# honglianghe/CDNet

Measured on AMD Instinct MI355X. Metric: tiles/sec (train fwd+bwd+Adam), 256x256, higher is better.
Workload: dtype fp32

## Files before the change

cdnet_amd/_lib.py:

```python
import ctypes as C
import os

_HERE = os.path.dirname(os.path.abspath(__file__))
LIB_PATH = os.environ.get('CDNET_LIB_PATH') or os.path.join(_HERE, 'libcdnet_hip.so')

_vp, _i, _sz, _f, _u = C.c_void_p, C.c_int, C.c_size_t, C.c_float, C.c_uint


class ConvSrc(C.Structure):
    _fields_ = [('x', C.c_void_p), ('res', C.c_void_p), ('scale', C.c_void_p), ('shift', C.c_void_p),
                ('C', C.c_int), ('Hs', C.c_int), ('Ws', C.c_int), ('pool', C.c_int), ('relu', C.c_int),
                ('off_y', C.c_int), ('off_x', C.c_int), ('f16', C.c_int), ('row_stride', C.c_int)]


class ConvArgs(C.Structure):
    _fields_ = [('src', ConvSrc * 2), ('nsrc', C.c_int), ('w', C.c_void_p), ('bias', C.c_void_p),
                ('oscale', C.c_void_p), ('oshift', C.c_void_p), ('orelu', C.c_int), ('out', C.c_void_p),
                ('Cout', C.c_int), ('out_cstride', C.c_int), ('out_coff', C.c_int), ('stats', C.c_void_p),
                ('N', C.c_int), ('H', C.c_int), ('W', C.c_int), ('taps', C.c_int), ('npar', C.c_int),
                ('ostride', C.c_int), ('nchunk', C.c_int), ('tile', C.c_int), ('CK', C.c_int), ('BN', C.c_int),
                ('out_f16', C.c_int), ('debug', C.c_int), ('ws', C.c_int), ('f32', C.c_int),
                ('eres', C.c_void_p), ('eres_scale', C.c_void_p), ('eres_shift', C.c_void_p), ('eres_f16', C.c_int), ('eres_relu', C.c_int),
                ('taps1', C.c_int), ('pad_', C.c_int), ('pool_out', C.c_void_p),
                ('dot_w', C.c_void_p), ('dot_b', C.c_void_p), ('dot_out', C.c_void_p)]


class PackJob(C.Structure):
    _fields_ = [('w', C.c_void_p), ('packed', C.c_void_p), ('Cout', C.c_int), ('Cin', C.c_int), ('KH', C.c_int), ('KW', C.c_int),
                ('CK', C.c_int), ('BN', C.c_int), ('mode', C.c_int), ('pad_', C.c_int)]


class HeadFeat(C.Structure):
    _fields_ = [('raw', C.c_void_p), ('res', C.c_void_p), ('scale', C.c_void_p), ('shift', C.c_void_p),
                ('relu', C.c_int), ('f16', C.c_int)]


class FuseTerm(C.Structure):
    _fields_ = [('x', C.c_void_p), ('Hs', C.c_int), ('Ws', C.c_int), ('scale', C.c_void_p), ('shift', C.c_void_p),
                ('f16', C.c_int), ('pad_', C.c_int)]


class GradTerm(C.Structure):
    _fields_ = [('g', C.c_void_p), ('cstride', C.c_int), ('coff', C.c_int)]


class GradIn(C.Structure):
    _fields_ = [('g', C.c_void_p), ('Hg', C.c_int), ('Wg', C.c_int), ('oy', C.c_int), ('ox', C.c_int),
                ('pooled', C.c_int), ('coff', C.c_int), ('cstride', C.c_int), ('pad_', C.c_int)]


class BnBwdArgs(C.Structure):
    _fields_ = [('raw', C.c_void_p), ('res', C.c_void_p), ('scale', C.c_void_p), ('shift', C.c_void_p),
                ('mean', C.c_void_p), ('invstd', C.c_void_p), ('gin', GradIn * 3), ('ngin', C.c_int),
                ('f16', C.c_int), ('relu', C.c_int), ('N', C.c_int), ('H', C.c_int), ('W', C.c_int), ('C', C.c_int)]


class AugSample(C.Structure):
    _fields_ = [('minv', C.c_double * 6), ('img', C.c_void_p), ('weight', C.c_void_p), ('label', C.c_void_p)] + \
        [(n, C.c_int32) for n in ('H', 'W', 'img_stride', 'weight_stride', 'label_stride', 'label_i32')] + \
        [('color', C.c_float * 4)] + [(n, C.c_int32) for n in ('hflip', 'vflip', 'filter', 'y0', 'x0')] + \
        [('alpha', C.c_float), ('sigma', C.c_float), ('seed', C.c_uint32)]


class AugGeo(C.Structure):
    _fields_ = [('paff', C.c_double * 6), ('rinv', C.c_double * 6)] + [(n, C.c_int32) for n in ('Hr', 'Wr', 'fy0', 'fx0')] + \
        [('flags', C.c_uint32), ('reserved', C.c_int32)]


class WgradReduceDesc(C.Structure):
    _fields_ = [('slab', C.c_void_p), ('dw', C.c_void_p)] + [(n, C.c_int) for n in (
        'ksplit', 'npar', 'ci_blocks', 'co_blocks', 'taps', 'CI', 'CO', 'Csrc_real', 'Cin_real', 'src_coff', 'Cout', 'mode', 'block0', 'blocks')]

class DilatedConvArgs(C.Structure):
    _fields_ = [(n, C.c_void_p) for n in ('in_', 'w', 'scale', 'shift', 'out')] + [(n, C.c_int) for n in (
        'N', 'H', 'W', 'Cin', 'in_cstride', 'Cout', 'out_cstride', 'out_coff', 'taps', 'dilation', 'leaky')] + [
        ('slope', C.c_float), ('f32', C.c_int), ('out_nchw', C.c_int)]

class DilatedBwdDataArgs(C.Structure):
    _fields_ = [(n, C.c_void_p) for n in ('g', 'w', 'dx')] + [(n, C.c_int) for n in (
        'N', 'H', 'W', 'Cout', 'g_cstride', 'Cin', 'dx_cstride', 'dx_coff', 'taps', 'dilation', 'accumulate', 'f32')]

class DilatedWgradArgs(C.Structure):
    _fields_ = [(n, C.c_void_p) for n in ('x', 'g', 'dw', 'ws')] + [('ws_bytes', C.c_size_t)] + [(n, C.c_int) for n in (
        'N', 'H', 'W', 'Cin', 'x_cstride', 'Cout', 'g_cstride', 'taps', 'dilation')]

class SliceBnFwdArgs(C.Structure):
    _fields_ = [(n, C.c_void_p) for n in ('z', 'out', 'gamma', 'beta', 'running_mean', 'running_var', 'mean', 'invstd', 'ws')] + [
        ('ws_floats', C.c_size_t), ('P', C.c_longlong)] + [(n, C.c_int) for n in ('C', 'z_cstride', 'out_cstride', 'out_coff')] + [
        (n, C.c_float) for n in ('eps', 'momentum', 'p_drop')] + [('layer', C.c_int), ('key', C.c_ulonglong)]

class SliceBnBwdArgs(C.Structure):
    _fields_ = [(n, C.c_void_p) for n in ('dy', 'z', 'mean', 'invstd', 'gamma', 'dgamma', 'dbeta', 'g', 'ws')] + [
        ('ws_floats', C.c_size_t), ('P', C.c_longlong)] + [(n, C.c_int) for n in ('C', 'z_cstride', 'dy_cstride', 'dy_coff', 'g_cstride')] + [
        (n, C.c_float) for n in ('slope', 'p_drop')] + [('layer', C.c_int), ('key', C.c_ulonglong)]


MIRRORS = {
    'cdnet_conv_src': ConvSrc, 'cdnet_conv_args': ConvArgs, 'cdnet_pack_job': PackJob, 'cdnet_head_feat': HeadFeat,
    'cdnet_wgrad_reduce_desc': WgradReduceDesc, 'cdnet_grad_in': GradIn, 'cdnet_bn_bwd_args': BnBwdArgs, 'cdnet_fuse_term': FuseTerm,
    'cdnet_grad_term': GradTerm, 'cdnet_aug_sample': AugSample, 'cdnet_aug_geo': AugGeo, 'cdnet_dilated_conv_args': DilatedConvArgs,
    'cdnet_dilated_bwd_data_args': DilatedBwdDataArgs, 'cdnet_dilated_wgrad_args': DilatedWgradArgs,
    'cdnet_slice_bn_fwd_args': SliceBnFwdArgs, 'cdnet_slice_bn_bwd_args': SliceBnBwdArgs,
}

SIGNATURES = {
    'cdnet_abi_version': (_i, []),
    'cdnet_abi_sizeof': (_sz, [C.c_char_p]),
    'cdnet_last_error': (C.c_char_p, []),
    'cdnet_build_info': (C.c_char_p, []),
    'cdnet_spin': (_i, [_i, _vp]),
    'cdnet_box_copy': (_i, [_vp, _vp, _sz, _vp]),
    'cdnet_box_mfma': (_i, [_vp, _vp, _vp, _i, _i, _i, _vp]),
    'cdnet_ddm_codes': (_i, [_vp, _i, _i, _i, _i, _vp, _i, _i, _vp, _vp, _vp]),
    'cdnet_ddm_normalize': (_i, [_vp, _vp, _i, _i, _i, _vp, _vp]),
    'cdnet_probmaps': (_i, [_vp, _vp, _i, _i, _i, _i, _vp, _vp, _vp]),
    'cdnet_tta_boost_argmax': (_i, [_vp, _vp, _vp, _vp, _i, _i, _vp, _i, _i, _vp, _vp, _vp, _vp, _vp, _vp]),
    'cdnet_fuse_sum': (_i, [_vp, _i, _i, _i, _i, _i, _i, _vp, _i, _i, _vp]),
    'cdnet_upsample_bilinear_backward': (_i, [_vp, _i, _i, _i, _i, _i, _i, _i, _i, _vp, _vp]),
    'cdnet_s2d_to_nhwc': (_i, [_vp, _i, _i, _i, _i, _vp, _vp]),
    'cdnet_fuse_sum_f32': (_i, [_vp, _i, _i, _i, _i, _i, _i, _vp, _i, _i, _vp]),
    'cdnet_upsample_bilinear_backward_f32': (_i, [_vp, _i, _i, _i, _i, _i, _i, _i, _i, _vp, _vp]),
    'cdnet_s2d_to_nhwc_f32': (_i, [_vp, _i, _i, _i, _i, _vp, _vp]),
    'cdnet_bn_backward_stats': (_i, [_vp, _vp, _vp, _vp, _vp, _sz, _vp, _vp]),
    'cdnet_bn_backward_apply': (_i, [_vp, _vp, _vp, _vp]),
    'cdnet_bn_backward_finalize': (_i, [_vp, _vp, _vp, _vp, _vp, _i, _vp, _vp]),
    'cdnet_conv_ws_eligible': (_i, [_vp]),
    'cdnet_grad_sum': (_i, [_vp, _i, _vp, C.c_longlong, _i, _vp, _vp]),
    'cdnet_grad_sum_f32': (_i, [_vp, _i, _vp, C.c_longlong, _i, _vp, _vp]),
    'cdnet_label_pair_histogram': (_i, [_vp, _vp, _i, _i, _i, _i, _vp, _vp, _vp, _vp, _vp, _vp]),
    'cdnet_remap_label': (_i, [_vp, _i, _i, _i, _vp, _vp, _vp, _vp]),
    'cdnet_label_areas': (_i, [_vp, _i, _i, _i, _vp, _vp, _vp]),
    'cdnet_label_apply': (_i, [_vp, _i, _i, _i, _vp, _vp, _vp]),
    'cdnet_label_csr_workspace_bytes': (_sz, [_i]),
    'cdnet_label_csr': (_i, [_vp, _i, _i, _i, _vp, _sz, _vp, _vp, _vp, _vp, _vp]),
    'cdnet_hausdorff_tile_pixels': (_i, []),
    'cdnet_hausdorff_chunk_pixels': (_i, []),
    'cdnet_hausdorff_pairs': (_i, [_vp] * 8 + [_i, _i, _i, _vp, _i, _vp, _i, _vp, _vp, _vp]),
    'cdnet_watershed_workspace_bytes': (_sz, [_i, _i, _i]),
    'cdnet_watershed_process': (_i, [_vp, _i, _i, _i, _i, _vp, _sz, _vp, _vp, _vp, _vp]),
    'cdnet_fill_label_process': (_i, [_vp, _i, _i, _i, _i, _vp, _sz, _vp, _vp]),
    'cdnet_label_process': (_i, [_vp, _i, _i, _i, _i, _vp, _sz, _vp, _vp]),
    'cdnet_instance_redilate_workspace_bytes': (_sz, [_i, _i, _i, _i]),
    'cdnet_instance_redilate': (_i, [_vp, _i, _i, _i, _i, _i, _vp, _sz, _vp, _vp, _vp]),
    'cdnet_instance_redilate_lds_rows': (_i, []),
    'cdnet_instance_redilate_lds_cols': (_i, []),
    'cdnet_label_count': (_i, [_vp, _i, _i, _i, _vp, _vp, _vp, _vp]),
    'cdnet_tile_postproc_workspace_bytes': (_sz, [_i, _i, _i, _i]),
    'cdnet_tile_postproc': (_i, [_vp, _vp, _vp, _i, _i, _i, _i, _vp, _i, _i, _i, _i, _vp, _sz] + [_vp] * 10),
    'cdnet_cc_workspace_bytes': (_sz, [_i, _i, _i]),
    'cdnet_cc_chain': (_i, [_vp, _i, _i, _i, _i, _i, _i, _vp, _sz, _vp, _vp, _vp, _vp, _vp, _vp]),
    'cdnet_mask_views_argmax': (_i, [_vp, _i, _i, _i, _vp, _i, _i, _vp, _vp, _vp]),
    'cdnet_tile_mask_postproc_workspace_bytes': (_sz, [_i, _i, _i, _i]),
    'cdnet_tile_mask_postproc': (_i, [_vp, _i, _i, _i, _i, _i, _i, _vp, _sz] + [_vp] * 8),
    'cdnet_dilate_labels': (_i, [_vp, _i, _i, _i, _i, _vp, _vp]),
    'cdnet_conv_packed_weight_elems': (_sz, [_i] * 6),
    'cdnet_pack_conv_weights': (_i, [_vp, _vp] + [_i] * 7 + [_vp]),
    'cdnet_pack_conv_weights_scaled': (_i, [_vp, _vp, _vp] + [_i] * 7 + [_vp]),
    'cdnet_pack_batch_table_bytes': (_sz, [_i]),
    'cdnet_pack_conv_weights_batch': (_i, [_vp, _i, _vp, _sz, _i, _vp]),
    'cdnet_conv_forward': (_i, [_vp, _vp]),
    'cdnet_dilated_packed_weight_elems': (_sz, [_i, _i, _i, _i]),
    'cdnet_dilated_pack_weights': (_i, [_vp, _vp, _i, _i, _i, _i, _vp]),
    'cdnet_dilated_conv_forward': (_i, [_vp, _vp]),
    'cdnet_dilated_pack_weights_bwd': (_i, [_vp, _vp, _i, _i, _i, _i, _vp]),
    'cdnet_dilated_conv_backward_data': (_i, [_vp, _vp]),
    'cdnet_dilated_wgrad_workspace_bytes': (_sz, [_i] * 6),
    'cdnet_dilated_conv_backward_weight': (_i, [_vp, _vp]),
    'cdnet_slice_bn_workspace_floats': (_sz, [C.c_longlong, _i]),
    'cdnet_slice_bn_train_forward': (_i, [_vp, _vp]),
    'cdnet_slice_bn_train_backward': (_i, [_vp, _vp]),
    'cdnet_dropout_mask': (_i, [C.c_ulonglong, _i, _sz, _f, _vp, _vp]),
    'cdnet_maxpool2_forward': (_i, [_vp, _i, _vp, _i, _i, _vp, _i, _i, _i, _i, _i, _i, _vp]),
    'cdnet_maxpool2_backward': (_i, [_vp, _i, _i, _vp, _i, _vp, _i, _i, _i, _i, _i, _vp]),
    'cdnet_upsample4_bilinear_forward': (_i, [_vp, _i, _vp, _i, _i, _i, _i, _i, _i, _i, _vp]),
    'cdnet_upsample4_bilinear_backward': (_i, [_vp, _i, _i, _vp, _i, _i, _i, _i, _i, _vp]),
    'cdnet_src_materialize': (_i, [_vp, _i, _i, _i, _vp, _vp]),
    'cdnet_input_pack': (_i, [_vp, _i, _i, _i, _i, _vp, _vp]),
    'cdnet_input_pack_f32': (_i, [_vp, _i, _i, _i, _i, _vp, _vp]),
    'cdnet_bn_fold_eval': (_i, [_vp, _vp, _vp, _vp, _vp, _f, _i, _vp, _vp, _vp]),
    'cdnet_bn_finalize_train': (_i, [_vp, _i, _i, _f, _vp, _vp, _vp, _f, _f, _vp, _vp, _vp, _vp, _vp, _vp, _vp]),
    'cdnet_dam_head_forward': (_i, [_vp, _vp, _vp, _vp, _i, _i, _i, _vp, _vp, _vp, _vp]),
    'cdnet_final_conv1x1': (_i, [_vp, _vp, _vp, _i, _i, _i, _i, _vp, _vp]),
    'cdnet_bias_grad_workspace_floats': (_sz, [_i]),
    'cdnet_bias_grad': (_i, [_vp, _sz, _i, _vp, _sz, _vp, _vp]),
    'cdnet_bias_grad_f32': (_i, [_vp, _sz, _i, _vp, _sz, _vp, _vp]),
    'cdnet_final_conv1x1_backward_workspace_floats': (_sz, []),
    'cdnet_final_conv1x1_backward': (_i, [_vp, _vp, _vp, _i, _i, _i, _i, _vp, _vp, _sz, _vp, _vp, _vp]),
    'cdnet_final_conv1x1_c16': (_i, [_vp, _vp, _vp, _i, _i, _i, _i, _vp, _vp]),
    'cdnet_final_conv1x1_c16_backward_workspace_floats': (_sz, []),
    'cdnet_final_conv1x1_c16_backward': (_i, [_vp, _vp, _vp, _i, _i, _i, _i, _vp, _vp, _sz, _vp, _vp, _vp]),
    'cdnet_conv_wgrad_slab_floats': (_sz, [_i] * 6),
    'cdnet_conv_backward_weight': (_i, [_vp, _i, _i, _i, _vp] + [_i] * 9 + [_vp, _vp, _i, _vp]),
    'cdnet_conv_backward_weight_last_form': (_i, []),
    'cdnet_conv_forward_last_form': (_i, []),
    'cdnet_wgrad_reduce_desc_fill': (_i, [_i] * 9 + [_vp, _vp, _i, _i, _vp]),
    'cdnet_wgrad_reduce_batch': (_i, [_vp, _i, _i, _vp]),
    'cdnet_bn_backward_workspace_floats': (_sz, [_i]),
    'cdnet_bn_backward': (_i, [_vp, _vp, _vp, _vp, _vp, _sz, _vp, _vp, _vp]),
    'cdnet_bn_backward_last_plan': (_i, []),
    'cdnet_bn_backward_last_sums_plan': (_i, []),
    'cdnet_dam_head_backward_workspace_floats': (_sz, [_i, _i, _i]),
    'cdnet_dam_head_backward': (_i, [_vp] * 7 + [_i, _i, _i, _vp, _vp, _vp, _vp, _sz, _vp, _vp]),
    'cdnet_dam_head_backward_fused_blocks': (_i, []),
    'cdnet_dam_head_backward_fused_scratch_bytes': (_i, []),
    'cdnet_dam_head_backward_fused_workspace_floats': (_sz, []),
    'cdnet_dam_head_backward_fused': (_i, [_vp] * 7 + [_i, _i, _i, _vp, _vp, _vp, _vp, _sz, _vp, _vp]),
    'cdnet_dam_loss_workspace_floats': (_sz, [_i, _i]),
    'cdnet_dam_loss': (_i, [_vp] * 7 + [_i, _i, _i, _i, _vp, _sz, _vp, _vp, _vp, _vp, _vp]),
    'cdnet_dam_loss_classes_workspace_floats': (_sz, [_i, _i, _i]),
    'cdnet_dam_loss_classes': (_i, [_vp] * 7 + [_i, _i, _i, _i, _i, _vp, _sz, _vp, _vp, _vp, _vp, _vp]),
    'cdnet_dam_loss_terms': (_i, [_vp] * 7 + [_i, _i, _i, _i, _i, _vp, _sz, _vp, _vp, _vp, _vp, _vp, _u]),
    'cdnet_mask_loss_workspace_floats': (_sz, [_i, _i]),
    'cdnet_mask_loss': (_i, [_vp, _vp, _vp, _i, _i, _i, _u, _vp, _sz, _vp, _vp, _vp]),
    'cdnet_variance_loss_workspace_bytes': (_sz, [_i, _i, _i, _i]),
    'cdnet_variance_loss': (_i, [_vp, _vp, _i, _i, _i, _i, _i, _f, _vp, _sz, _vp, _vp, _vp, _vp, _vp, _vp]),
    'cdnet_boundary_loss_workspace_bytes': (_sz, [_i, _i, _i, _i, _i]),
    'cdnet_boundary_loss': (_i, [_vp, _vp, _i, _i, _i, _i, _i, _f, _vp, _sz, _vp, _vp, _vp, _vp]),
    'cdnet_boundary_loss_scratch_bytes': (_i, []),
    'cdnet_dam_val_sums_workspace_floats': (_sz, [_i, _i]),
    'cdnet_dam_val_sums': (_i, [_vp] * 8 + [_i, _i, _i, _vp, _sz, _vp, _vp]),
    'cdnet_dam_val_sums_classes_workspace_floats': (_sz, [_i, _i, _i]),
    'cdnet_dam_val_sums_classes': (_i, [_vp] * 8 + [_i, _i, _i, _i, _vp, _sz, _vp, _vp]),
    'cdnet_adam_step': (_i, [_vp, _vp, _vp, _vp, _sz, _f, _f, _f, _f, _f, _i, _f, _vp]),
    'cdnet_moment_step': (_i, [_vp, _vp, _vp, _vp, _vp, _sz, C.c_double, C.c_double, _f, _i, _i, _f, _f, _f, _f, _i, _f, _vp]),
    'cdnet_sgd_step': (_i, [_vp, _vp, _vp, _sz, _f, _f, _f, _i, _f, _vp]),
    'cdnet_window_pack': (_i, [_vp] + [_i] * 9 + [_vp, _vp]),
    'cdnet_window_pack_f32': (_i, [_vp] + [_i] * 9 + [_vp, _vp]),
    'cdnet_window_stitch': (_i, [_vp] + [_i] * 9 + [_vp, _vp]),
    'cdnet_label_encoding_workspace_bytes': (_sz, [_i, _i, _i, _i]),
    'cdnet_label_encoding_instances_workspace_bytes': (_sz, [_i, _i, _i, _i]),
    'cdnet_label_encoding_instances': (_i, [_vp, _i, _i, _i, _i, _vp, _vp, _vp, _sz, _vp, _vp, _vp, _vp, _vp, _vp]),
    'cdnet_augment_workspace_bytes': (_sz, [_i, _i, _i]),
    'cdnet_augment_batch': (_i, [_vp, _vp, _i, _i, _vp, _vp, _sz, _vp, _vp, _vp, _i, _vp, _vp, _vp]),
    'cdnet_augment_geo_workspace_bytes': (_sz, [_i, _i, _i, _i]),
    'cdnet_augment_batch_geo': (_i, [_vp, _vp, _vp, _vp, _i, _i, _i, _vp, _vp, _sz, _vp, _vp, _vp, _i, _vp, _vp, _vp]),
    'cdnet_label_encoding': (_i, [_vp, _i, _i, _i, _i, _vp, _vp, _vp, _sz, _vp, _vp, _vp, _vp, _vp, _vp]),
    'cdnet_weight_map_radius': (_i, [C.c_double, C.c_double]),
    'cdnet_weight_map': (_i, [_vp, _i, _i, C.c_double, C.c_double, _vp, _vp]),
}

_lib = None


class CdnetHipError(RuntimeError):
    pass


def load():
    global _lib
    if _lib is not None:
        return _lib
    import torch
    if not os.path.exists(LIB_PATH):
        raise CdnetHipError('libcdnet_hip.so is not built: run `python -m cdnet_amd.csrc.build` '
                            '(or __graft_entry__.build()). There is no CPU fallback.')
    lib = C.CDLL(LIB_PATH)
    for name, (res, args) in SIGNATURES.items():
        fn = getattr(lib, name)
        fn.restype = res
        fn.argtypes = args
    if lib.cdnet_abi_version() != 5:
        raise CdnetHipError('ABI version mismatch (libcdnet_hip.so is version %d, this binding 5): rebuild with python -m cdnet_amd.csrc.build' % lib.cdnet_abi_version())
    _lib = lib
    return lib


def check(status, what=''):
    if status != 0:
        msg = load().cdnet_last_error().decode(errors='replace')
        raise CdnetHipError('%s failed (code %d): %s' % (what, status, msg))


def call(name, *args):
    check(getattr(load(), name)(*args), name)


def entry(name, f32):
    return name + '_f32' if f32 else name


_RAW_STREAM = None


def stream_ptr():
    global _RAW_STREAM
    if _RAW_STREAM is None:
        import torch
        get, dev = getattr(torch._C, '_cuda_getCurrentRawStream', None), getattr(torch._C, '_cuda_getDevice', None)
        if get is not None and dev is not None:
            _RAW_STREAM = lambda: get(dev())
        else:
            _RAW_STREAM = lambda: torch.cuda.current_stream().cuda_stream
    return C.c_void_p(_RAW_STREAM())


def ptr(t):
    if t is None:
        return None
    assert t.is_cuda and t.is_contiguous(), 'ABI needs contiguous device tensors'
    return C.c_void_p(t.data_ptr())
```

cdnet_amd/csrc/bn_bwd.hip:

```cpp
#include "train_util.h"
#include "bn_sums.h"

using namespace cdnet;

namespace {

struct GradIn {
    const unsigned short *g;
    int Hg, Wg;
    int oy, ox;
    int pooled;
    int coff, cstride;
};

struct BnBwdArgs {
    const unsigned short *raw;
    const unsigned short *res;
    int f16;
    const float *scale, *shift;
    int relu;
    const float *mean, *invstd;
    GradIn gin[3];
    int ngin;
    int N, H, W, C;
    float *partial;
    const float *k1, *k2, *k3;
    unsigned short *draw;
    unsigned short *dz_out;
    int rev;
};


__device__ __forceinline__ void act8_f32(const BnBwdArgs &A, size_t e, const float *sc, const float *sh, float *a, float *rawf) {
    float x[8], r[8];
    ldf8(A.raw, e, x);
    if (A.res) ldf8(A.res, e, r);
#pragma unroll
    for (int j = 0; j < 8; ++j) {
        if (rawf) rawf[j] = x[j];
        float v = A.scale ? fmaf(x[j], sc[j], sh[j]) : x[j];
        if (A.relu == 2) v = r[j];
        else {
            if (A.res) v += r[j];
            if (A.relu) v = fmaxf(v, 0.f);
        }
        a[j] = v;
    }
}

template <bool F32 = false>
__device__ __forceinline__ void act8(const BnBwdArgs &A, size_t e, const float *sc, const float *sh, float *a, float *rawf) {
    if (F32) { act8_f32(A, e, sc, sh, a, rawf); return; }
    V16 r, rr;
    r.u = *reinterpret_cast<const uint4 *>(A.raw + e);
    rr.u = make_uint4(0, 0, 0, 0);
    if (A.res) rr.u = *reinterpret_cast<const uint4 *>(A.res + e);
    const bool f16 = A.f16 != 0;
#pragma unroll
    for (int j = 0; j < 8; ++j) {
        float x = ld16(r.h[j], f16);
        if (rawf) rawf[j] = x;
        float v = A.scale ? fmaf(x, sc[j], sh[j]) : x;
        if (A.res) v += ld16(rr.h[j], f16);
        if (A.relu) v = fmaxf(v, 0.f);
        a[j] = bf2f(f2bf(v));
    }
}

template <bool WANT_XHAT, bool F32 = false>
__device__ __forceinline__ void dz8(const BnBwdArgs &A, int n, int y, int x, int c0, const float *sc, const float *sh,
                                    const float *mu, const float *is, float *dz, float *xhat) {
    const size_t e = (((size_t)n * A.H + y) * A.W + x) * A.C + c0;
    float a[8], rawf[8];
    act8<F32>(A, e, sc, sh, a, rawf);
    float g[8];
#pragma unroll
    for (int j = 0; j < 8; ++j) g[j] = 0.f;
    for (int k = 0; k < A.ngin; ++k) {
        const GradIn &gi = A.gin[k];
        if (!gi.pooled) {
            const int yy = y + gi.oy, xx = x + gi.ox;
            if (yy >= 0 && yy < gi.Hg && xx >= 0 && xx < gi.Wg) {
                const size_t ge = (((size_t)n * gi.Hg + yy) * gi.Wg + xx) * gi.cstride + gi.coff + c0;
                if (F32) {
                    float t[8];
                    ldf8(gi.g, ge, t);
#pragma unroll
                    for (int j = 0; j < 8; ++j) g[j] += t[j];
                } else {
                    V16 v;
                    v.u = *reinterpret_cast<const uint4 *>(gi.g + ge);
#pragma unroll
                    for (int j = 0; j < 8; ++j) g[j] += bf2f(v.h[j]);
                }
            }
        } else {
            const int py = y >> 1, px = x >> 1;
            if (py < gi.Hg && px < gi.Wg) {
                bool sel[8];
#pragma unroll
                for (int j = 0; j < 8; ++j) sel[j] = true;
                const int q0 = (y & 1) * 2 + (x & 1);
#pragma unroll
                for (int q = 0; q < 4; ++q) {
                    if (q == q0) continue;
                    const int yy = (y & ~1) + (q >> 1), xx = (x & ~1) + (q & 1);
                    if (yy >= A.H || xx >= A.W) continue;
                    float b[8];
                    act8<F32>(A, (((size_t)n * A.H + yy) * A.W + xx) * A.C + c0, sc, sh, b, nullptr);
#pragma unroll
                    for (int j = 0; j < 8; ++j) sel[j] = sel[j] && (q < q0 ? a[j] > b[j] : a[j] >= b[j]);
                }
                const size_t ge = (((size_t)n * gi.Hg + py) * gi.Wg + px) * gi.cstride + gi.coff + c0;
                if (F32) {
                    float t[8];
                    ldf8(gi.g, ge, t);
#pragma unroll
                    for (int j = 0; j < 8; ++j) g[j] += sel[j] ? t[j] : 0.f;
                } else {
                    V16 v;
                    v.u = *reinterpret_cast<const uint4 *>(gi.g + ge);
#pragma unroll
                    for (int j = 0; j < 8; ++j) g[j] += sel[j] ? bf2f(v.h[j]) : 0.f;
                }
            }
        }
    }
#pragma unroll
    for (int j = 0; j < 8; ++j) {
        dz[j] = (A.relu && !(a[j] > 0.f)) ? 0.f : g[j];
        if (WANT_XHAT) xhat[j] = A.mean ? (rawf[j] - mu[j]) * is[j] : 0.f;
    }
}

template <int V>
__device__ __forceinline__ void bn_load_row(const float *p, int c0, float *o, float dflt) {
#pragma unroll
    for (int j = 0; j < V; ++j) o[j] = p ? p[c0 + j] : dflt;
}

template <int V>
__device__ __forceinline__ void bn_load_const(const BnBwdArgs &A, int c0, bool apply, float (&sc)[V], float (&sh)[V], float (&mu)[V], float (&is)[V],
                                              float (&k1)[V], float (&k2)[V], float (&k3)[V]) {
    bn_load_row<V>(A.scale, c0, sc, 1.f); bn_load_row<V>(A.shift, c0, sh, 0.f); bn_load_row<V>(A.mean, c0, mu, 0.f); bn_load_row<V>(A.invstd, c0, is, 1.f);
    if (apply) { bn_load_row<V>(A.k1, c0, k1, 1.f); bn_load_row<V>(A.k2, c0, k2, 0.f); bn_load_row<V>(A.k3, c0, k3, 0.f); }
}

template <int V>
__device__ __forceinline__ void bn_write_partial(float *partial, int C, int VPP, const float *s1, const float *s2) {
    __shared__ float s_red[256][2 * V + 1];
    const int tid = threadIdx.x;
#pragma unroll
    for (int j = 0; j < V; ++j) { s_red[tid][j] = s1[j]; s_red[tid][V + j] = s2[j]; }
    __syncthreads();
    for (int q = tid; q < 2 * V * VPP; q += 256) {
        const int sl = q % VPP, j = q / VPP;
        float t = 0.f;
        for (int k = sl; k < 256; k += VPP) t += s_red[k][j];
        float *op = partial + (size_t)blockIdx.x * 2 * C;
        op[(j / V) * C + sl * V + (j % V)] = t;
    }
}

constexpr int BN_U = 4;
constexpr int BN_MAX_BLOCKS = 2048;
constexpr int BN_BLOCKS_CAP = 512;
static_assert(BN_BLOCKS_CAP <= BN_MAX_BLOCKS, "workspace rows");

static int bn_grid(size_t count, int C, int V, int unroll) {
    const size_t per_block = (size_t)(256 / (C / V)) * unroll;
    const size_t nb = (count + per_block - 1) / per_block;
    return nb > (size_t)BN_BLOCKS_CAP ? BN_BLOCKS_CAP : (nb < 1 ? 1 : (int)nb);
}

template <bool F32 = false>
__device__ __forceinline__ void dz8_at(const BnBwdArgs &A, unsigned p, unsigned HW, int c0, const float *sc, const float *sh, const float *mu,
                                       const float *is, float *dz, float *xh) {
    const unsigned n = p / HW, r = p - n * HW;
    const unsigned y = r / (unsigned)A.W, x = r - y * (unsigned)A.W;
    dz8<true, F32>(A, (int)n, (int)y, (int)x, c0, sc, sh, mu, is, dz, xh);
}

template <typename Body>
__device__ __forceinline__ void bn_bwd_dispatch(bool f16, int relu, Body &&body) {
    using T_ = std::true_type;
    using F_ = std::false_type;
    if (f16) {
        if (relu == 0) body(T_{}, std::integral_constant<int, 0>{});
        else if (relu == 1) body(T_{}, std::integral_constant<int, 1>{});
        else body(T_{}, std::integral_constant<int, 2>{});
    } else {
        if (relu == 0) body(F_{}, std::integral_constant<int, 0>{});
        else if (relu == 1) body(F_{}, std::integral_constant<int, 1>{});
        else body(F_{}, std::integral_constant<int, 2>{});
    }
}

template <int NF, bool APPLY>
__global__ __launch_bounds__(256) void bn_bwd_window_kernel(BnBwdArgs A, int kp) {
    const int VPP = A.C / 8;
    const int slot = (int)threadIdx.x % VPP, c0 = slot * 8;
    float sc[8], sh[8], mu[8], is[8], k1[8], k2[8], k3[8], s1[8], s2[8];
    bn_load_const(A, c0, APPLY, sc, sh, mu, is, k1, k2, k3);
#pragma unroll
    for (int j = 0; j < 8; ++j) { s1[j] = 0.f; s2[j] = 0.f; }
    const unsigned H = A.H, W = A.W, Hp = (H + 1) / 2, Wp = (W + 1) / 2, nwin = (unsigned)A.N * Hp * Wp;
    const unsigned ppb = 256 / VPP;
    const GradIn gp = A.gin[kp];
    int kf[2] = {0, 0};
    {
        int m = 0;
        for (int k = 0; k < A.ngin && m < NF; ++k)
            if (k != kp) kf[m++] = k;
    }
    bn_bwd_dispatch(A.f16 != 0, A.relu != 0 ? 1 : 0, [&](auto f16_c, auto relu_c) {
    constexpr bool f16 = decltype(f16_c)::value, relu = decltype(relu_c)::value != 0;
    for (unsigned w0 = first_pixel(ppb, VPP); w0 < nwin; w0 += gridDim.x * ppb) {
        const unsigned w = (APPLY && A.rev) ? nwin - 1 - w0 : w0;
        const unsigned n = w / (Hp * Wp), r = w - n * Hp * Wp;
        const unsigned py = r / Wp, px = r - py * Wp;
        V16 raw[4], g[4][NF > 0 ? NF : 1], gv;
        unsigned pix[4];
        bool ok[4];
#pragma unroll
        for (int q = 0; q < 4; ++q) {
            unsigned yy = 2 * py + (q >> 1), xx = 2 * px + (q & 1);
            ok[q] = yy < H && xx < W;
            yy = yy < H ? yy : H - 1;
            xx = xx < W ? xx : W - 1;
            pix[q] = (n * H + yy) * W + xx;
            raw[q].u = *reinterpret_cast<const uint4 *>(A.raw + (size_t)pix[q] * A.C + c0);
#pragma unroll
            for (int m = 0; m < NF; ++m)
                g[q][m].u = *reinterpret_cast<const uint4 *>(A.gin[kf[m]].g + (size_t)pix[q] * A.gin[kf[m]].cstride + A.gin[kf[m]].coff + c0);
        }
        const bool pok = py < (unsigned)gp.Hg && px < (unsigned)gp.Wg;
        {
            const unsigned cy = pok ? py : 0, cx = pok ? px : 0;
            gv.u = *reinterpret_cast<const uint4 *>(gp.g + (((size_t)n * gp.Hg + cy) * gp.Wg + cx) * gp.cstride + gp.coff + c0);
        }
        V16 o[4];
#pragma unroll
        for (int j = 0; j < 8; ++j) {
            float x[4], a[4];
#pragma unroll
            for (int q = 0; q < 4; ++q) {
                x[q] = ld16(raw[q].h[j], f16);
                float v = fmaf(x[q], sc[j], sh[j]);
                if (relu) v = fmaxf(v, 0.f);
                a[q] = bf2f(f2bf(v));
            }
            int bi = 0;
            float best = a[0];
#pragma unroll
            for (int q = 1; q < 4; ++q)
                if (ok[q] && a[q] > best) { best = a[q]; bi = q; }
            const float gpool = pok ? bf2f(gv.h[j]) : 0.f;
#pragma unroll
            for (int q = 0; q < 4; ++q) {
                float gs = (bi == q) ? gpool : 0.f;
#pragma unroll
                for (int m = 0; m < NF; ++m) gs += bf2f(g[q][m].h[j]);
                const float dz = (!ok[q] || (relu && !(a[q] > 0.f))) ? 0.f : gs;
                const float xh = (x[q] - mu[j]) * is[j];
                if (APPLY) o[q].h[j] = f2bf(k1[j] * (dz - k2[j] - xh * k3[j]));
                else { s1[j] += dz; s2[j] = fmaf(dz, xh, s2[j]); }
            }
        }
        if (APPLY) {
#pragma unroll
            for (int q = 0; q < 4; ++q)
                if (ok[q]) *reinterpret_cast<uint4 *>(A.draw + (size_t)pix[q] * A.C + c0) = o[q].u;
        }
    }
    });
    if (!APPLY) bn_write_partial<8>(A.partial, A.C, VPP, s1, s2);
}

template <int NG, bool RES, bool APPLY>
__global__ __launch_bounds__(256) void bn_bwd_flat_kernel(BnBwdArgs A) {
    const int VPP = A.C / 8;
    const int slot = (int)threadIdx.x % VPP, c0 = slot * 8;
    float sc[8], sh[8], mu[8], is[8], k1[8], k2[8], k3[8], s1[8], s2[8];
    bn_load_const(A, c0, APPLY, sc, sh, mu, is, k1, k2, k3);
#pragma unroll
    for (int j = 0; j < 8; ++j) { s1[j] = 0.f; s2[j] = 0.f; }
    const unsigned npix = (unsigned)(A.N * A.H * A.W);
    const unsigned ppb = 256 / VPP, step = gridDim.x * ppb;
    const bool rev = APPLY && A.rev != 0;
    bn_bwd_dispatch(A.f16 != 0, A.relu, [&](auto f16_c, auto relu_c) {
        constexpr bool F16 = decltype(f16_c)::value;
        constexpr int RELU = decltype(relu_c)::value;
        for (unsigned p0 = first_pixel(ppb, VPP); p0 < npix; p0 += step * BN_U) {
            V16 raw[BN_U], res[BN_U], g[BN_U][NG];
#pragma unroll
            for (int u = 0; u < BN_U; ++u) {
                unsigned p = p0 + u * step;
                p = p < npix ? p : npix - 1;
                p = rev ? npix - 1 - p : p;
                raw[u].u = *reinterpret_cast<const uint4 *>(A.raw + (size_t)p * A.C + c0);
                if (RES) res[u].u = *reinterpret_cast<const uint4 *>(A.res + (size_t)p * A.C + c0);
#pragma unroll
                for (int k = 0; k < NG; ++k)
                    g[u][k].u = *reinterpret_cast<const uint4 *>(A.gin[k].g + (size_t)p * A.gin[k].cstride + A.gin[k].coff + c0);
            }
#pragma unroll
            for (int u = 0; u < BN_U; ++u) {
                const unsigned p = p0 + u * step;
                const bool valid = p < npix;
                V16 o, z;
#pragma unroll
                for (int j = 0; j < 8; ++j) {
                    const float x = ld16(raw[u].h[j], F16);
                    float v = fmaf(x, sc[j], sh[j]);
                    if (RES) v = RELU == 2 ? bf2f(res[u].h[j]) : v + ld16(res[u].h[j], F16);
                    float gs = bf2f(g[u][0].h[j]);
#pragma unroll
                    for (int k = 1; k < NG; ++k) gs += bf2f(g[u][k].h[j]);
                    const bool keep = (APPLY || valid) & (RELU == 0 || bf2f(f2bf(v)) > 0.f);
                    const float dz = keep ? gs : 0.f;
                    const float xh = (x - mu[j]) * is[j];
                    if (APPLY) {
                        o.h[j] = f2bf(k1[j] * (dz - k2[j] - xh * k3[j]));
                        z.h[j] = f2bf(dz);
                    } else {
                        s1[j] += dz;
                        s2[j] = fmaf(dz, xh, s2[j]);
                        if (RES) res[u].h[j] = f2bf(dz);
                    }
                }
                if (APPLY) {
                    if (valid) {
                        const unsigned pw = rev ? npix - 1 - p : p;
                        *reinterpret_cast<uint4 *>(A.draw + (size_t)pw * A.C + c0) = o.u;
                        if (RES) *reinterpret_cast<uint4 *>(A.dz_out + (size_t)pw * A.C + c0) = z.u;
                    }
                } else {
                    if (RES && A.dz_out && valid) *reinterpret_cast<uint4 *>(A.dz_out + (size_t)p * A.C + c0) = res[u].u;
                }
            }
        }
    });
    if (!APPLY) bn_write_partial<8>(A.partial, A.C, VPP, s1, s2);
}

template <int NG, bool RES, bool APPLY>
__global__ __launch_bounds__(256) void bn_bwd_flat32_kernel(BnBwdArgs A) {
    const int VPP = A.C / 4;
    const int slot = (int)threadIdx.x % VPP, c0 = slot * 4;
    float sc[4], sh[4], mu[4], is[4], k1[4], k2[4], k3[4], s1[4], s2[4];
    bn_load_row<4>(A.scale, c0, sc, 1.f); bn_load_row<4>(A.shift, c0, sh, 0.f); bn_load_row<4>(A.mean, c0, mu, 0.f); bn_load_row<4>(A.invstd, c0, is, 1.f);
    if (APPLY) { bn_load_row<4>(A.k1, c0, k1, 1.f); bn_load_row<4>(A.k2, c0, k2, 0.f); bn_load_row<4>(A.k3, c0, k3, 0.f); }
#pragma unroll
    for (int j = 0; j < 4; ++j) { s1[j] = 0.f; s2[j] = 0.f; }
    const unsigned npix = (unsigned)(A.N * A.H * A.W);
    const unsigned ppb = 256 / VPP, step = gridDim.x * ppb;
    const bool relu = A.relu != 0, outmask = A.relu == 2;
    const float *raw = reinterpret_cast<const float *>(A.raw), *resp = reinterpret_cast<const float *>(A.res);
    float *draw = reinterpret_cast<float *>(A.draw), *dzo = reinterpret_cast<float *>(A.dz_out);
    for (unsigned p0 = first_pixel(ppb, VPP); p0 < npix; p0 += step * BN_U) {
        f32x4 x[BN_U], r[BN_U], g[BN_U][NG];
#pragma unroll
        for (int u = 0; u < BN_U; ++u) {
            unsigned p = p0 + u * step;
            p = p < npix ? p : npix - 1;
            if (APPLY && A.rev) p = npix - 1 - p;
            x[u] = *reinterpret_cast<const f32x4 *>(raw + (size_t)p * A.C + c0);
            if (RES) r[u] = *reinterpret_cast<const f32x4 *>(resp + (size_t)p * A.C + c0);
#pragma unroll
            for (int k = 0; k < NG; ++k)
                g[u][k] = *reinterpret_cast<const f32x4 *>(reinterpret_cast<const float *>(A.gin[k].g) + (size_t)p * A.gin[k].cstride + A.gin[k].coff + c0);
        }
#pragma unroll
        for (int u = 0; u < BN_U; ++u) {
            const unsigned p = p0 + u * step;
            const bool valid = p < npix;
            f32x4 o, z;
#pragma unroll
            for (int j = 0; j < 4; ++j) {
                float v = fmaf(x[u][j], sc[j], sh[j]);
                if (RES) v = outmask ? r[u][j] : v + r[u][j];
                float gs = g[u][0][j];
#pragma unroll
                for (int k = 1; k < NG; ++k) gs += g[u][k][j];
                const float dz = (!valid || (relu && !(v > 0.f))) ? 0.f : gs;
                const float xh = (x[u][j] - mu[j]) * is[j];
                if (APPLY) { o[j] = k1[j] * (dz - k2[j] - xh * k3[j]); z[j] = dz; }
                else { s1[j] += dz; s2[j] = fmaf(dz, xh, s2[j]); z[j] = dz; }
            }
            if (APPLY && valid) {
                const unsigned pw = A.rev ? npix - 1 - p : p;
                *reinterpret_cast<f32x4 *>(draw + (size_t)pw * A.C + c0) = o;
                if (RES) *reinterpret_cast<f32x4 *>(dzo + (size_t)pw * A.C + c0) = z;
            }
            if (!APPLY && RES && dzo && valid) *reinterpret_cast<f32x4 *>(dzo + (size_t)p * A.C + c0) = z;
        }
    }
    if (!APPLY) bn_write_partial<4>(A.partial, A.C, VPP, s1, s2);
}

template <int NF, bool APPLY>
__global__ __launch_bounds__(256) void bn_bwd_window32_kernel(BnBwdArgs A, int kp) {
    const int VPP = A.C / 4;
    const int slot = (int)threadIdx.x % VPP, c0 = slot * 4;
    float sc[4], sh[4], mu[4], is[4], k1[4], k2[4], k3[4], s1[4], s2[4];
    bn_load_const(A, c0, APPLY, sc, sh, mu, is, k1, k2, k3);
#pragma unroll
    for (int j = 0; j < 4; ++j) { s1[j] = 0.f; s2[j] = 0.f; }
    const unsigned H = A.H, W = A.W, Hp = (H + 1) / 2, Wp = (W + 1) / 2, nwin = (unsigned)A.N * Hp * Wp;
    const unsigned ppb = 256 / VPP;
    const bool relu = A.relu != 0;
    const GradIn gp = A.gin[kp];
    const float *gpool_p = reinterpret_cast<const float *>(gp.g);
    const float *raw = reinterpret_cast<const float *>(A.raw);
    float *draw = reinterpret_cast<float *>(A.draw);
    const float *gf[NF > 0 ? NF : 1];
    int gcs[NF > 0 ? NF : 1], gco[NF > 0 ? NF : 1];
    {
        int m = 0;
        for (int k = 0; k < A.ngin && m < NF; ++k)
            if (k != kp) { gf[m] = reinterpret_cast<const float *>(A.gin[k].g); gcs[m] = A.gin[k].cstride; gco[m] = A.gin[k].coff; ++m; }
    }
    for (unsigned w0 = first_pixel(ppb, VPP); w0 < nwin; w0 += gridDim.x * ppb) {
        const unsigned w = (APPLY && A.rev) ? nwin - 1 - w0 : w0;
        const unsigned n = w / (Hp * Wp), r = w - n * Hp * Wp;
        const unsigned py = r / Wp, px = r - py * Wp;
        f32x4 x[4], g[4][NF > 0 ? NF : 1], gv;
        unsigned pix[4];
        bool ok[4];
#pragma unroll
        for (int q = 0; q < 4; ++q) {
            unsigned yy = 2 * py + (q >> 1), xx = 2 * px + (q & 1);
            ok[q] = yy < H && xx < W;
            yy = yy < H ? yy : H - 1;
            xx = xx < W ? xx : W - 1;
            pix[q] = (n * H + yy) * W + xx;
            x[q] = *reinterpret_cast<const f32x4 *>(raw + (size_t)pix[q] * A.C + c0);
#pragma unroll
            for (int m = 0; m < NF; ++m)
                g[q][m] = *reinterpret_cast<const f32x4 *>(gf[m] + (size_t)pix[q] * gcs[m] + gco[m] + c0);
        }
        const bool pok = py < (unsigned)gp.Hg && px < (unsigned)gp.Wg;
        {
            const unsigned cy = pok ? py : 0, cx = pok ? px : 0;
            gv = *reinterpret_cast<const f32x4 *>(gpool_p + (((size_t)n * gp.Hg + cy) * gp.Wg + cx) * gp.cstride + gp.coff + c0);
        }
        f32x4 o[4];
#pragma unroll
        for (int j = 0; j < 4; ++j) {
            float a[4];
#pragma unroll
            for (int q = 0; q < 4; ++q) {
                const float v = fmaf(x[q][j], sc[j], sh[j]);
                a[q] = relu ? fmaxf(v, 0.f) : v;
            }
            int bi = 0;
            float best = a[0];
#pragma unroll
            for (int q = 1; q < 4; ++q)
                if (ok[q] && a[q] > best) { best = a[q]; bi = q; }
            const float gpool = pok ? gv[j] : 0.f;
#pragma unroll
            for (int q = 0; q < 4; ++q) {
                const float pt = (bi == q) ? gpool : 0.f;
                float gsum;
                if (NF == 0) gsum = 0.f + pt;
                else if (NF == 1) gsum = (0.f + (kp == 0 ? pt : g[q][0][j])) + (kp == 0 ? g[q][0][j] : pt);
                else gsum = ((0.f + (kp == 0 ? pt : g[q][0][j])) + (kp == 0 ? g[q][0][j] : (kp == 1 ? pt : g[q][NF - 1][j]))) +
                            (kp == 2 ? pt : g[q][NF - 1][j]);
                const float dz = (!ok[q] || (relu && !(a[q] > 0.f))) ? 0.f : gsum;
                const float xh = (x[q][j] - mu[j]) * is[j];
                if (APPLY) o[q][j] = k1[j] * (dz - k2[j] - xh * k3[j]);
                else { s1[j] += dz; s2[j] = fmaf(dz, xh, s2[j]); }
            }
        }
        if (APPLY) {
#pragma unroll
            for (int q = 0; q < 4; ++q)
                if (ok[q]) *reinterpret_cast<f32x4 *>(draw + (size_t)pix[q] * A.C + c0) = o[q];
        }
    }
    if (!APPLY) bn_write_partial<4>(A.partial, A.C, VPP, s1, s2);
}

template <bool F32, bool APPLY>
__global__ __launch_bounds__(256) void bn_bwd_generic_kernel(BnBwdArgs A) {
    const int VPP = A.C / 8;
    const int slot = (int)threadIdx.x % VPP, c0 = slot * 8;
    float sc[8], sh[8], mu[8], is[8], k1[8], k2[8], k3[8], s1[8], s2[8];
    bn_load_const(A, c0, APPLY, sc, sh, mu, is, k1, k2, k3);
#pragma unroll
    for (int j = 0; j < 8; ++j) { s1[j] = 0.f; s2[j] = 0.f; }
    const unsigned HW = (unsigned)(A.H * A.W), npix = (unsigned)A.N * HW;
    const unsigned ppb = 256 / VPP;
    const unsigned step = gridDim.x * ppb;
    for (unsigned p0 = first_pixel(ppb, VPP); p0 < npix; p0 += step * BN_U) {
        float dz[BN_U][8], xh[BN_U][8];
#pragma unroll
        for (int u = 0; u < BN_U; ++u) {
            const unsigned p = p0 + u * step;
            if (p < npix) dz8_at<F32>(A, p, HW, c0, sc, sh, mu, is, dz[u], xh[u]);
            else if (!APPLY) {
#pragma unroll
                for (int j = 0; j < 8; ++j) { dz[u][j] = 0.f; xh[u][j] = 0.f; }
            }
        }
#pragma unroll
        for (int u = 0; u < BN_U; ++u) {
            const unsigned p = p0 + u * step;
            if (!APPLY) {
#pragma unroll
                for (int j = 0; j < 8; ++j) { s1[j] += dz[u][j]; s2[j] = fmaf(dz[u][j], xh[u][j], s2[j]); }
                continue;
            }
            if (p >= npix) continue;
            float o32[8];
#pragma unroll
            for (int j = 0; j < 8; ++j) o32[j] = k1[j] * (dz[u][j] - k2[j] - xh[u][j] * k3[j]);
            if (F32) {
                if (A.draw) stf8(A.draw, (size_t)p * A.C + c0, o32);
                if (A.dz_out) stf8(A.dz_out, (size_t)p * A.C + c0, dz[u]);
                continue;
            }
            V16 o, z;
#pragma unroll
            for (int j = 0; j < 8; ++j) { o.h[j] = f2bf(o32[j]); z.h[j] = f2bf(dz[u][j]); }
            if (A.draw) *reinterpret_cast<uint4 *>(A.draw + (size_t)p * A.C + c0) = o.u;
            if (A.dz_out) *reinterpret_cast<uint4 *>(A.dz_out + (size_t)p * A.C + c0) = z.u;
        }
    }
    if (!APPLY) bn_write_partial<8>(A.partial, A.C, VPP, s1, s2);
}

__global__ __launch_bounds__(256) void bn_bwd_finalize_kernel(const float *__restrict__ partial, int nb, int C, float M, const float *gamma,
                                                              const float *invstd, float *dgamma, float *dbeta, float *k1, float *k2,
                                                              float *k3) {
    const int c = blockIdx.x;
    double s1, s2;
    bn_sum_partials(partial, nb, C, c, s1, s2);
    if (threadIdx.x == 0) {
        if (dbeta) dbeta[c] = (float)s1;
        if (dgamma) dgamma[c] = (float)s2;
        k1[c] = gamma[c] * invstd[c];
        k2[c] = (float)(s1 / M);
        k3[c] = (float)(s2 / M);
    }
}

__global__ void bn_ktab_copy_kernel(const float *scale, const float *shift, const float *mean, const float *invstd, int C, float *ktab) {
    const int c = blockIdx.x * blockDim.x + threadIdx.x;
    if (c < C) { ktab[c] = scale[c]; ktab[C + c] = shift[c]; ktab[2 * C + c] = mean[c]; ktab[3 * C + c] = invstd[c]; }
}

}

static int fill_bn_args(const cdnet_bn_bwd_args *a, BnBwdArgs &A, const char *who) {
    CDNET_REQUIRE(a && a->raw, "%s: null pointer", who);
    CDNET_REQUIRE(a->C % 8 == 0 && a->C >= 8 && a->C <= 2048 , "%s: C=%d unsupported", who, a->C);
    CDNET_REQUIRE(a->ngin >= 1 && a->ngin <= 3, "%s: ngin=%d", who, a->ngin);
    A.raw = a->raw; A.res = a->res; A.f16 = a->f16; A.scale = a->scale; A.shift = a->shift; A.relu = a->relu;
    A.mean = a->mean; A.invstd = a->invstd;
    for (int k = 0; k < 3; ++k) {
        A.gin[k].g = a->gin[k].g; A.gin[k].Hg = a->gin[k].Hg; A.gin[k].Wg = a->gin[k].Wg;
        A.gin[k].oy = a->gin[k].oy; A.gin[k].ox = a->gin[k].ox; A.gin[k].pooled = a->gin[k].pooled;
        A.gin[k].coff = a->gin[k].coff; A.gin[k].cstride = a->gin[k].cstride ? a->gin[k].cstride : a->C;
        if (k < a->ngin) CDNET_REQUIRE(a->gin[k].g, "%s: null gradient input %d", who, k);
        if (k < a->ngin) CDNET_REQUIRE(a->gin[k].Hg >= 1 && a->gin[k].Wg >= 1, "%s: empty gradient input %d (%d x %d)", who, k, a->gin[k].Hg, a->gin[k].Wg);
    }
    A.ngin = a->ngin; A.N = a->N; A.H = a->H; A.W = a->W; A.C = a->C;
    A.partial = nullptr; A.k1 = A.k2 = A.k3 = nullptr; A.draw = nullptr; A.dz_out = nullptr;
    return CDNET_OK;
}

enum BnPath { BN_WINDOW, BN_FLAT, BN_GENERIC };
struct BnPlan {
    BnPath path;
    bool f32;
    int nb;
    int kp, nflat;
    bool flat_sources;
};

static size_t bn_npix(const BnBwdArgs &A) { return (size_t)A.N * A.H * A.W; }

static BnPlan bn_plan_plain(const BnBwdArgs &A) {
    const bool f32 = A.f16 == 2;
    return BnPlan{BN_FLAT, f32, bn_grid(bn_npix(A), A.C, f32 ? 4 : 8, BN_U), 0, 0, true};
}

static BnPlan bn_plan(const BnBwdArgs &A, const void *draw, const void *dz_out) {
    bool simple = true;
    int npool = 0, kp = 0, nflat = 0;
    for (int k = 0; k < A.ngin; ++k) {
        const GradIn &g = A.gin[k];
        const bool same = !g.pooled && g.oy == 0 && g.ox == 0 && g.Hg == A.H && g.Wg == A.W;
        simple = simple && same;
        if (g.pooled) { ++npool; kp = k; }
        else if (same) ++nflat;
    }
    const bool window = npool == 1 && nflat == A.ngin - 1 && nflat <= 2 && A.mean && A.scale && !A.res && draw && !dz_out;
    const bool flat = !window && simple && A.mean && A.scale && draw && ((A.res != nullptr) == (dz_out != nullptr));
    const bool f32 = A.f16 == 2, fits32 = A.C <= 1024;
    BnPlan P{BN_GENERIC, f32, 0, kp, nflat, flat};
    if (window && (!f32 || (fits32 && A.shift && A.invstd))) P.path = BN_WINDOW;
    else if (flat && (!f32 || fits32)) P.path = BN_FLAT;
    const int V = f32 && P.path != BN_GENERIC ? 4 : 8;
    P.nb = window ? bn_grid((size_t)A.N * ((A.H + 1) / 2) * ((A.W + 1) / 2), A.C, V, 1) : bn_grid(bn_npix(A), A.C, V, BN_U);
    return P;
}

static thread_local int g_bn_last_plan[2] = {0, 0};
static thread_local int g_bn_last_pass = 0;

static int bn_plan_record(const BnPlan &P, const BnBwdArgs &A, bool apply, bool dz_source) {
    const int path = P.path == BN_WINDOW ? CDNET_BN_PATH_WINDOW : P.path == BN_FLAT ? CDNET_BN_PATH_FLAT : CDNET_BN_PATH_GENERIC;
    const int n = P.path == BN_WINDOW ? P.nflat : P.path == BN_FLAT ? A.ngin : 0;
    const int res = P.path == BN_FLAT && A.res ? 1 : 0;
    const int kp = P.path == BN_WINDOW ? P.kp : 0;
    return path | (P.f32 ? 1 : 0) << 2 | n << 3 | res << 5 | kp << 6 | (apply ? 1 : 0) << 8 | (dz_source ? 1 : 0) << 9 | P.nb << 10;
}

template <bool APPLY>
static void launch(const BnPlan &P, const BnBwdArgs &A, hipStream_t st, bool dz_source = false) {
    g_bn_last_plan[APPLY ? 1 : 0] = bn_plan_record(P, A, APPLY, dz_source);
    g_bn_last_pass = APPLY ? 1 : 0;
    auto window = [&](auto nf) {
        constexpr int NF = decltype(nf)::value;
        if (P.f32) bn_bwd_window32_kernel<NF, APPLY><<<P.nb, 256, 0, st>>>(A, P.kp);
        else bn_bwd_window_kernel<NF, APPLY><<<P.nb, 256, 0, st>>>(A, P.kp);
    };
    auto flat = [&](auto ng, auto res) {
        constexpr int NG = decltype(ng)::value;
        constexpr bool RES = decltype(res)::value;
        if (P.f32) bn_bwd_flat32_kernel<NG, RES, APPLY><<<P.nb, 256, 0, st>>>(A);
        else bn_bwd_flat_kernel<NG, RES, APPLY><<<P.nb, 256, 0, st>>>(A);
    };
    using std::integral_constant;
    using std::true_type;
    using std::false_type;
    switch (P.path) {
        case BN_WINDOW:
            if (P.nflat == 0) window(integral_constant<int, 0>{});
            else if (P.nflat == 1) window(integral_constant<int, 1>{});
            else window(integral_constant<int, 2>{});
            break;
        case BN_FLAT:
            switch (A.ngin * 2 + (A.res ? 1 : 0)) {
                case 2: flat(integral_constant<int, 1>{}, false_type{}); break;
                case 3: flat(integral_constant<int, 1>{}, true_type{}); break;
                case 4: flat(integral_constant<int, 2>{}, false_type{}); break;
                case 5: flat(integral_constant<int, 2>{}, true_type{}); break;
                case 6: flat(integral_constant<int, 3>{}, false_type{}); break;
                default: flat(integral_constant<int, 3>{}, true_type{}); break;
            }
            break;
        case BN_GENERIC:
            if (P.f32) bn_bwd_generic_kernel<true, APPLY><<<P.nb, 256, 0, st>>>(A);
            else bn_bwd_generic_kernel<false, APPLY><<<P.nb, 256, 0, st>>>(A);
            break;
    }
}

static void bn_finalize(const BnBwdArgs &A, const float *partial, int nb, const float *gamma, float *dgamma, float *dbeta, float *k,
                        hipStream_t st) {
    bn_bwd_finalize_kernel<<<A.C, 256, 0, st>>>(partial, nb, A.C, (float)bn_npix(A), gamma, A.invstd, dgamma, dbeta, k, k + A.C, k + 2 * A.C);
}

static void bn_set_coeffs(BnBwdArgs &A, const float *k) { A.k1 = k; A.k2 = k + A.C; A.k3 = k + 2 * A.C; }

static BnBwdArgs bn_dz_as_source(const BnBwdArgs &A, const unsigned short *dz) {
    BnBwdArgs B = A;
    B.ngin = 1;
    B.gin[0].g = dz; B.gin[0].Hg = A.H; B.gin[0].Wg = A.W; B.gin[0].oy = 0; B.gin[0].ox = 0; B.gin[0].pooled = 0;
    B.gin[0].coff = 0; B.gin[0].cstride = A.C;
    B.res = nullptr; B.relu = 0; B.dz_out = nullptr;
    return B;
}

extern "C" int cdnet_bn_backward(const cdnet_bn_bwd_args *a, const float *gamma, float *dgamma, float *dbeta, float *workspace,
                                 size_t workspace_floats, uint16_t *draw, uint16_t *dz_out, void *stream) {
    BnBwdArgs A;
    int rc = fill_bn_args(a, A, "cdnet_bn_backward");
    if (rc) return rc;
    hipStream_t st = (hipStream_t)stream;
    const size_t npix = bn_npix(A);
    CDNET_REQUIRE(npix * (size_t)A.C < ((size_t)1 << 32) && npix < ((size_t)1 << 31), "cdnet_bn_backward: tensor too large for 32-bit pixel indexing");
    const BnPlan P = bn_plan(A, draw, dz_out);
    CDNET_REQUIRE(A.relu != 2 || (P.flat_sources && A.res), "cdnet_bn_backward: relu = 2 (mask from the stored output) needs same-size gradient sources and res");
    static const bool dz_reuse = !(getenv("CDNET_BN_DZ_REUSE") && atoi(getenv("CDNET_BN_DZ_REUSE")) == 0);
    const bool reuse = dz_reuse && P.path == BN_FLAT && A.mean && A.res && dz_out;
    A.draw = draw;
    A.rev = 1;
    if (A.mean) {
        CDNET_REQUIRE(gamma && A.invstd && workspace, "cdnet_bn_backward: BatchNorm layer needs gamma/invstd/workspace");
        const size_t need = (size_t)P.nb * 2 * A.C + 3 * (size_t)A.C;
        if (workspace_floats < need) { set_error("cdnet_bn_backward: workspace %zu < %zu floats", workspace_floats, need); return CDNET_E_WORKSPACE; }
        A.partial = workspace;
        A.dz_out = dz_reuse ? dz_out : nullptr;
        float *k = workspace + (size_t)P.nb * 2 * A.C;
        launch<false>(P, A, st);
        bn_finalize(A, A.partial, P.nb, gamma, dgamma, dbeta, k, st);
        bn_set_coeffs(A, k);
    }
    A.dz_out = dz_out;
    launch<true>(P, reuse ? bn_dz_as_source(A, dz_out) : A, st, reuse);
    return check_launch("cdnet_bn_backward");
}

static bool bn_plain_case(const BnBwdArgs &A, bool masked = false) {
    const GradIn &g = A.gin[0];
    return A.ngin == 1 && !g.pooled && g.oy == 0 && g.ox == 0 && g.Hg == A.H && g.Wg == A.W && A.mean && A.scale && A.shift && A.invstd && !A.res &&
           (A.relu == 1 || (masked && A.relu == 0)) && (g.cstride == 0 || g.cstride == A.C) && g.coff == 0;
}

extern "C" int cdnet_bn_backward_stats(const cdnet_bn_bwd_args *a, const float *gamma, float *dgamma, float *dbeta, float *workspace,
                                       size_t workspace_floats, float *ktab, void *stream) {
    BnBwdArgs A;
    int rc = fill_bn_args(a, A, "cdnet_bn_backward_stats");
    if (rc) return rc;
    CDNET_REQUIRE(bn_plain_case(A) && A.f16 != 2 && gamma && workspace && ktab, "cdnet_bn_backward_stats: plain 16-bit case only (one same-size gradient, BatchNorm + ReLU, no residual)");
    hipStream_t st = (hipStream_t)stream;
    const size_t npix = bn_npix(A);
    CDNET_REQUIRE(npix * (size_t)A.C < ((size_t)1 << 32) && npix < ((size_t)1 << 31), "cdnet_bn_backward_stats: tensor too large for 32-bit pixel indexing");
    const BnPlan P = bn_plan_plain(A);
    const size_t need = (size_t)P.nb * 2 * A.C;
    if (workspace_floats < need) { set_error("cdnet_bn_backward_stats: workspace %zu < %zu floats", workspace_floats, need); return CDNET_E_WORKSPACE; }
    A.partial = workspace;
    A.rev = 0;
    bn_ktab_copy_kernel<<<cdiv(A.C, 256), 256, 0, st>>>(A.scale, A.shift, A.mean, A.invstd, A.C, ktab);
    launch<false>(P, A, st);
    bn_finalize(A, A.partial, P.nb, gamma, dgamma, dbeta, ktab + 4 * A.C, st);
    return check_launch("cdnet_bn_backward_stats");
}

extern "C" int cdnet_bn_backward_finalize(const cdnet_bn_bwd_args *a, const float *gamma, float *dgamma, float *dbeta, const float *partial,
                                          int nb, float *ktab, void *stream) {
    BnBwdArgs A;
    int rc = fill_bn_args(a, A, "cdnet_bn_backward_finalize");
    if (rc) return rc;
    CDNET_REQUIRE(bn_plain_case(A) && gamma && partial && ktab && nb >= 1, "cdnet_bn_backward_finalize: plain case only");
    bn_finalize(A, partial, nb, gamma, dgamma, dbeta, ktab + 4 * A.C, (hipStream_t)stream);
    return check_launch("cdnet_bn_backward_finalize");
}

extern "C" int cdnet_bn_backward_apply(const cdnet_bn_bwd_args *a, const float *ktab, uint16_t *draw, void *stream) {
    BnBwdArgs A;
    int rc = fill_bn_args(a, A, "cdnet_bn_backward_apply");
    if (rc) return rc;
    CDNET_REQUIRE(bn_plain_case(A, true) && ktab && draw, "cdnet_bn_backward_apply: plain case only");
    CDNET_REQUIRE(A.f16 != 2 || A.C <= 1024, "cdnet_bn_backward_apply(f32): C=%d > 1024", A.C);
    A.rev = 1;
    A.draw = draw;
    bn_set_coeffs(A, ktab + 4 * A.C);
    launch<true>(bn_plan_plain(A), A, (hipStream_t)stream);
    return check_launch("cdnet_bn_backward_apply");
}

extern "C" int cdnet_bn_backward_last_plan(void) { return g_bn_last_plan[g_bn_last_pass]; }
extern "C" int cdnet_bn_backward_last_sums_plan(void) { return g_bn_last_plan[0]; }

extern "C" size_t cdnet_bn_backward_workspace_floats(int C) { return (size_t)BN_MAX_BLOCKS * 2 * C + 3 * (size_t)C; }
```

cdnet_amd/csrc/head_bwd.hip:

```cpp
#include "train_util.h"
#include "head_feat.h"

using namespace cdnet;

namespace {

__device__ __forceinline__ void feat8_f32(const HeadFeat &f, size_t pix, int c0, const float *s_sc, const float *s_sh, float *v) {
    float x[8], r[8];
    ldf8(f.raw, pix * 64 + c0, x);
    if (f.res) ldf8(f.res, pix * 64 + c0, r);
#pragma unroll
    for (int j = 0; j < 8; ++j) {
        float t = x[j];
        if (f.scale) t = fmaf(t, s_sc[c0 + j], s_sh[c0 + j]);
        if (f.res) t += r[j];
        if (f.relu) t = fmaxf(t, 0.f);
        v[j] = t;
    }
}

__device__ __forceinline__ void feat8(const HeadFeat &f, size_t pix, int c0, const float *s_sc, const float *s_sh, float *v) {
    if (f.f16 == 2) { feat8_f32(f, pix, c0, s_sc, s_sh, v); return; }
    V16 r, rr;
    r.u = *reinterpret_cast<const uint4 *>(f.raw + pix * 64 + c0);
    rr.u = make_uint4(0, 0, 0, 0);
    if (f.res) rr.u = *reinterpret_cast<const uint4 *>(f.res + pix * 64 + c0);
    if (f.f16 && f.scale && f.relu) {
        const u32x4 a = __builtin_bit_cast(u32x4, r.u), b = __builtin_bit_cast(u32x4, rr.u);
        if (f.res) xf_bnrelu_f16_to_f32<true>(a, b, s_sc + c0, s_sh + c0, v);
        else xf_bnrelu_f16_to_f32<false>(a, a, s_sc + c0, s_sh + c0, v);
        return;
    }
#pragma unroll
    for (int j = 0; j < 8; ++j) {
        float x = f.f16 ? h2f(r.h[j]) : bf2f(r.h[j]);
        if (f.scale || f.res || f.relu) {
            if (f.scale) x = fmaf(x, s_sc[c0 + j], s_sh[c0 + j]);
            if (f.res) x += f.f16 ? h2f(rr.h[j]) : bf2f(rr.h[j]);
            if (f.relu) x = fmaxf(x, 0.f);
            x = bf2f(f2bf(x));
        }
        v[j] = x;
    }
}

struct FeatRaw8 {
    uint4 r, s;
};
template <int FM>
__device__ __forceinline__ void load_raw8(const HeadFeat &f, size_t pix, int c0, FeatRaw8 &R) {
    R.r = *reinterpret_cast<const uint4 *>(f.raw + pix * 64 + c0);
    R.s = make_uint4(0, 0, 0, 0);
    if (FM == 1 || (FM == 2 && f.res)) R.s = *reinterpret_cast<const uint4 *>(f.res + pix * 64 + c0);
}
template <int FM>
__device__ __forceinline__ void feat_from_raw8(const HeadFeat &f, const FeatRaw8 &R, int c0, const float *s_sc, const float *s_sh, float *v) {
    const u32x4 a = __builtin_bit_cast(u32x4, R.r), b = __builtin_bit_cast(u32x4, R.s);
    if (FM == 1) { xf_bnrelu_f16_to_f32<true>(a, b, s_sc + c0, s_sh + c0, v); return; }
    if (FM == 0) {
        V16 r0;
        r0.u = R.r;
#pragma unroll
        for (int j = 0; j < 8; ++j) v[j] = bf2f(r0.h[j]);
        return;
    }
    if (f.f16 && f.scale && f.relu) {
        if (f.res) xf_bnrelu_f16_to_f32<true>(a, b, s_sc + c0, s_sh + c0, v);
        else xf_bnrelu_f16_to_f32<false>(a, a, s_sc + c0, s_sh + c0, v);
        return;
    }
    V16 r, rr;
    r.u = R.r; rr.u = R.s;
#pragma unroll
    for (int j = 0; j < 8; ++j) {
        float x = f.f16 ? h2f(r.h[j]) : bf2f(r.h[j]);
        if (f.scale || f.res || f.relu) {
            if (f.scale) x = fmaf(x, s_sc[c0 + j], s_sh[c0 + j]);
            if (f.res) x += f.f16 ? h2f(rr.h[j]) : bf2f(rr.h[j]);
            if (f.relu) x = fmaxf(x, 0.f);
            x = bf2f(f2bf(x));
        }
        v[j] = x;
    }
}

__device__ __forceinline__ void feat16(const HeadFeat &f, size_t pix, int q, const float *s_sc, const float *s_sh, float *v) {
    feat8(f, pix, q * 16, s_sc, s_sh, v);
    feat8(f, pix, q * 16 + 8, s_sc, s_sh, v + 8);
}
__device__ __forceinline__ void store16_bf16(unsigned short *dst, const float *v) {
#pragma unroll
    for (int h2 = 0; h2 < 2; ++h2) {
        V16 o;
#pragma unroll
        for (int j = 0; j < 8; ++j) o.h[j] = f2bf(v[h2 * 8 + j]);
        reinterpret_cast<uint4 *>(dst)[h2] = o.u;
    }
}

__device__ __forceinline__ void store16_grad(unsigned short *base, size_t e, const float *v, bool f32) {
    if (f32) { stf8(base, e, v); stf8(base, e + 8, v + 8); }
    else store16_bf16(base + e, v);
}

template <int FM>
__global__ __launch_bounds__(256) void dam_head_bwd_kernel(HeadFeat f1, HeadFeat f2, HeadFeat f3, const HeadW *__restrict__ hw,
                                                           const float *__restrict__ dmask, const float *__restrict__ dpoint,
                                                           const float *__restrict__ ddir, int N, int plane,
                                                           unsigned short *__restrict__ df1, unsigned short *__restrict__ df2,
                                                           unsigned short *__restrict__ df3, float *__restrict__ coef,
                                                           float *__restrict__ partial) {
    __shared__ HeadW w;
    __shared__ float s_sc[3][64], s_sh[3][64];
    __shared__ float s_red[64][24];
    const int tid = threadIdx.x;
    {
        const float *src = reinterpret_cast<const float *>(hw);
        float *dst = reinterpret_cast<float *>(&w);
        for (int i = tid; i < HEADW_FLOATS; i += 256) dst[i] = src[i];
        if (tid < 64) {
            const HeadFeat *fs[3] = {&f1, &f2, &f3};
#pragma unroll
            for (int k = 0; k < 3; ++k) {
                s_sc[k][tid] = fs[k]->scale ? fs[k]->scale[tid] : 1.f;
                s_sh[k][tid] = fs[k]->scale ? fs[k]->shift[tid] : 0.f;
            }
        }
    }
    __syncthreads();
    const size_t total = (size_t)N * plane;
    const int q = tid & 3;
    const bool f32 = f1.f16 == 2;
    float sg[23];
#pragma unroll
    for (int j = 0; j < 23; ++j) sg[j] = 0.f;
    for (size_t base = (size_t)blockIdx.x * 64; base < total; base += (size_t)gridDim.x * 64) {
        const size_t i = base + (tid >> 2);
        const bool ok = i < total;
        const size_t ii = ok ? i : total - 1;
        const size_t n = ii / plane, p = ii - n * plane;
        asm volatile("" ::: "memory");
        float v[16];
        FeatRaw8 R3[2], R2[2], R1[2];
        constexpr bool all16 = FM != 2;
        if (all16) {
#pragma unroll
            for (int h2 = 0; h2 < 2; ++h2) {
                load_raw8<FM>(f3, ii, q * 16 + h2 * 8, R3[h2]);
                load_raw8<FM>(f2, ii, q * 16 + h2 * 8, R2[h2]);
                load_raw8<FM>(f1, ii, q * 16 + h2 * 8, R1[h2]);
            }
        }
        float go_m[3], go_d[9], go_p;
#pragma unroll
        for (int k = 0; k < 3; ++k) go_m[k] = ok ? dmask[(n * 3 + k) * plane + p] : 0.f;
#pragma unroll
        for (int k = 0; k < 9; ++k) go_d[k] = ok ? ddir[(n * 9 + k) * plane + p] : 0.f;
        go_p = ok ? dpoint[n * plane + p] : 0.f;
        auto feat = [&](const HeadFeat &f, const FeatRaw8 (&R)[2], int k) {
            if (all16) {
                feat_from_raw8<FM>(f, R[0], q * 16, s_sc[k], s_sh[k], v);
                feat_from_raw8<FM>(f, R[1], q * 16 + 8, s_sc[k], s_sh[k], v + 8);
            } else {
                feat16(f, ii, q, s_sc[k], s_sh[k], v);
            }
        };
        feat(f3, R3, 2);
        const float pt = xf_quad_sum(xf_dot16(w.wp + q * 16, v)) + w.bp;
        const float sg1 = 1.f / (1.f + expf(-(w.a1 * pt)));
        const float g1 = 1.f + sg1;
        feat(f2, R2, 1);
        float u[9], d[9], q2 = 0.f;
#pragma unroll
        for (int k = 0; k < 9; ++k) {
            u[k] = xf_quad_sum(xf_dot16(w.wd[k] + q * 16, v));
            d[k] = fmaf(g1, u[k], w.bd[k]);
            q2 = fmaf(w.a2[k], d[k], q2);
        }
        const float sg2 = 1.f / (1.f + expf(-q2));
        const float g2 = 1.f + sg2;
        feat(f1, R1, 0);
        float dm[3], dg2 = 0.f;
#pragma unroll
        for (int k = 0; k < 3; ++k) {
            const float mk = xf_quad_sum(xf_dot16(w.wm[k] + q * 16, v));
            const float go = go_m[k];
            dg2 = fmaf(go, mk, dg2);
            dm[k] = go * g2;
            sg[k] += go;
        }
        xf_axpy16(dm[0], w.wm[0] + q * 16, v, false);
        xf_axpy16(dm[1], w.wm[1] + q * 16, v, true);
        xf_axpy16(dm[2], w.wm[2] + q * 16, v, true);
        if (ok) store16_grad(df1, ii * 64 + q * 16, v, f32);
        const float dq2 = dg2 * sg2 * (1.f - sg2);
        float du[9], dg1 = 0.f;
#pragma unroll
        for (int k = 0; k < 9; ++k) {
            const float dd = go_d[k] + dq2 * w.a2[k];
            sg[3 + k] += dd;
            sg[14 + k] = fmaf(dq2, d[k], sg[14 + k]);
            dg1 = fmaf(dd, u[k], dg1);
            du[k] = dd * g1;
        }
#pragma unroll
        for (int k = 0; k < 9; ++k) xf_axpy16(du[k], w.wd[k] + q * 16, v, k != 0);
        if (ok) store16_grad(df2, ii * 64 + q * 16, v, f32);
        const float dsg1 = dg1 * sg1 * (1.f - sg1);
        const float dpt = go_p + dsg1 * w.a1;
        sg[12] += dpt;
        sg[13] = fmaf(dsg1, pt, sg[13]);
        xf_axpy16(dpt, w.wp + q * 16, v, false);
        if (ok) {
            store16_grad(df3, ii * 64 + q * 16, v, f32);
            float4 cf;
            if (q == 0) cf = make_float4(dpt, du[0], du[1], du[2]);
            else if (q == 1) cf = make_float4(du[3], du[4], du[5], du[6]);
            else if (q == 2) cf = make_float4(du[7], du[8], dm[0], dm[1]);
            else cf = make_float4(dm[2], 0.f, 0.f, 0.f);
            reinterpret_cast<float4 *>(coef + ii * 16)[q] = cf;
        }
    }
    if (q == 0) {
#pragma unroll
        for (int j = 0; j < 23; ++j) s_red[tid >> 2][j] = sg[j];
    }
    __syncthreads();
    if (tid < 23) {
        float s = 0.f;
        for (int k = 0; k < 64; ++k) s += s_red[k][tid];
        int dst;
        if (tid < 3) dst = 832 + 10 + tid;
        else if (tid < 12) dst = 832 + 1 + (tid - 3);
        else if (tid == 12) dst = 832;
        else if (tid == 13) dst = 832 + 13;
        else dst = 832 + 14 + (tid - 14);
        partial[(size_t)blockIdx.x * HEADW_FLOATS + dst] = s;
    }
}

template <int FM>
__global__ __launch_bounds__(256) void dam_head_wgrad_kernel(HeadFeat f1, HeadFeat f2, HeadFeat f3, const float *__restrict__ coef,
                                                             int N, int plane, float *__restrict__ partial) {
    __shared__ float s_sc[3][64], s_sh[3][64];
    __shared__ float s_w[4][13][64];
    const int tid = threadIdx.x;
    if (tid < 64) {
        const HeadFeat *fs[3] = {&f1, &f2, &f3};
#pragma unroll
        for (int k = 0; k < 3; ++k) {
            s_sc[k][tid] = fs[k]->scale ? fs[k]->scale[tid] : 1.f;
            s_sh[k][tid] = fs[k]->scale ? fs[k]->shift[tid] : 0.f;
        }
    }
    __syncthreads();
    float gw[13][8];
#pragma unroll
    for (int j = 0; j < 13; ++j)
#pragma unroll
        for (int q = 0; q < 8; ++q) gw[j][q] = 0.f;
    const int c8 = (tid & 7) * 8, pg = tid >> 3;
    const size_t total = (size_t)N * plane;
    for (size_t ip = (size_t)blockIdx.x * 32 + pg; ip < total; ip += (size_t)gridDim.x * 32) {
        const float4 *cr = reinterpret_cast<const float4 *>(coef + ip * 16);
        const float4 c0 = cr[0], c1 = cr[1], c2 = cr[2], c3 = cr[3];
        const float cf[13] = {c0.x, c0.y, c0.z, c0.w, c1.x, c1.y, c1.z, c1.w, c2.x, c2.y, c2.z, c2.w, c3.x};
        float x[8];
        FeatRaw8 R3, R2, R1;
        constexpr bool all16 = FM != 2;
        if (all16) { load_raw8<FM>(f3, ip, c8, R3); load_raw8<FM>(f2, ip, c8, R2); load_raw8<FM>(f1, ip, c8, R1); }
        if (all16) feat_from_raw8<FM>(f3, R3, c8, s_sc[2], s_sh[2], x);
        else feat8(f3, ip, c8, s_sc[2], s_sh[2], x);
#pragma unroll
        for (int q = 0; q < 8; ++q) gw[0][q] = fmaf(cf[0], x[q], gw[0][q]);
        if (all16) feat_from_raw8<FM>(f2, R2, c8, s_sc[1], s_sh[1], x);
        else feat8(f2, ip, c8, s_sc[1], s_sh[1], x);
#pragma unroll
        for (int j = 0; j < 9; ++j)
#pragma unroll
            for (int q = 0; q < 8; ++q) gw[1 + j][q] = fmaf(cf[1 + j], x[q], gw[1 + j][q]);
        if (all16) feat_from_raw8<FM>(f1, R1, c8, s_sc[0], s_sh[0], x);
        else feat8(f1, ip, c8, s_sc[0], s_sh[0], x);
#pragma unroll
        for (int j = 0; j < 3; ++j)
#pragma unroll
            for (int q = 0; q < 8; ++q) gw[10 + j][q] = fmaf(cf[10 + j], x[q], gw[10 + j][q]);
    }
#pragma unroll
    for (int j = 0; j < 13; ++j)
#pragma unroll
        for (int q = 0; q < 8; ++q) {
            float t = gw[j][q];
            t += __shfl_xor(t, 8); t += __shfl_xor(t, 16); t += __shfl_xor(t, 32);
            gw[j][q] = t;
        }
    if ((tid & 63) < 8) {
#pragma unroll
        for (int j = 0; j < 13; ++j)
#pragma unroll
            for (int q = 0; q < 8; ++q) s_w[tid >> 6][j][c8 + q] = gw[j][q];
    }
    __syncthreads();
    float *o = partial + (size_t)blockIdx.x * HEADW_FLOATS;
    for (int idx = tid; idx < 13 * 64; idx += 256) {
        const int row = idx / 64, cc = idx % 64;
        o[idx] = (s_w[0][row][cc] + s_w[1][row][cc]) + (s_w[2][row][cc] + s_w[3][row][cc]);
    }
}

constexpr int HEAD_FUSED_BLOCKS = 1024;
constexpr int HF_ROW = 68;

template <int R0>
__device__ __forceinline__ void head_wgrad_rows(float (&gw)[7][8], const float *cfrow, const float *f3p, const float *f2p, const float *f1p) {
    const float4 *cr = reinterpret_cast<const float4 *>(cfrow);
    const float4 c0 = cr[0], c1 = cr[1], c2 = cr[2], c3 = cr[3];
    const float cf[16] = {c0.x, c0.y, c0.z, c0.w, c1.x, c1.y, c1.z, c1.w, c2.x, c2.y, c2.z, c2.w, c3.x, c3.y, c3.z, c3.w};
    float x3[8], x2[8], x1[8];
    if (R0 == 0) ldf8(f3p, 0, x3);
    ldf8(f2p, 0, x2);
    if (R0 != 0) ldf8(f1p, 0, x1);
#pragma unroll
    for (int r = 0; r < 7; ++r) {
        const int row = R0 + r;
        if (row >= 13) continue;
#pragma unroll
        for (int k = 0; k < 8; ++k) {
            const float x = row == 0 ? x3[k] : row < 10 ? x2[k] : x1[k];
            gw[r][k] = fmaf(cf[row], x, gw[r][k]);
        }
    }
}

__global__ __launch_bounds__(512)
void dam_head_bwd_fused_kernel(const float *__restrict__ f1, const float *__restrict__ f2, const float *__restrict__ f3,
                               const HeadW *__restrict__ hw, const float *__restrict__ dmask, const float *__restrict__ dpoint,
                               const float *__restrict__ ddir, int N, int plane, float *__restrict__ df1, float *__restrict__ df2,
                               float *__restrict__ dz3, float *__restrict__ partial, float *__restrict__ sgbuf) {
    __shared__ HeadW w;
    __shared__ __attribute__((aligned(16))) float s_cf[128 * 16];
    __shared__ __attribute__((aligned(16))) float s_f[3][128 * HF_ROW];
    __shared__ float s_sg[64 * 4][12];
    const int tid = threadIdx.x;
    {
        const float *src = reinterpret_cast<const float *>(hw);
        float *dst = reinterpret_cast<float *>(&w);
        for (int i = tid; i < HEADW_FLOATS; i += 512) dst[i] = src[i];
    }
    __syncthreads();
    const unsigned total = (unsigned)N * (unsigned)plane;
    const int q = tid & 3, slot = tid >> 2;
    const int sh = slot >> 5, sj = slot & 31;
    const int c8 = (tid & 7) * 8, pg = (tid & 255) >> 3, rs = tid >> 8;
    float sgq[6];
#pragma unroll
    for (int j = 0; j < 6; ++j) sgq[j] = 0.f;
    float gw[7][8];
#pragma unroll
    for (int j = 0; j < 7; ++j)
#pragma unroll
        for (int k = 0; k < 8; ++k) gw[j][k] = 0.f;
    for (unsigned base = blockIdx.x * 32; base < total; base += 4 * 32768) {
        const unsigned i = base + sj + sh * 32768;
        const bool ok = i < total;
        const unsigned ii = ok ? i : total - 1;
        const unsigned n = ii / (unsigned)plane, p = ii - n * (unsigned)plane;
        asm volatile("" ::: "memory");
        float F3[16], F2[16], F1[16], v[16];
        const unsigned e = ii * 64 + q * 16;
        ldf8(f3, e, F3); ldf8(f3, e + 8, F3 + 8);
        ldf8(f2, e, F2); ldf8(f2, e + 8, F2 + 8);
        ldf8(f1, e, F1); ldf8(f1, e + 8, F1 + 8);
        float go_m[3], go_d[9], go_p;
#pragma unroll
        for (int k = 0; k < 3; ++k) go_m[k] = dmask[(n * 3 + k) * plane + p];
#pragma unroll
        for (int k = 0; k < 9; ++k) go_d[k] = ddir[(n * 9 + k) * plane + p];
        go_p = dpoint[n * plane + p];
#pragma unroll
        for (int k = 0; k < 3; ++k) go_m[k] = ok ? go_m[k] : 0.f;
#pragma unroll
        for (int k = 0; k < 9; ++k) go_d[k] = ok ? go_d[k] : 0.f;
        go_p = ok ? go_p : 0.f;
        auto stage = [&](const float *F, int k) {
            float *dst = s_f[k] + slot * HF_ROW + q * 16;
#pragma unroll
            for (int h = 0; h < 4; ++h) *reinterpret_cast<float4 *>(dst + 4 * h) = make_float4(F[4 * h], F[4 * h + 1], F[4 * h + 2], F[4 * h + 3]);
        };
        __syncthreads();
        const float pt = xf_quad_sum(xf_dot16(w.wp + q * 16, F3)) + w.bp;
        unsigned pos3 = 0;
#pragma unroll
        for (int j = 0; j < 16; ++j) pos3 |= F3[j] > 0.f ? 1u << j : 0u;
        stage(F3, 0);
        __builtin_amdgcn_sched_barrier(0);
        const float sg1 = 1.f / (1.f + expf(-(w.a1 * pt)));
        const float g1 = 1.f + sg1;
        float u[9], d[9], q2 = 0.f;
#pragma unroll
        for (int k = 0; k < 9; ++k) {
            u[k] = xf_quad_sum(xf_dot16(w.wd[k] + q * 16, F2));
            d[k] = fmaf(g1, u[k], w.bd[k]);
            q2 = fmaf(w.a2[k], d[k], q2);
        }
        stage(F2, 1);
        __builtin_amdgcn_sched_barrier(0);
        const float sg2 = 1.f / (1.f + expf(-q2));
        const float g2 = 1.f + sg2;
        float dm[3], dg2 = 0.f;
#pragma unroll
        for (int k = 0; k < 3; ++k) {
            const float mk = xf_quad_sum(xf_dot16(w.wm[k] + q * 16, F1));
            const float go = go_m[k];
            dg2 = fmaf(go, mk, dg2);
            dm[k] = go * g2;
        }
        stage(F1, 2);
        __builtin_amdgcn_sched_barrier(0);
        xf_axpy16(dm[0], w.wm[0] + q * 16, v, false);
        xf_axpy16(dm[1], w.wm[1] + q * 16, v, true);
        xf_axpy16(dm[2], w.wm[2] + q * 16, v, true);
        if (ok) { stf8(df1, e, v); stf8(df1, e + 8, v + 8); }
        __builtin_amdgcn_sched_barrier(0);
        const float dq2 = dg2 * sg2 * (1.f - sg2);
        float du[9], dd[9], dg1 = 0.f;
#pragma unroll
        for (int k = 0; k < 9; ++k) {
            dd[k] = go_d[k] + dq2 * w.a2[k];
            dg1 = fmaf(dd[k], u[k], dg1);
            du[k] = dd[k] * g1;
        }
#pragma unroll
        for (int k = 0; k < 9; ++k) xf_axpy16(du[k], w.wd[k] + q * 16, v, k != 0);
        if (ok) { stf8(df2, e, v); stf8(df2, e + 8, v + 8); }
        __builtin_amdgcn_sched_barrier(0);
        const float dsg1 = dg1 * sg1 * (1.f - sg1);
        const float dpt = go_p + dsg1 * w.a1;
        float sx[6], sy[6];
        {
            float tx[24], ty[24];
#pragma unroll
            for (int j = 0; j < 3; ++j) { tx[j] = go_m[j]; ty[j] = 1.f; }
#pragma unroll
            for (int j = 0; j < 9; ++j) { tx[3 + j] = dd[j]; ty[3 + j] = 1.f; tx[14 + j] = dq2; ty[14 + j] = d[j]; }
            tx[12] = dpt; ty[12] = 1.f; tx[13] = dsg1; ty[13] = pt; tx[23] = 0.f; ty[23] = 0.f;
#pragma unroll
            for (int s = 0; s < 6; ++s) {
                sx[s] = q == 0 ? tx[4 * s] : q == 1 ? tx[4 * s + 1] : q == 2 ? tx[4 * s + 2] : tx[4 * s + 3];
                sy[s] = q == 0 ? ty[4 * s] : q == 1 ? ty[4 * s + 1] : q == 2 ? ty[4 * s + 2] : ty[4 * s + 3];
            }
        }
        if (sh < 2) {
#pragma unroll
            for (int s = 0; s < 6; ++s) sgq[s] = fmaf(sx[s], sy[s], sgq[s]);
        } else {
#pragma unroll
            for (int s = 0; s < 6; ++s) { s_sg[tid - 256][s] = sx[s]; s_sg[tid - 256][6 + s] = sy[s]; }
        }
        xf_axpy16(dpt, w.wp + q * 16, v, false);
#pragma unroll
        for (int j = 0; j < 16; ++j) v[j] = (pos3 >> j & 1) ? v[j] : 0.f;
        if (ok) { stf8(dz3, e, v); stf8(dz3, e + 8, v + 8); }
        __builtin_amdgcn_sched_barrier(0);
        {
            float4 cf;
            if (q == 0) cf = make_float4(dpt, du[0], du[1], du[2]);
            else if (q == 1) cf = make_float4(du[3], du[4], du[5], du[6]);
            else if (q == 2) cf = make_float4(du[7], du[8], dm[0], dm[1]);
            else cf = make_float4(dm[2], 0.f, 0.f, 0.f);
            *reinterpret_cast<float4 *>(s_cf + slot * 16 + q * 4) = cf;
        }
        __syncthreads();
        if (sh < 2) {
#pragma unroll
            for (int s = 0; s < 6; ++s) sgq[s] = fmaf(s_sg[tid][s], s_sg[tid][6 + s], sgq[s]);
        }
#pragma unroll 1
        for (int h = 0; h < 4; ++h) {
            if (base + pg + h * 32768 < total) {
                const int s = h * 32 + pg;
                if (rs == 0) head_wgrad_rows<0>(gw, s_cf + s * 16, s_f[0] + s * HF_ROW + c8, s_f[1] + s * HF_ROW + c8, s_f[2] + s * HF_ROW + c8);
                else head_wgrad_rows<7>(gw, s_cf + s * 16, s_f[0] + s * HF_ROW + c8, s_f[1] + s * HF_ROW + c8, s_f[2] + s * HF_ROW + c8);
            }
        }
    }
    if (sh < 2) {
        float *o = sgbuf + ((size_t)((blockIdx.x >> 1) + 512 * sh) * 64 + 32 * (blockIdx.x & 1) + sj) * 24;
#pragma unroll
        for (int s = 0; s < 6; ++s) o[4 * s + q] = sgq[s];
    }
#pragma unroll
    for (int j = 0; j < 7; ++j)
#pragma unroll
        for (int k = 0; k < 8; ++k) {
            float t = gw[j][k];
            t += __shfl_xor(t, 8); t += __shfl_xor(t, 16); t += __shfl_xor(t, 32);
            gw[j][k] = t;
        }
    __syncthreads();
    float *s_w = s_f[0];
    if ((tid & 63) < 8) {
#pragma unroll
        for (int j = 0; j < 7; ++j)
            if (rs * 7 + j < 13) {
#pragma unroll
                for (int k = 0; k < 8; ++k) s_w[((((tid & 255) >> 6) * 13) + rs * 7 + j) * 64 + c8 + k] = gw[j][k];
            }
    }
    __syncthreads();
    float *o = partial + (size_t)blockIdx.x * HEADW_FLOATS;
    for (int idx = tid; idx < 13 * 64; idx += 512) o[idx] = (s_w[idx] + s_w[832 + idx]) + (s_w[2 * 832 + idx] + s_w[3 * 832 + idx]);
}

__global__ __launch_bounds__(64) void head_scalar_reduce_kernel(const float *__restrict__ sgbuf, float *__restrict__ partial) {
    const int tid = threadIdx.x;
    if (tid < 23) {
        const float *sg = sgbuf + (size_t)blockIdx.x * 64 * 24;
        float s = 0.f;
        for (int k = 0; k < 64; ++k) s += sg[k * 24 + tid];
        int dst;
        if (tid < 3) dst = 832 + 10 + tid;
        else if (tid < 12) dst = 832 + 1 + (tid - 3);
        else if (tid == 12) dst = 832;
        else if (tid == 13) dst = 832 + 13;
        else dst = 832 + 14 + (tid - 14);
        partial[(size_t)blockIdx.x * HEADW_FLOATS + dst] = s;
    }
}

constexpr int FC_KMAX = 4;
constexpr int FC_KWIDE = 12;
constexpr int FC_KMOST = 20;

template <int KM, int LPP>
__global__ __launch_bounds__(256) void final_conv_bwd_kernel(HeadFeat f, const float *__restrict__ w, const float *__restrict__ dl,
                                                             int K, int N, int plane, unsigned short *__restrict__ df,
                                                             float *__restrict__ partial) {
    constexpr int CH = 64 / LPP, PPB = 256 / LPP, ROW = KM * 64 + KM;
    static_assert(CH == 16 || CH == 8, "16 or 8 channels per lane");
    __shared__ float s_w[KM * 64], s_sc[64], s_sh[64];
    __shared__ float s_red[4][ROW];
    const int tid = threadIdx.x, lane = tid & 63, wave = tid >> 6;
    for (int i = tid; i < K * 64; i += 256) s_w[i] = w[i];
    if (tid < 64) { s_sc[tid] = f.scale ? f.scale[tid] : 1.f; s_sh[tid] = f.scale ? f.shift[tid] : 0.f; }
    __syncthreads();
    const int q = tid % LPP;
    float gw[KM][CH], gb[KM];
#pragma unroll
    for (int k = 0; k < KM; ++k) {
        gb[k] = 0.f;
#pragma unroll
        for (int c = 0; c < CH; ++c) gw[k][c] = 0.f;
    }
    const size_t total = (size_t)N * plane;
    for (size_t base = (size_t)blockIdx.x * PPB; base < total; base += (size_t)gridDim.x * PPB) {
        const size_t i = base + (tid / LPP);
        const bool ok = i < total;
        const size_t ii = ok ? i : total - 1;
        const size_t n = ii / plane, p = ii - n * plane;
        float v[CH], d[KM];
        if (CH == 16) feat16(f, ii, q, s_sc, s_sh, v);
        else feat8(f, ii, q * 8, s_sc, s_sh, v);
#pragma unroll
        for (int k = 0; k < KM; ++k) d[k] = (ok && k < K) ? dl[(n * K + k) * plane + p] : 0.f;
        float o[CH];
#pragma unroll
        for (int c = 0; c < CH; ++c) {
            float t = 0.f;
#pragma unroll
            for (int k = 0; k < KM; ++k) {
                t = fmaf(d[k], s_w[(k < K ? k : 0) * 64 + q * CH + c], t);
                gw[k][c] = fmaf(d[k], v[c], gw[k][c]);
            }
            o[c] = t;
        }
#pragma unroll
        for (int k = 0; k < KM; ++k) gb[k] += d[k];
        if (ok) {
            if (CH == 16) store16_grad(df, ii * 64 + q * 16, o, f.f16 == 2);
            else if (f.f16 == 2) stf8(df, ii * 64 + q * 8, o);
            else {
                V16 ov;
#pragma unroll
                for (int j = 0; j < 8; ++j) ov.h[j] = f2bf(o[j]);
                *reinterpret_cast<uint4 *>(df + ii * 64 + q * 8) = ov.u;
            }
        }
    }
#pragma unroll
    for (int k = 0; k < KM; ++k) {
#pragma unroll
        for (int c = 0; c < CH; ++c) {
            float t = gw[k][c];
#pragma unroll
            for (int m = LPP; m < 64; m <<= 1) t += __shfl_xor(t, m);
            if (lane < LPP) s_red[wave][k * 64 + lane * CH + c] = t;
        }
        float t = gb[k];
#pragma unroll
        for (int m = LPP; m < 64; m <<= 1) t += __shfl_xor(t, m);
        if (lane == 0) s_red[wave][KM * 64 + k] = t;
    }
    __syncthreads();
    for (int j = tid; j < ROW; j += 256)
        partial[(size_t)blockIdx.x * ROW + j] = (s_red[0][j] + s_red[1][j]) + (s_red[2][j] + s_red[3][j]);
}

__global__ void final_conv_scatter_kernel(const float *__restrict__ sums, int K, int KM, float *__restrict__ dw, float *__restrict__ db) {
    const int t = threadIdx.x + blockIdx.x * blockDim.x;
    if (t < K * 64) dw[t] = sums[t];
    if (t < K) db[t] = sums[KM * 64 + t];
}

template <bool F32>
__global__ __launch_bounds__(256) void bias_grad_kernel(const unsigned short *__restrict__ g, unsigned npix, int C,
                                                        float *__restrict__ partial) {
    __shared__ float s_red[256][9];
    const int VPP = C / 8, tid = threadIdx.x;
    const int slot = tid % VPP;
    float acc[8];
#pragma unroll
    for (int j = 0; j < 8; ++j) acc[j] = 0.f;
    const unsigned ppb = 256 / VPP;
    for (unsigned p = first_pixel(ppb, VPP); p < npix; p += gridDim.x * ppb) {
        if (F32) {
            float t[8];
            ldf8(g, (size_t)p * C + slot * 8, t);
#pragma unroll
            for (int j = 0; j < 8; ++j) acc[j] += t[j];
        } else {
            V16 v;
            v.u = *reinterpret_cast<const uint4 *>(g + (size_t)p * C + slot * 8);
#pragma unroll
            for (int j = 0; j < 8; ++j) acc[j] += bf2f(v.h[j]);
        }
    }
#pragma unroll
    for (int j = 0; j < 8; ++j) s_red[tid][j] = acc[j];
    __syncthreads();
    for (int q = tid; q < C; q += 256) {
        const int sl = q / 8, j = q % 8;
        float t = 0.f;
        for (int k = sl; k < 256; k += VPP) t += s_red[k][j];
        partial[(size_t)blockIdx.x * C + q] = t;
    }
}

}

extern "C" int cdnet_dam_head_backward(const cdnet_head_feat *f1, const cdnet_head_feat *f2, const cdnet_head_feat *f3,
                                       const float *head_weights, const float *dmask, const float *dpoint, const float *ddir,
                                       int N, int H, int W, uint16_t *df1, uint16_t *df2, uint16_t *df3, float *workspace,
                                       size_t workspace_floats, float *dhead_weights, void *stream) {
    CDNET_REQUIRE(f1 && f2 && f3 && head_weights && dmask && dpoint && ddir && df1 && df2 && df3 && workspace && dhead_weights,
                  "cdnet_dam_head_backward: null pointer");
    const size_t total = (size_t)N * H * W;
    const int nb = 1024;
    const size_t need = (size_t)nb * HEADW_FLOATS + total * 16;
    if (workspace_floats < need) { set_error("cdnet_dam_head_backward: workspace %zu < %zu floats", workspace_floats, need); return CDNET_E_WORKSPACE; }
    hipStream_t st = (hipStream_t)stream;
    float *partial = workspace, *coef = workspace + (size_t)nb * HEADW_FLOATS;
    const HeadFeat a = mk_hf(*f1), b = mk_hf(*f2), c = mk_hf(*f3);
    auto plain = [](const HeadFeat &f) { return f.f16 == 0 && !f.scale && !f.relu && !f.res; };
    auto train = [](const HeadFeat &f) { return f.f16 == 1 && f.scale && f.relu && f.res; };
    const HeadW *hw = reinterpret_cast<const HeadW *>(head_weights);
    if (plain(a) && plain(b) && plain(c)) {
        dam_head_bwd_kernel<0><<<nb, 256, 0, st>>>(a, b, c, hw, dmask, dpoint, ddir, N, H * W, df1, df2, df3, coef, partial);
        dam_head_wgrad_kernel<0><<<nb, 256, 0, st>>>(a, b, c, coef, N, H * W, partial);
    } else if (train(a) && train(b) && train(c)) {
        dam_head_bwd_kernel<1><<<nb, 256, 0, st>>>(a, b, c, hw, dmask, dpoint, ddir, N, H * W, df1, df2, df3, coef, partial);
        dam_head_wgrad_kernel<1><<<nb, 256, 0, st>>>(a, b, c, coef, N, H * W, partial);
    } else {
        dam_head_bwd_kernel<2><<<nb, 256, 0, st>>>(a, b, c, hw, dmask, dpoint, ddir, N, H * W, df1, df2, df3, coef, partial);
        dam_head_wgrad_kernel<2><<<nb, 256, 0, st>>>(a, b, c, coef, N, H * W, partial);
    }
    reduce_partials_kernel<<<cdiv(HEADW_FLOATS, 4), 256, 0, st>>>(workspace, nb, HEADW_FLOATS, dhead_weights);
    return check_launch("cdnet_dam_head_backward");
}

extern "C" size_t cdnet_dam_head_backward_workspace_floats(int N, int H, int W) {
    return (size_t)1024 * HEADW_FLOATS + (size_t)N * H * W * 16;
}

extern "C" int cdnet_dam_head_backward_fused_blocks(void) { return HEAD_FUSED_BLOCKS; }
extern "C" int cdnet_dam_head_backward_fused_scratch_bytes(void) {
    hipFuncAttributes at;
    if (hipFuncGetAttributes(&at, reinterpret_cast<const void *>(dam_head_bwd_fused_kernel)) != hipSuccess) return -1;
    return (int)at.localSizeBytes;
}
extern "C" size_t cdnet_dam_head_backward_fused_workspace_floats(void) { return (size_t)HEAD_FUSED_BLOCKS * (HEADW_FLOATS + 64 * 24); }

extern "C" int cdnet_dam_head_backward_fused(const cdnet_head_feat *f1, const cdnet_head_feat *f2, const cdnet_head_feat *f3,
                                             const float *head_weights, const float *dmask, const float *dpoint, const float *ddir,
                                             int N, int H, int W, float *df1, float *df2, float *dz3, float *workspace,
                                             size_t workspace_floats, float *dhead_weights, void *stream) {
    CDNET_REQUIRE(f1 && f2 && f3 && head_weights && dmask && dpoint && ddir && df1 && df2 && dz3 && workspace && dhead_weights,
                  "cdnet_dam_head_backward_fused: null pointer");
    auto plain32 = [](const cdnet_head_feat &f) { return f.raw && f.f16 == 2 && !f.scale && !f.shift && !f.relu && !f.res; };
    CDNET_REQUIRE(plain32(*f1) && plain32(*f2) && plain32(*f3),
                  "cdnet_dam_head_backward_fused: plain stored fp32 features only (f16 = 2, no scale / shift / relu / res)");
    CDNET_REQUIRE(N >= 1 && H >= 1 && W >= 1, "cdnet_dam_head_backward_fused: N=%d H=%d W=%d", N, H, W);
    CDNET_REQUIRE((size_t)N * H * W * 64 < ((size_t)1 << 32), "cdnet_dam_head_backward_fused: tensor too large for 32-bit element indexing");
    static_assert(HEAD_FUSED_BLOCKS == 1024, "the chains of the two-kernel path: 1024 workgroups");
    const int nb = HEAD_FUSED_BLOCKS;
    const size_t need = (size_t)nb * (HEADW_FLOATS + 64 * 24);
    if (workspace_floats < need) { set_error("cdnet_dam_head_backward_fused: workspace %zu < %zu floats", workspace_floats, need); return CDNET_E_WORKSPACE; }
    hipStream_t st = (hipStream_t)stream;
    float *partial = workspace, *sgbuf = workspace + (size_t)nb * HEADW_FLOATS;
    auto fp = [](const cdnet_head_feat &f) { return reinterpret_cast<const float *>(f.raw); };
    dam_head_bwd_fused_kernel<<<nb, 512, 0, st>>>(fp(*f1), fp(*f2), fp(*f3), reinterpret_cast<const HeadW *>(head_weights), dmask, dpoint, ddir,
                                                  N, H * W, df1, df2, dz3, partial, sgbuf);
    head_scalar_reduce_kernel<<<nb, 64, 0, st>>>(sgbuf, partial);
    reduce_partials_kernel<<<cdiv(HEADW_FLOATS, 4), 256, 0, st>>>(workspace, nb, HEADW_FLOATS, dhead_weights);
    return check_launch("cdnet_dam_head_backward_fused");
}

extern "C" size_t cdnet_final_conv1x1_backward_workspace_floats(void) { return (size_t)1025 * (FC_KMOST * 64 + FC_KMOST); }

extern "C" int cdnet_final_conv1x1_backward(const cdnet_head_feat *f, const float *w, const float *dlogits, int K, int N, int H, int W,
                                            uint16_t *df, float *workspace, size_t workspace_floats, float *dw, float *db, void *stream) {
    CDNET_REQUIRE(f && f->raw && w && dlogits && df && workspace && dw && db, "cdnet_final_conv1x1_backward: null pointer");
    CDNET_REQUIRE(K >= 1 && K <= FC_KMOST && N > 0 && H > 0 && W > 0, "cdnet_final_conv1x1_backward: K=%d must be in [1,%d]", K, FC_KMOST);
    if (workspace_floats < cdnet_final_conv1x1_backward_workspace_floats()) { set_error("cdnet_final_conv1x1_backward: workspace too small"); return CDNET_E_WORKSPACE; }
    hipStream_t st = (hipStream_t)stream;
    const size_t npix = (size_t)N * H * W;
    const bool wide = K > FC_KMAX;
    const bool most = K > FC_KWIDE;
    const int KM = most ? FC_KMOST : wide ? FC_KWIDE : FC_KMAX;
    int nb = (int)((npix + (wide ? 31 : 63)) / (wide ? 32 : 64));
    if (nb > 1024) nb = 1024;
    const int ROW = KM * 64 + KM;
    float *sums = workspace + (size_t)1024 * ROW;
    if (most) final_conv_bwd_kernel<FC_KMOST, 8><<<nb, 256, 0, st>>>(mk_hf(*f), w, dlogits, K, N, H * W, df, workspace);
    else if (wide) final_conv_bwd_kernel<FC_KWIDE, 8><<<nb, 256, 0, st>>>(mk_hf(*f), w, dlogits, K, N, H * W, df, workspace);
    else final_conv_bwd_kernel<FC_KMAX, 4><<<nb, 256, 0, st>>>(mk_hf(*f), w, dlogits, K, N, H * W, df, workspace);
    reduce_partials_kernel<<<cdiv(ROW, 4), 256, 0, st>>>(workspace, nb, ROW, sums);
    final_conv_scatter_kernel<<<cdiv(K * 64, 256), 256, 0, st>>>(sums, K, KM, dw, db);
    return check_launch("cdnet_final_conv1x1_backward");
}

extern "C" size_t cdnet_bias_grad_workspace_floats(int C) { return (size_t)512 * C; }

static int bias_grad_impl(const uint16_t *grad_out, size_t npix, int C, float *workspace, size_t workspace_floats, float *db, void *stream, bool f32);
extern "C" int cdnet_bias_grad(const uint16_t *grad_out, size_t npix, int C, float *workspace, size_t workspace_floats, float *db,
                               void *stream) {
    return bias_grad_impl(grad_out, npix, C, workspace, workspace_floats, db, stream, false);
}
extern "C" int cdnet_bias_grad_f32(const float *grad_out, size_t npix, int C, float *workspace, size_t workspace_floats, float *db,
                                   void *stream) {
    return bias_grad_impl(reinterpret_cast<const uint16_t *>(grad_out), npix, C, workspace, workspace_floats, db, stream, true);
}
static int bias_grad_impl(const uint16_t *grad_out, size_t npix, int C, float *workspace, size_t workspace_floats, float *db, void *stream, bool f32) {
    CDNET_REQUIRE(grad_out && workspace && db, "cdnet_bias_grad: null pointer");
    CDNET_REQUIRE(C >= 8 && C % 8 == 0 && C <= 2048 && npix > 0 && npix < ((size_t)1 << 31), "cdnet_bias_grad: C=%d unsupported", C);
    if (workspace_floats < cdnet_bias_grad_workspace_floats(C)) { set_error("cdnet_bias_grad: workspace too small"); return CDNET_E_WORKSPACE; }
    hipStream_t st = (hipStream_t)stream;
    const unsigned ppb = 256 / (C / 8);
    int nb = (int)((npix + ppb * 8 - 1) / (ppb * 8));
    if (nb > 512) nb = 512;
    if (nb < 1) nb = 1;
    if (f32) bias_grad_kernel<true><<<nb, 256, 0, st>>>(grad_out, (unsigned)npix, C, workspace);
    else bias_grad_kernel<false><<<nb, 256, 0, st>>>(grad_out, (unsigned)npix, C, workspace);
    reduce_partials_kernel<<<cdiv(C, 4), 256, 0, st>>>(workspace, nb, C, db);
    return check_launch("cdnet_bias_grad");
}
```

cdnet_amd/trainer.py:

```python
import ctypes as C
import os

import torch

from . import _lib, engine, optim, runtime, streams
from ._lib import BnBwdArgs, GradIn, GradTerm
from .allreduce import BucketReducer, bucketed_allreduce
from .engine import Src
from .optim import HEAD_PARAMS, FlatState
from .synth import synthetic_batch


_WGRAD_WGS_DEEP, _WGRAD_WGS_SHALLOW = 128, 160
_WGRAD_WGS_KQ = 128
_WGRAD_WGS_F32 = 160
_RU_1X1_SIDE = True
WGRAD_STREAM = True
HEAD_BWD_FUSE = True
_WGRAD_DEFER = 0x100
_WGRAD_DEEP_HW = 16384


class _on_stream:
    __slots__ = ('s', 'prev')

    def __init__(self, s):
        self.s = s

    def __enter__(self):
        self.prev = torch.cuda.current_stream()
        torch.cuda.set_stream(self.s)

    def __exit__(self, *exc):
        torch.cuda.set_stream(self.prev)
        return False


class _G:
    __slots__ = ('t', 'Hg', 'Wg', 'oy', 'ox', 'pooled', 'coff', 'cstride', 'event', 'masked')

    def __init__(self, t, Hg, Wg, oy=0, ox=0, pooled=0, coff=0, cstride=0):
        self.t, self.Hg, self.Wg, self.oy, self.ox, self.pooled, self.coff, self.cstride = t, Hg, Wg, oy, ox, pooled, coff, cstride
        self.event = None
        self.masked = False


def _choose_ci_tiles(C_src, Cout):
    if Cout <= 32 and runtime.PRECISION != 'fp32':
        return 1
    best, best_cost = 2, None
    for ci_t in (2, 1, 4):
        CI, CO = ci_t * 32, (4 // ci_t) * 32
        cost = -(-C_src // CI) * CI * -(-Cout // CO) * CO
        if best_cost is None or cost < best_cost:
            best, best_cost = ci_t, cost
    return best


def _wgrad_wgs(beside, HW, Cout):
    if not beside:
        return 256
    if runtime.PRECISION == 'fp32':
        return _WGRAD_WGS_F32
    if Cout <= 32 and HW > 65536:
        return _WGRAD_WGS_KQ
    return _WGRAD_WGS_DEEP if HW <= _WGRAD_DEEP_HW or HW > 65536 else _WGRAD_WGS_SHALLOW


class Trainer:
    def __init__(self, model, lr=1e-3, weight_decay=1e-4, betas=(0.9, 0.99), eps=None, quirk_sample0=True,
                 world_size=1, bucket_mb=25, optimizer='adam', momentum=0.95):
        self.model = model
        self._pack_jobs = None
        self._pack_prec = None
        self._ar = None
        self.optimizer = str(optimizer).lower()
        if self.optimizer not in optim.OPTIMIZERS:
            raise ValueError('Optimizer {} not available (one of {})'.format(optimizer, ', '.join(optim.OPTIMIZERS)))
        if eps is None:
            eps = optim.RANGER_EPS if self.optimizer == 'ranger' else 1e-8
        self.lr, self.wd, self.betas, self.eps, self.momentum = lr, weight_decay, betas, eps, momentum
        self.quirk = int(quirk_sample0)
        self.world = world_size
        self.bucket = int(float(bucket_mb) * (1 << 20) // 4)
        self.flat = FlatState(model, self.optimizer)
        model._head_flat = self.flat.P[:self.flat.n_head] if self.flat.n_head == 855 else None
        self.dev = self.flat.P.device
        self._bufs = {}
        self._wss = {}
        self.losses = torch.zeros((11,), dtype=torch.float32, device=self.dev)
        self.alpha = 0.0
        self.dice, self.weight_map = 1, 1
        self.loss_var = torch.full((1,), -1.0, dtype=torch.float32, device=self.dev)
        self.boundary = 0
        self.loss_boundary = torch.zeros((1,), dtype=torch.float32, device=self.dev)
        self.tape = []
        self._cat_cache = {}
        self._wstream, self._events = None, {}
        self.ar_stats = None
        self._packb_pending = False
        self._packb_stream = True
        self._side_active = False
        self.head_fused = False
        self._rd_mb = float(os.environ.get('CDNET_WGRAD_REDUCE_MB', '300'))
        self._rd_pending, self._rd_params, self._rd_bytes, self._rd_tables = [], [], 0, {}
        self._forwards, self._bn_base = 0, 0
        if world_size > 1:
            self.sync_from_rank0()

    def sync_from_rank0(self, src=0):
        import torch.distributed as dist
        if not (dist.is_available() and dist.is_initialized()) or dist.get_world_size() == 1:
            return
        f = self.flat
        works = [dist.broadcast(t, src=src, async_op=True) for t in (f.P, f.M, f.V, f.S) if t is not None]
        meta = torch.tensor([float(f.step_count), float(self._bn_base + self._forwards)], dtype=torch.float64, device=self.dev)
        works.append(dist.broadcast(meta, src=src, async_op=True))
        bufs = [b for b in self.model.buffers() if b.is_floating_point()]
        if bufs:
            flatb = torch.cat([b.detach().reshape(-1).float() for b in bufs])
            dist.broadcast(flatb, src=src)
            off = 0
            with torch.no_grad():
                for b in bufs:
                    b.copy_(flatb[off:off + b.numel()].view(b.shape))
                    off += b.numel()
        for w in works:
            w.wait()
        f.step_count = int(meta[0].item())
        self._bn_base, self._forwards = int(meta[1].item()), 0
        self.refresh_parameters()

    def reduce_scalars(self, values):
        import torch.distributed as dist
        if self.world <= 1 or not (dist.is_available() and dist.is_initialized()):
            return values
        t = torch.as_tensor(values, dtype=torch.float64).to(self.dev)
        dist.all_reduce(t, op=dist.ReduceOp.SUM)
        return (t / dist.get_world_size()).cpu().numpy()

    def buf(self, key, shape, dtype):
        b = self._bufs.get(key)
        if b is None or tuple(b.shape) != tuple(shape) or b.dtype != dtype:
            b = torch.empty(shape, dtype=dtype, device=self.dev)
            self._bufs[key] = b
        return b

    def _ws(self, name, need, side=False):
        ws = self._wss.get(name)
        if ws is None or ws.numel() < need:
            if side and self._wstream is not None:
                self._wstream.synchronize()
            ws = self._wss[name] = torch.empty((need,), dtype=torch.float32, device=self.dev)
        return ws

    def grad_sum(self, gl, mask, npix, Cc, out):
        assert 1 <= len(gl) <= 6
        arr = (GradTerm * len(gl))()
        for k, g in enumerate(gl):
            assert not g.pooled and g.oy == 0 and g.ox == 0
            arr[k].g, arr[k].cstride, arr[k].coff = g.t.data_ptr(), g.cstride or Cc, g.coff
        _lib.call(_lib.entry('cdnet_grad_sum', out.dtype == torch.float32), C.byref(arr), len(gl), None if mask is None else _lib.ptr(mask),
                  npix, Cc, _lib.ptr(out), _lib.stream_ptr())

    def take(self, grads, key):
        gl = grads.pop(key, None)
        if gl is not None:
            for g_ in gl:
                if g_.event is not None:
                    torch.cuda.current_stream().wait_event(g_.event)
                    g_.event = None
        return gl

    def cat_grad(self, o, grads):
        key = id(o)
        if key not in self._cat_cache:
            gl = self.take(grads, key)
            if gl is None:
                d = None
            elif len(gl) == 1 and not gl[0].coff and gl[0].cstride in (0, o.shape[3]):
                d = gl[0].t
            else:
                d = self.buf(('dcat', key), o.shape, runtime.act_dtype())
                self.grad_sum(gl, None, o.shape[0] * o.shape[1] * o.shape[2], o.shape[3], d)
            self._cat_cache[key] = d
        return self._cat_cache[key]

    def forward(self, x):
        m = self.model
        m.train()
        self._forwards += 1
        runtime.TAPE = self.tape
        del self.tape[:]
        try:
            out = m(x)
        finally:
            runtime.TAPE = None
        return out

    def loss_and_grads(self, mask, point, direction, label, dirlab, point_t, weight):
        B, _, H, W = mask.shape
        lib = _lib.load()
        ND = direction.shape[1]
        ws = self._ws('loss', lib.cdnet_dam_loss_classes_workspace_floats(B, H * W, ND))
        dmask = self.buf('dmask', mask.shape, torch.float32)
        dpoint = self.buf('dpoint', point.shape, torch.float32)
        ddir = self.buf('ddir', direction.shape, torch.float32)
        assert label.dtype == torch.uint8 and dirlab.dtype == torch.uint8 and weight.dtype == torch.uint8
        assert point_t.dtype == torch.float16
        if self.dice != 1:
            raise ValueError('dice = %r with a DAM model: the reference dies on an unbound loss_direction_dice (train_util_dam.py:297); only 1 works'
                             % (self.dice,))
        from .utils import loss_terms
        terms = loss_terms(self.dice, self.weight_map, self.alpha)
        args = (_lib.ptr(mask), _lib.ptr(point), _lib.ptr(direction), _lib.ptr(label.contiguous()),
                _lib.ptr(dirlab.contiguous()), _lib.ptr(point_t.contiguous()), _lib.ptr(weight.contiguous()), B, H, W, ND,
                self.quirk, _lib.ptr(ws), ws.numel(), _lib.ptr(self.losses), _lib.ptr(dmask),
                _lib.ptr(dpoint), _lib.ptr(ddir), _lib.stream_ptr())
        if terms == 7:
            _lib.call('cdnet_dam_loss_classes', *args)
        else:
            _lib.call('cdnet_dam_loss_terms', *args, terms)
        if self.alpha:
            self._variance_term(mask, label, dmask)
        if self.boundary:
            self._boundary_term(mask, label, dmask)
        return dmask, dpoint, ddir

    def _variance_term(self, mask, label, dmask, total=None):
        if self.alpha not in (1, 2):
            raise ValueError('alpha = %r: the variance term is built for alpha = 1 and 2 (0 switches it off)' % (self.alpha,))
        B, K, H, W = mask.shape
        need = _lib.load().cdnet_variance_loss_workspace_bytes(B, K, H, W)
        ws = self._ws('variance', (need + 3) // 4)
        total = self.losses[0:1] if total is None else total
        _lib.call('cdnet_variance_loss', _lib.ptr(mask), _lib.ptr(label.contiguous()), 1, B, K, H, W, float(self.alpha), _lib.ptr(ws),
                  ws.numel() * 4, _lib.ptr(self.loss_var), None if dmask is None else _lib.ptr(total), None if dmask is None else _lib.ptr(dmask),
                  None, None, _lib.stream_ptr())

    def _boundary_term(self, mask, label, dmask, total=None):
        if self.boundary not in (1, 2, 3):
            raise ValueError('boundary = %r: 1 (BoundaryLoss), 2 (FocalLoss2d) or 3 (RobustFocalLoss2d); 0 switches the term off' % (self.boundary,))
        B, K, H, W = mask.shape
        need = _lib.load().cdnet_boundary_loss_workspace_bytes(self.boundary, B, K, H, W)
        if need == 0:
            raise ValueError('the boundary term serves three-class mask logits, got %s' % (tuple(mask.shape),))
        ws = self._ws('boundary', (need + 3) // 4)
        total = self.losses[0:1] if total is None else total
        _lib.call('cdnet_boundary_loss', _lib.ptr(mask), _lib.ptr(label.contiguous()), self.boundary, B, K, H, W, 1.0, _lib.ptr(ws),
                  ws.numel() * 4, _lib.ptr(self.loss_boundary), _lib.ptr(total), _lib.ptr(dmask), _lib.stream_ptr())

    def backward(self, dmask, dpoint, ddir):
        m = self.model
        f1, f2, f3 = m._last_feats
        N, H, W, _ = f1.x.shape
        df = [self.buf('dF%d' % k, (N, H, W, 64), runtime.act_dtype()) for k in range(3)]
        hf = [runtime.head_feat(f) for f in (f1, f2, f3)]
        dhead = self.flat.G[:self.flat.n_head]
        owner = self._head_fusable(f1, f2, f3)
        self.head_fused = owner is not None
        if owner is not None:
            ws = self._ws('head', _lib.load().cdnet_dam_head_backward_fused_workspace_floats())
            _lib.call('cdnet_dam_head_backward_fused', C.byref(hf[0]), C.byref(hf[1]), C.byref(hf[2]), _lib.ptr(m.head_weight_block()),
                      _lib.ptr(dmask), _lib.ptr(dpoint), _lib.ptr(ddir), N, H, W, _lib.ptr(df[0]), _lib.ptr(df[1]), _lib.ptr(df[2]),
                      _lib.ptr(ws), ws.numel(), _lib.ptr(dhead), _lib.stream_ptr())
            heads = [(f.x, _G(d, H, W)) for f, d in zip((f1, f2, f3), df)]
            heads[2][1].masked = True
            self._run_tape(heads, None)
            return
        ws = self._ws('head', _lib.load().cdnet_dam_head_backward_workspace_floats(N, H, W))
        _lib.call('cdnet_dam_head_backward', C.byref(hf[0]), C.byref(hf[1]), C.byref(hf[2]), _lib.ptr(m.head_weight_block()),
                  _lib.ptr(dmask), _lib.ptr(dpoint), _lib.ptr(ddir), N, H, W, _lib.ptr(df[0]), _lib.ptr(df[1]),
                  _lib.ptr(df[2]), _lib.ptr(ws), ws.numel(), _lib.ptr(dhead), _lib.stream_ptr())
        self._run_tape([((f.grad_to or (f.x,))[0], _G(d, H, W)) for f, d in zip((f1, f2, f3), df)], None)

    def _head_fusable(self, f1, f2, f3):
        if not HEAD_BWD_FUSE or runtime.PRECISION != 'fp32' or getattr(self.model, 'VARIANT', None) != 'rev1':
            return None
        for f in (f1, f2, f3):
            if f.x.dtype != torch.float32 or f.scale is not None or f.shift is not None or f.res is not None or f.relu or f.pool \
                    or f.grad_to is not None or tuple(f.off) != (0, 0) or f.C != 64:
                return None
        owner = None
        for Rt in self.tape:
            if isinstance(Rt, runtime.FuseRecord):
                if any(t.x is f3.x for t in Rt.terms):
                    return None
                continue
            if any(sx.x is f3.x or sx.res is f3.x for sx in Rt.srcs):
                return None
            if Rt.out is f3.x:
                owner = Rt.fused_res_of if Rt.layer.kind == 'conv1' else None
        if owner is None or owner.layer.bn is None or owner.relu != 2 or owner.res is not f3.x \
                or owner.out.dtype != torch.float32 or tuple(owner.out.shape) != tuple(f3.x.shape):
            return None
        return owner

    def _classifier_backward(self, key, f, conv, dl):
        N, H, W, _ = f.x.shape
        K = conv.out_channels
        df = self.buf(key, (N, H, W, 64), runtime.act_dtype())
        ws = self._ws('slab', _lib.load().cdnet_final_conv1x1_backward_workspace_floats(), side=True)
        hf = runtime.head_feat(f)
        w = conv.weight.detach().reshape(K, 64)
        _lib.call('cdnet_final_conv1x1_backward', C.byref(hf), _lib.ptr(w), _lib.ptr(dl), K, N, H, W, _lib.ptr(df), _lib.ptr(ws),
                  ws.numel(), _lib.ptr(conv.weight.grad), _lib.ptr(conv.bias.grad), _lib.stream_ptr())
        return _G(df, H, W)

    def _run_tape(self, heads, params):
        grads = {}

        def add(t, g):
            grads.setdefault(id(t), []).append(g)
        for t, g in heads:
            add(t, g)
        self._overlap_begin()
        self._overlap_done(params)
        self._backward_tape(grads, add)

    def _backward_tape(self, grads, add):
        self._cat_cache = {}
        self._rd_pending, self._rd_params, self._rd_bytes = [], [], 0
        if len(self._rd_tables) > 16:
            self._rd_tables.clear()
        self._readers, self._producer, self._bn_partials = {}, {}, {}
        self._tape_pos = {Rt: k for k, Rt in enumerate(self.tape)}
        for Rt in self.tape:
            if isinstance(Rt, runtime.FuseRecord):
                for t in Rt.terms:
                    self._readers[id(t.x)] = self._readers.get(id(t.x), 0) + 1
                continue
            for sx in Rt.srcs:
                self._readers[id(sx.x)] = self._readers.get(id(sx.x), 0) + 1
                if sx.res is not None:
                    self._readers[id(sx.res)] = self._readers.get(id(sx.res), 0) + 1
            self._producer[id(Rt.out)] = Rt
        side = self._side_stream()
        self._side_active = side is not None
        if self._packb_pending:
            torch.cuda.current_stream().wait_event(self._event('packb'))
            self._packb_pending = False
        for k, R in enumerate(reversed(self.tape)):
            if isinstance(R, runtime.FuseRecord):
                self._fuse_backward(R, grads, add)
                continue
            gl = self.take(grads, id(R.out))
            if gl is None:
                continue
            owner = R.fused_res_of
            if owner is not None:
                grads.setdefault(id(owner.out), []).extend(gl)
                owner.deferred = R
                continue
            self._layer_backward(k, R, gl, grads, add, side)
            d = R.deferred
            if d is not None:
                R.deferred = None
                self._layer_backward(('deferred', k), d, self.take(grads, id(d.out)), grads, add, side)
        if side is not None:
            with _on_stream(side):
                self._flush_reduces()
            ev = self._event(-1)
            ev.record(side)
            torch.cuda.current_stream().wait_event(ev)
        else:
            self._flush_reduces()

    def _fuse_backward(self, R, grads, add):
        terms, o, relu, H, W, Cc, coff, name = R.terms, R.out, R.relu, R.H, R.W, R.C, R.coff, R.node.name
        sliced = o.shape[3] != Cc
        if sliced:
            d, dcs, dco = self.cat_grad(o, grads), o.shape[3], coff
            if d is None:
                return
        else:
            gl = self.take(grads, id(o))
            if gl is None:
                return
            if relu and self._residual_tail(grads, gl, terms, o, H, W, Cc):
                return
            if relu or len(gl) > 1 or gl[0].coff or gl[0].cstride not in (0, Cc):
                d = self.buf(('dfuse', name), o.shape, o.dtype)
                self.grad_sum(gl, o if relu else None, o.shape[0] * H * W, Cc, d)
            else:
                d = gl[0].t
            dcs, dco = 0, 0
        N = o.shape[0]
        for k, t in enumerate(terms):
            if t.Hs == H and t.Ws == W:
                add(t.x, _G(d, H, W, coff=dco, cstride=dcs))
            else:
                din = self.buf(('dup', name, k), (N, t.Hs, t.Ws, Cc), d.dtype)
                _lib.call(_lib.entry('cdnet_upsample_bilinear_backward', d.dtype == torch.float32), _lib.ptr(d),
                          N, H, W, Cc, dcs, dco, t.Hs, t.Ws, _lib.ptr(din), _lib.stream_ptr())
                add(t.x, _G(din, t.Hs, t.Ws))

    def _residual_tail(self, grads, gl, terms, o, H, W, Cc):
        if runtime.DEBUG_NORELU:
            return False
        if len(terms) == 1:
            y = terms[0]
            P = self._producer.get(id(y.x)) if y.scale is not None else None
            if P is None or P.layer.bn is None or P.res is not None or self._readers.get(id(y.x), 0) != 1 or id(y.x) in grads \
                    or tuple(y.x.shape) != tuple(o.shape) or P.fused_res_of is not None or (y.Hs, y.Ws) != (H, W):
                return False
            P.relu, P.res = True, None
            grads[id(y.x)] = gl
            return True
        if len(terms) != 2 or len(gl) > 3:
            return False
        bn_t = [t for t in terms if t.scale is not None]
        if not bn_t or any((t.Hs, t.Ws) != (H, W) for t in terms):
            return False
        y = max(bn_t, key=lambda t: self._tape_pos.get(self._producer.get(id(t.x)), -1))
        x = terms[1] if terms[0] is y else terms[0]
        P = self._producer.get(id(y.x))
        if P is None or P.layer.bn is None or P.res is not None or self._readers.get(id(y.x), 0) != 1 or id(y.x) in grads \
                or tuple(y.x.shape) != tuple(o.shape) or P.fused_res_of is not None:
            return False
        if any(g.pooled or g.oy or g.ox or (g.Hg, g.Wg) != (H, W) for g in gl):
            return False
        P.relu, P.res, P.res_grad_to = 2, o, x.x
        grads[id(y.x)] = gl
        return True

    def _weights_done(self, params):
        if not self._rd_pending:
            self._overlap_done(params)
            return
        self._rd_params.append(params)
        if self._rd_bytes >= self._rd_mb * (1 << 20):
            self._flush_reduces()

    def _flush_reduces(self):
        if self._rd_pending:
            key = tuple(self._rd_pending)
            tab = self._rd_tables.get(key)
            if tab is None:
                lib = _lib.load()
                descs = (_lib.WgradReduceDesc * len(key))()
                b0 = 0
                for i, a in enumerate(key):
                    _lib.call('cdnet_wgrad_reduce_desc_fill', *a, b0, C.byref(descs[i]))
                    b0 += descs[i].blocks
                dev_tab = torch.frombuffer(bytearray(bytes(descs)), dtype=torch.uint8).to(self.dev)
                tab = self._rd_tables[key] = (dev_tab, len(key), b0)
            _lib.call('cdnet_wgrad_reduce_batch', _lib.ptr(tab[0]), tab[1], tab[2], _lib.stream_ptr())
        for params in self._rd_params:
            self._overlap_done(params)
        self._rd_pending, self._rd_params, self._rd_bytes = [], [], 0

    def _layer_backward(self, k, R, gl, grads, add, side):
        L, srcs, out, Hl, Wl = R.layer, R.srcs, R.out, R.H, R.W
        No, Ho, Wo, Co = out.shape
        params = (L.weight, L.bias, None if L.bn is None else L.bn.weight, None if L.bn is None else L.bn.bias)
        part = self._bn_partials.pop(id(out), None)
        if len(gl) == 1 and gl[0].masked:
            g = self._bn_backward_masked(R, out, gl[0], add)
        elif part is not None:
            assert len(gl) == 1, (L.name, len(gl))
            a, ktab = self._bn_backward_stats(L, out, gl[0], partial=part)
            g = self.buf(('draw', L.name), (No, Ho, Wo, Co), runtime.act_dtype())
            _lib.call('cdnet_bn_backward_apply', C.byref(a), _lib.ptr(ktab), _lib.ptr(g), _lib.stream_ptr())
        elif L.bn is not None or len(gl) > 1 or gl[0].pooled or gl[0].coff or (gl[0].cstride not in (0, Co)):
            g = self._bn_backward(R, out, gl, add)
        else:
            g = gl[0].t
        if side is None:
            self._weight_backward(L, srcs, g, Hl, Wl)
            self._weights_done(params)
            self._input_backward(L, srcs, g, Hl, Wl, add)
        else:
            ev = self._event(k)
            ev.record()
            beside = _RU_1X1_SIDE and L.kind == 'conv1' and isinstance(k, tuple) and L.needs_input_grad
            if not beside:
                self._input_backward(L, srcs, g, Hl, Wl, add)
            side.wait_event(ev)
            with _on_stream(side):
                if beside:
                    ev2 = self._event(('beside', k))

                    def add_beside(tgt, g_):
                        g_.event = ev2
                        add(tgt, g_)
                    self._input_backward(L, srcs, g, Hl, Wl, add_beside)
                    ev2.record()
                self._weight_backward(L, srcs, g, Hl, Wl)
                self._weights_done(params)

    def _bn_backward_stats(self, L, out, g, partial):
        a = self._bn_args(L, out, [_G(g.t, g.Hg, g.Wg)], res=None, relu=1)
        ktab = self.buf(('ktab', L.name), (7, out.shape[3]), torch.float32)
        bn = L.bn
        _lib.call('cdnet_bn_backward_finalize', C.byref(a), _lib.ptr(bn.weight.detach()), _lib.ptr(bn.weight.grad), _lib.ptr(bn.bias.grad),
                  _lib.ptr(partial), partial.shape[0], _lib.ptr(ktab), _lib.stream_ptr())
        return a, ktab

    def _bn_backward_masked(self, R, out, g, add):
        L = R.layer
        No, Ho, Wo, Co = out.shape
        a = self._bn_args(L, out, [_G(g.t, g.Hg, g.Wg)], res=None, relu=0)
        draw = self.buf(('draw', L.name), (No, Ho, Wo, Co), runtime.act_dtype())
        ws = self._ws('bn', _lib.load().cdnet_bn_backward_workspace_floats(Co))
        bn = L.bn
        _lib.call('cdnet_bn_backward', C.byref(a), _lib.ptr(bn.weight.detach()), _lib.ptr(bn.weight.grad), _lib.ptr(bn.bias.grad),
                  _lib.ptr(ws), ws.numel(), _lib.ptr(draw), None, _lib.stream_ptr())
        add(R.res, _G(g.t, Ho, Wo))
        return draw

    def _stats_fusable(self, L, srcs, H, W, N, wpb, cfgb, cin_total):
        f32 = runtime.PRECISION == 'fp32'
        if not f32 or os.environ.get('CDNET_BN_STATS_FUSE', '1') != '1' or runtime.DEBUG_NORELU:
            return None
        if L.kind != 'conv3' or L.transposed or len(srcs) != 1:
            return None
        sx = srcs[0]
        if sx.is_input or sx.scale is None or sx.shift is None or sx.relu is not True or sx.res is not None or sx.pool \
                or tuple(sx.off) != (0, 0) or sx.x.dtype != runtime.raw_dtype() or sx.grad_to is not None or sx.row_stride:
            return None
        if f32 and cin_total % 64:
            return None
        PR = self._producer.get(id(sx.x))
        if PR is None or PR.layer.bn is None or PR.res is not None or PR.relu is not True \
                or self._readers.get(id(sx.x), 0) != 1 or tuple(sx.x.shape) != (N, H, W, cin_total):
            return None
        P = PR.layer
        key = ('statsfusable', L.name, N, H, W, runtime.PRECISION)
        hit = self._bufs.get(key)
        if hit is None:
            part = torch.zeros((1024, 2, cin_total), dtype=torch.float32, device=self.dev)
            gin = self.buf(('din', L.name), (N, H, W, cin_total), runtime.act_dtype())
            gdummy = self.buf(('draw', L.name), (N, H, W, L.Cout), runtime.act_dtype())
            ok = engine.conv_forward([Src(gdummy)], wpb, cin_total, cfgb, taps=L.taps, out=gin, H=H, W=W, query_ws=True,
                                     bns=(sx.x, P.scale, P.shift, P.save_mean, P.save_invstd, part))
            hit = self._bufs[key] = (part if ok else False)
        if hit is False:
            return None
        return P, hit

    def _bn_args(self, L, out, gl, res, relu):
        a = BnBwdArgs()
        a.raw = out.data_ptr()
        a.res = None if res is None else res.data_ptr()
        if L.bn is not None:
            a.scale, a.shift = L.scale.data_ptr(), L.shift.data_ptr()
            a.mean, a.invstd = L.save_mean.data_ptr(), L.save_invstd.data_ptr()
        a.ngin = len(gl)
        assert 1 <= len(gl) <= 3, (L.name, len(gl))
        for k, g in enumerate(gl):
            a.gin[k].g = g.t.data_ptr()
            a.gin[k].Hg, a.gin[k].Wg, a.gin[k].oy, a.gin[k].ox = g.Hg, g.Wg, g.oy, g.ox
            a.gin[k].pooled, a.gin[k].coff, a.gin[k].cstride = int(g.pooled), g.coff, g.cstride or out.shape[3]
        a.f16 = {torch.bfloat16: 0, torch.float16: 1, torch.float32: 2}[out.dtype]
        a.relu = relu
        a.N, a.H, a.W, a.C = out.shape
        return a

    def _bn_backward(self, R, out, gl, add):
        L = R.layer
        No, Ho, Wo, Co = out.shape
        res = R.res
        has_bn = L.bn is not None
        if len(gl) > 3:
            plain = [g for g in gl if not g.pooled and g.oy == 0 and g.ox == 0 and (g.Hg, g.Wg) == (Ho, Wo)]
            rest = [g for g in gl if g not in plain]
            assert len(rest) <= 2 and len(plain) >= 2, (L.name, len(gl))
            d = self.buf(('gsum', L.name), (No, Ho, Wo, Co), runtime.act_dtype())
            self.grad_sum(plain, None, No * Ho * Wo, Co, d)
            gl = rest + [_G(d, Ho, Wo)]
        a = self._bn_args(L, out, gl, res, int(R.relu))
        draw = self.buf(('draw', L.name), (No, Ho, Wo, Co), runtime.act_dtype())
        dz = None
        if res is not None:
            dz = self.buf(('dz', L.name), (No, Ho, Wo, Co), runtime.act_dtype())
        ws = self._ws('bn', _lib.load().cdnet_bn_backward_workspace_floats(Co))
        bn = L.bn
        _lib.call('cdnet_bn_backward', C.byref(a), _lib.ptr(bn.weight.detach()) if has_bn else None,
                  _lib.ptr(bn.weight.grad) if has_bn else None, _lib.ptr(bn.bias.grad) if has_bn else None,
                  _lib.ptr(ws), ws.numel(), _lib.ptr(draw), _lib.ptr(dz), _lib.stream_ptr())
        if res is not None:
            add(R.res_grad_to if R.res_grad_to is not None else res, _G(dz, Ho, Wo))
            R.res_grad_to = None
        return draw

    def _side_stream(self):
        if not WGRAD_STREAM or self.dev.type != 'cuda':
            return None
        if self._wstream is None:
            self._wstream = streams.side_stream(self.dev)
            self._events = {}
        return self._wstream

    def _event(self, k):
        e = self._events.get(k)
        if e is None:
            e = self._events[k] = torch.cuda.Event()
        return e

    def _weight_backward(self, L, srcs, g, H, W):
        lib = _lib.load()
        N = g.shape[0]
        Cout = L.Cout
        cin_total = sum(s.C for s in srcs)
        cin_real = L.Cin
        mode = {'conv3': 0, 'conv1': 0, 'convT4': 2, 'convT2': 3, 'conv3s2': 6}[L.kind]
        taps, npar, ostride = L.taps, (4 if L.transposed else 1), (2 if L.transposed else 1)
        cap = _wgrad_wgs(self._side_active and L.needs_input_grad, H * W, Cout)
        coff = 0
        for s in srcs:
            ci_t = _choose_ci_tiles(s.C, Cout)
            CI, CO = ci_t * 32, (4 // ci_t) * 32
            other = -(-s.C // CI) * -(-Cout // CO) * npar
            ntiles = N * (-(-H // 8)) * (-(-W // 16))
            ksplit = max(1, min(ntiles, cap // other if other < cap else 1))
            nslab = lib.cdnet_conv_wgrad_slab_floats(s.C, Cout, taps, npar, ci_t, ksplit)
            defer = self._rd_mb > 0
            slab = self.buf(('wslab', L.name, coff), (nslab,), torch.float32) if defer else self._ws('slab', nslab, side=True)
            cs = engine.ConvSrc()
            s.fill(cs)
            csrc_real = min(s.C, cin_real - coff) if cin_total != cin_real else s.C
            _lib.call('cdnet_conv_backward_weight', C.byref(cs), coff, csrc_real, cin_real, _lib.ptr(g), Cout, N, H, W, taps,
                      npar, ostride, ci_t, ksplit, _lib.ptr(slab), _lib.ptr(L.weight.grad), mode | (_WGRAD_DEFER if defer else 0),
                      _lib.stream_ptr())
            if defer:
                self._rd_pending.append((s.C, coff, csrc_real, cin_real, Cout, taps, npar, ci_t, ksplit, slab.data_ptr(),
                                         L.weight.grad.data_ptr(), mode))
                self._rd_bytes += nslab * 4
            coff += s.C
        if L.bias is not None and L.bn is None:
            owner = L.bias_grad_from
            if owner is not None:
                L.bias.grad.copy_(owner.bn.bias.grad)
            else:
                ws = self._ws('slab', lib.cdnet_bias_grad_workspace_floats(Cout), side=True)
                _lib.call(_lib.entry('cdnet_bias_grad', g.dtype == torch.float32), _lib.ptr(g), g.numel() // Cout, Cout,
                          _lib.ptr(ws), ws.numel(), _lib.ptr(L.bias.grad), _lib.stream_ptr())

    def _input_backward(self, L, srcs, g, H, W, add):
        if not L.needs_input_grad:
            return
        N = g.N if isinstance(g, Src) else g.shape[0]
        Cout = L.Cout
        cin_total = sum(s.C for s in srcs)
        wpb, cfgb = L.backward_pack(cin_total, H, W)
        if L.kind == 'conv3s2':
            Cp = cin_total // 4
            gs2d = self.buf(('ds2d', L.name), (N, H, W, cin_total), runtime.act_dtype())
            engine.conv_forward([Src(g)], wpb, cin_total, cfgb, taps=9, out=gs2d, H=H, W=W)
            gin = self.buf(('din', L.name), (N, 2 * H, 2 * W, Cp), runtime.act_dtype())
            _lib.call(_lib.entry('cdnet_s2d_to_nhwc', gin.dtype == torch.float32), _lib.ptr(gs2d), N, H, W, Cp, _lib.ptr(gin),
                      _lib.stream_ptr())
            add(srcs[0].x, _G(gin, 2 * H, 2 * W))
            return
        if not L.transposed:
            gin = self.buf(('din', L.name), (N, H, W, cin_total), runtime.act_dtype())
            fuse = None if isinstance(g, Src) else self._stats_fusable(L, srcs, H, W, N, wpb, cfgb, cin_total)
            if fuse is not None:
                P, part = fuse
                engine.conv_forward([Src(g)], wpb, cin_total, cfgb, taps=L.taps, out=gin, H=H, W=W,
                                    bns=(srcs[0].x, P.scale, P.shift, P.save_mean, P.save_invstd, part))
                self._bn_partials[id(srcs[0].x)] = part
            else:
                engine.conv_forward([g if isinstance(g, Src) else Src(g)], wpb, cin_total, cfgb, taps=L.taps, out=gin, H=H, W=W)
        else:
            gin = self.buf(('din', L.name), (N, H, W, cin_total), runtime.act_dtype())
            views = [Src(g, view=(a * 2 * W * Cout, H, W, 2 * Cout, 4 * W * Cout)) for a in (0, 1)]
            engine.conv_forward(views, wpb, cin_total, cfgb, taps=(9 if L.kind == 'convT4' else 1), out=gin, H=H, W=W)
        coff = 0
        for s in srcs:
            if s.is_input:
                coff += s.C
                continue
            tgt, pool = s.grad_to or (s.x, int(s.pool))
            add(tgt, _G(gin, H, W, oy=s.off[0], ox=s.off[1], pooled=pool, coff=coff, cstride=cin_total))
            coff += s.C

    def _overlap_begin(self):
        self._ar = None
        if not self._reduce_active() or os.environ.get('CDNET_ALLREDUCE_OVERLAP', '1') == '0':
            return
        f = self.flat
        base = f.G.data_ptr()
        pend = {}
        owners = [p for L in (R.layer for R in self.tape if not isinstance(R, runtime.FuseRecord)) for p in (L.weight, L.bias, None if L.bn is None else L.bn.weight,
                                                 None if L.bn is None else L.bn.bias) if p is not None]
        for p in owners:
            off = (p.grad.data_ptr() - base) // 4
            if 0 <= off < f.n_used:
                pend[off] = off + p.numel()
        if f.n_head:
            pend[0] = f.n_head
        self._ar = BucketReducer(f.G, f.n_used, self.bucket, pend)

    def _overlap_done(self, params):
        if self._ar is None:
            return
        if params is None:
            self._ar.done([0])
        else:
            base = self.flat.G.data_ptr()
            self._ar.done([(p.grad.data_ptr() - base) // 4 for p in params if p is not None])

    def _reduce_active(self):
        return self.world > 1 or os.environ.get('CDNET_FORCE_ALLREDUCE', '0') == '1'

    def allreduce_and_step(self):
        f = self.flat
        gscale = 1.0
        works = None
        if self._reduce_active():
            if self._ar is not None:
                ranges = self._ar.finish(wait=False)
                works = self._ar.works
                self.ar_stats = dict(buckets=len(works), released_during_backward=self._ar.early)
                self._ar = None
            else:
                bucketed_allreduce(f.G, f.n_used, self.bucket)
            gscale = 1.0 / self.world
        f.step_count += 1
        step = self._rule_stepper(gscale)
        if works is None:
            step(0, f.n_used)
        else:
            for w, (a, b) in zip(works, ranges):
                w.wait()
                step(a, b)
        runtime.WEIGHTS_EPOCH[0] += 1
        self._repack_all()

    def _rule_stepper(self, gscale):
        return optim.stepper(self, gscale)

    def _repack_all(self):
        f = self.flat
        lo, hi = f.P.data_ptr(), f.P.data_ptr() + f.P.numel() * 4
        if self._pack_jobs is not None and self._pack_prec != runtime.PRECISION:
            self._pack_jobs = None
        if self._pack_jobs is None:
            groups = ([], []), ([], [])
            for L in runtime.LAYERS:
                if not (lo <= L.weight.data_ptr() < hi):
                    continue
                w = L.weight.detach()
                if L.wp is not None and not L.wp_padded:
                    groups[0][0].append(engine.pack_job(w, L.cfg, L.pack_mode, L.wp, split=L.cfg_f32)); groups[0][1].append((L, 'wp_version'))
                if L.wpb is not None:
                    mode = (4 if L.kind == 'convT4' else 5) if L.transposed else (7 if L.kind == 'conv3s2' else 1)
                    groups[1][0].append(engine.pack_job(w, L.cfg_bwd, mode, L.wpb, split=L.cfg_f32)); groups[1][1].append((L, 'wpb_version'))
            if not groups[0][0] or not groups[1][0] or self.flat.step_count < 1:
                return
            self._pack_jobs = []
            self._pack_prec = runtime.PRECISION
            for jobs, owners in groups:
                arr = (engine.PackJob * len(jobs))(*jobs)
                nbytes = _lib.load().cdnet_pack_batch_table_bytes(len(jobs))
                table = torch.empty((nbytes,), dtype=torch.uint8, device=f.P.device)
                self._pack_jobs.append((arr, len(jobs), table, owners, [True]))
        side = self._side_stream()
        for k, (arr, n, table, owners, first) in enumerate(self._pack_jobs):
            if k == 1 and side is not None and self._packb_stream:
                ev = self._event('adam')
                ev.record()
                side.wait_event(ev)
                with _on_stream(side):
                    _lib.call('cdnet_pack_conv_weights_batch', C.byref(arr), n, _lib.ptr(table), table.numel(), int(first[0]), _lib.stream_ptr())
                    self._event('packb').record()
                self._packb_pending = True
            else:
                _lib.call('cdnet_pack_conv_weights_batch', C.byref(arr), n, _lib.ptr(table), table.numel(), int(first[0]), _lib.stream_ptr())
            first[0] = False
            for L, attr in owners:
                setattr(L, attr, (L.weight._version, runtime.WEIGHTS_EPOCH[0]))

    def write_bn_counters(self):
        with torch.no_grad():
            unused = tuple(getattr(self.model, 'UNUSED_PREFIXES', ()))
            for name, mod in self.model.named_modules():
                if isinstance(mod, torch.nn.BatchNorm2d) and mod.num_batches_tracked is not None and not (name + '.').startswith(unused or ('\0',)):
                    mod.num_batches_tracked.fill_(self._bn_base + self._forwards)

    def refresh_parameters(self):
        if hasattr(self.model, 'sync_real_parameters') and getattr(self.model, '_rt', None) is not None:
            self.model._ensure_runtime()
        runtime.WEIGHTS_EPOCH[0] += 1

    def state_dict(self):
        return optim.state_dict(self)

    def load_state_dict(self, sd):
        optim.load_state_dict(self, sd)

    def train_step(self, x, label, dirlab, point_t, weight):
        mask, point, direction = self.forward(x)
        dmask, dpoint, ddir = self.loss_and_grads(mask, point, direction, label, dirlab, point_t, weight)
        self.backward(dmask, dpoint, ddir)
        self.allreduce_and_step()
        return self.losses


class UNetTrainer(Trainer):

    def __init__(self, model, **kw):
        super().__init__(model, **kw)
        self.mask_losses = torch.zeros((8,), dtype=torch.float32, device=self.dev)
        self.unet_losses = self.mask_losses[0:3]
        self.unet_metrics = self.mask_losses[3:8]

    def mask_loss(self, logits, label, weight, terms, dmask):
        B, K, H, W = logits.shape
        if K != 3:
            raise ValueError('the mask loss serves the 3-class configuration (options.py: out_c = 3), got %d classes' % K)
        assert label.dtype == torch.uint8 and (weight is None or weight.dtype == torch.uint8)
        ws = self._ws('mask_loss', _lib.load().cdnet_mask_loss_workspace_floats(B, H * W))
        _lib.call('cdnet_mask_loss', _lib.ptr(logits), _lib.ptr(label.contiguous()), None if weight is None else _lib.ptr(weight.contiguous()),
                  B, H, W, terms, _lib.ptr(ws), ws.numel(), _lib.ptr(self.mask_losses), None if dmask is None else _lib.ptr(dmask),
                  _lib.stream_ptr())

    def loss_and_grads(self, logits, label, weight):
        from .utils import loss_terms
        terms = loss_terms(self.dice, self.weight_map, self.alpha)
        dmask = self.buf('dmask', logits.shape, torch.float32)
        self.mask_loss(logits, label, weight, terms, dmask)
        total = self.mask_losses[0:1]
        if self.dice == 2:
            if self.alpha:
                self._variance_term(logits, label, None)
            return dmask
        if self.alpha:
            self._variance_term(logits, label, dmask, total)
        if self.boundary:
            self._boundary_term(logits, label, dmask, total)
        return dmask

    def backward(self, dlogits):
        conv, feat = self.model.final_conv, self.model._last_feat
        self._run_tape([(feat.x, self._classifier_backward('dF', feat, conv, dlogits))], [conv.weight, conv.bias])

    def train_step(self, x, label, weight):
        logits = self.forward(x)
        dlogits = self.loss_and_grads(logits, label, weight)
        self.backward(dlogits)
        self.allreduce_and_step()
        return self.unet_losses


class BackboneUNetTrainer(UNetTrainer):

    def _classifier_backward(self, key, f, conv, dl):
        N, H, W, _ = f.x.shape
        K = conv.out_channels
        df = self.buf(key, (N, H, W, 16), runtime.act_dtype())
        ws = self._ws('classifier16', _lib.load().cdnet_final_conv1x1_c16_backward_workspace_floats())
        hf = runtime.head_feat16(f)
        w = conv.weight.detach().reshape(K, 16)
        _lib.call('cdnet_final_conv1x1_c16_backward', C.byref(hf), _lib.ptr(w), _lib.ptr(dl), K, N, H, W, _lib.ptr(df), _lib.ptr(ws),
                  ws.numel(), _lib.ptr(conv.weight.grad), _lib.ptr(conv.bias.grad), _lib.stream_ptr())
        return _G(df, H, W)


class FullNetTrainer(UNetTrainer):

    def __init__(self, model, seed=0, **kw):
        if runtime.PRECISION != 'fp32':
            raise NotImplementedError('FullNet trains in the fp32 precision mode only (CDNET_PRECISION=fp32 / runtime.set_precision("fp32")); '
                                      'bf16-mode training is not built')
        super().__init__(model, **kw)
        self.seed = int(seed)

    def dropout_key(self):
        return ((self.seed & 0xffffffff) << 32) | (self.flat.step_count & 0xffffffff)

    def forward(self, x):
        self.model._train_key = self.dropout_key()
        return super().forward(x)

    def backward(self, dlogits):
        self._ar = None
        self.model.train_backward(self.tape[-1], dlogits)


class AblationTrainer(Trainer):

    def __init__(self, model, **kw):
        assert getattr(model, 'VARIANT', 'rev1') in ('MandD', 'MandDandP') and model.DIRECTION_OUT in (5, 9, 17), \
            'AblationTrainer serves model_unet_MandD / MandD4 / MandD16 / MandDandP'
        super().__init__(model, **kw)

    def loss_and_grads(self, outputs, label, dirlab, point_t, weight):
        if len(outputs) == 3:
            return super().loss_and_grads(outputs[0], outputs[1], outputs[2], label, dirlab, point_t, weight)
        mask, direction = outputs
        B, _, H, W = mask.shape
        point = self.buf('zero_point', (B, 1, H, W), torch.float32)
        pt = self.buf('zero_point_t', (B, H, W), torch.float16)
        point.zero_()
        pt.zero_()
        dmask, _, ddir = super().loss_and_grads(mask, point, direction, label, dirlab, pt, weight)
        return dmask, None, ddir

    def backward(self, dmask, dpoint, ddir):
        m = self.model
        f1m, f2, f3 = m._last_feats
        heads, params = [], []
        for name, f, conv, dl in (('m', f1m, m.mask_conv, dmask), ('d', f2, m.direction_conv, ddir), ('p', f3, m.point_conv, dpoint)):
            if f is None or dl is None:
                continue
            heads.append(((f.grad_to or (f.x,))[0], self._classifier_backward('dF' + name, f, conv, dl)))
            params += [conv.weight, conv.bias]
        self._run_tape(heads, params)

    def train_step(self, x, label, dirlab, point_t, weight):
        out = self.forward(x)
        g = self.loss_and_grads(out, label, dirlab, point_t, weight)
        self.backward(*g)
        self.allreduce_and_step()
        return self.losses


def make_bench_step(model, B, dev, rank, world):
    tr = Trainer(model, world_size=world)
    batch = synthetic_batch(B, dev, seed=2022 + rank)

    def step():
        return tr.train_step(*batch)
    metric = 'tiles/sec (train fwd+bwd+Adam), 256x256'
    workload = ('CDNet UNet2RevA1_vgg16 (UNet+DAM) training step: forward, 5-term loss, backward%s, %s fused Adam; '
                '256x256x3 synthetic tiles, batch %d per GPU' % ('', 'RCCL gradient all-reduce,' if world > 1 else '', B))
    return step, metric, workload
```

include/cdnet_hip.h:

```cpp
#ifndef CDNET_HIP_H
#define CDNET_HIP_H

#include <stddef.h>
#include <stdint.h>

#ifdef __cplusplus
extern "C" {
#endif

#define CDNET_OK            0
#define CDNET_E_ARG         1
#define CDNET_E_WORKSPACE   2
#define CDNET_E_LAUNCH      3

#define CDNET_ABI_VERSION   5

int         cdnet_abi_version(void);
size_t      cdnet_abi_sizeof(const char *struct_name);
const char *cdnet_last_error(void);
const char *cdnet_build_info(void);
int         cdnet_spin(int microseconds, void *stream);
int         cdnet_box_copy(const void *src, void *dst, size_t bytes, void *stream);
int         cdnet_box_mfma(const uint32_t *seed, float *sink, unsigned long long *stamps, int workgroups, int waves_per_wg, int iters, void *stream);

size_t cdnet_tile_postproc_workspace_bytes(int B, int C, int H, int W);
int cdnet_tile_postproc(const float *mask_logits, const float *dir_logits, const float *point, int B, int C, int H, int W,
                        const int8_t *lut_host, int nbr, int extra_zero, int min_area, int radius, void *workspace, size_t workspace_bytes,
                        float *prob, uint8_t *dcm, int32_t *minmax, uint8_t *pred, uint8_t *fill, uint8_t *small, int32_t *label,
                        int32_t *final_, int32_t *counts, void *stream);

int cdnet_ddm_codes(const uint8_t *dcm, int N, int H, int W, int classes, const int8_t *lut_host, int nbr,
                    int extra_zero, uint8_t *code, int32_t *minmax, void *stream);
int cdnet_ddm_normalize(const uint8_t *code, const int32_t *minmax, int N, int H, int W, float *out,
                        void *stream);

int cdnet_probmaps(const float *mask_logits, const float *dir_logits, int N, int C, int H, int W,
                   float *prob, uint8_t *dcm, void *stream);

int cdnet_tta_boost_argmax(const float *probs, const float *points, const uint8_t *codes, const int32_t *minmax,
                           int I, int V, const int *view_xform_host, int H, int W,
                           float *prob_mean, float *point_mean, uint8_t *ddm16, uint8_t *pred,
                           float *pmax_ws, void *stream);

size_t cdnet_watershed_workspace_bytes(int N, int H, int W);
int cdnet_watershed_process(const uint8_t *pred, int N, int H, int W, int min_size, void *workspace, size_t workspace_bytes,
                            uint8_t *dist, int32_t *marker, int32_t *labels, void *stream);
int cdnet_fill_label_process(const uint8_t *pred, int N, int H, int W, int min_size, void *workspace, size_t workspace_bytes,
                             int32_t *labels, void *stream);
int cdnet_label_process(const uint8_t *pred, int N, int H, int W, int min_size, void *workspace, size_t workspace_bytes,
                        int32_t *labels, void *stream);

size_t cdnet_instance_redilate_workspace_bytes(int N, int H, int W, int cap);
int cdnet_instance_redilate(const int32_t *label, int N, int H, int W, int r, int cap, void *workspace, size_t workspace_bytes,
                            int32_t *out, int32_t *err_flag, void *stream);
int cdnet_instance_redilate_lds_rows(void);
int cdnet_instance_redilate_lds_cols(void);
int cdnet_label_count(const int32_t *lab, int N, int plane, int cap, int32_t *seen, int32_t *counts, int32_t *err_flag, void *stream);

size_t cdnet_cc_workspace_bytes(int N, int H, int W);
int cdnet_cc_chain(const uint8_t *pred, int fg_value, int N, int H, int W, int min_area, int radius,
                   void *workspace, size_t workspace_bytes,
                   uint8_t *fill, uint8_t *small, int32_t *label, int32_t *final_, int32_t *counts,
                   void *stream);

int cdnet_mask_views_argmax(const float *logits, int I, int V, int K, const int *view_xform_host, int H, int W, float *prob_mean,
                            uint8_t *pred, void *stream);
size_t cdnet_tile_mask_postproc_workspace_bytes(int B, int K, int H, int W);
int cdnet_tile_mask_postproc(const float *logits, int B, int K, int H, int W, int min_area, int radius, void *workspace, size_t workspace_bytes,
                             float *prob, uint8_t *pred, uint8_t *fill, uint8_t *small, int32_t *label, int32_t *final_, int32_t *counts,
                             void *stream);
int cdnet_dilate_labels(const int32_t *label, int N, int H, int W, int radius, int32_t *out, void *stream);


typedef struct cdnet_conv_src {
    const uint16_t *x;
    const uint16_t *res;
    const float *scale;
    const float *shift;
    int C;
    int Hs, Ws;
    int pool;
    int relu;
    int off_y, off_x;
    int f16;
    int row_stride;
} cdnet_conv_src;

typedef struct cdnet_conv_args {
    cdnet_conv_src src[2];
    int nsrc;
    const uint16_t *w;
    const float *bias;
    const float *oscale;
    const float *oshift;
    int orelu;
    uint16_t *out;
    int Cout, out_cstride, out_coff;
    float *stats;
    int N, H, W;
    int taps;
    int npar;
    int ostride;
    int nchunk;
    int tile, CK, BN;
    int out_f16;
    int debug;
    int ws;
    int f32;
    const uint16_t *eres;
    const float *eres_scale, *eres_shift;
    int eres_f16, eres_relu;
    int taps1;
    int pad_;
    uint16_t *pool_out;
    const float *dot_w;
    const float *dot_b;
    float *dot_out;
} cdnet_conv_args;

size_t cdnet_conv_packed_weight_elems(int Cout, int nchunk, int taps, int CK, int BN, int npar);
#define CDNET_PACK_SPLIT 16
int cdnet_pack_conv_weights(const float *w, void *packed, int Cout, int Cin, int KH, int KW, int CK, int BN, int mode,
                            void *stream);
int cdnet_pack_conv_weights_scaled(const float *w, const float *cout_scale, void *packed, int Cout, int Cin, int KH, int KW, int CK,
                                   int BN, int mode, void *stream);
typedef struct cdnet_pack_job {
    const float *w;
    void *packed;
    int Cout, Cin, KH, KW, CK, BN, mode, pad_;
} cdnet_pack_job;
size_t cdnet_pack_batch_table_bytes(int n_jobs);
int cdnet_pack_conv_weights_batch(const cdnet_pack_job *jobs, int n_jobs, void *table, size_t table_bytes, int upload,
                                  void *stream);
int cdnet_conv_forward(const cdnet_conv_args *args, void *stream);

#define CDNET_CONV_FAMILY_FWD    1
#define CDNET_CONV_FAMILY_WS     2
#define CDNET_CONV_FAMILY_WS16   3
#define CDNET_CONV_FAMILY_F32    4
#define CDNET_CONV_FAMILY_STREAM 5
#define CDNET_CONV_FAMILY_WS32   6
int cdnet_conv_forward_last_form(void);

typedef struct cdnet_dilated_conv_args {
    const void *in;
    const void *w;
    const float *scale;
    const float *shift;
    void *out;
    int N, H, W;
    int Cin, in_cstride;
    int Cout, out_cstride, out_coff;
    int taps, dilation;
    int leaky;
    float slope;
    int f32, out_nchw;
} cdnet_dilated_conv_args;
size_t cdnet_dilated_packed_weight_elems(int Cin, int Cout, int taps, int f32);
int cdnet_dilated_pack_weights(const float *w, void *packed, int Cin, int Cout, int taps, int f32, void *stream);
int cdnet_dilated_conv_forward(const cdnet_dilated_conv_args *args, void *stream);


typedef struct cdnet_dilated_bwd_data_args {
    const void *g;
    const void *w;
    void *dx;
    int N, H, W;
    int Cout, g_cstride;
    int Cin, dx_cstride, dx_coff;
    int taps, dilation;
    int accumulate;
    int f32;
} cdnet_dilated_bwd_data_args;
int cdnet_dilated_pack_weights_bwd(const float *w, void *packed, int Cin, int Cout, int taps, int f32, void *stream);
int cdnet_dilated_conv_backward_data(const cdnet_dilated_bwd_data_args *args, void *stream);

typedef struct cdnet_dilated_wgrad_args {
    const float *x;
    const float *g;
    float *dw;
    void *ws;
    size_t ws_bytes;
    int N, H, W;
    int Cin, x_cstride;
    int Cout, g_cstride;
    int taps, dilation;
} cdnet_dilated_wgrad_args;
size_t cdnet_dilated_wgrad_workspace_bytes(int N, int H, int W, int Cin, int Cout, int taps);
int cdnet_dilated_conv_backward_weight(const cdnet_dilated_wgrad_args *args, void *stream);

typedef struct cdnet_slice_bn_fwd_args {
    const float *z;
    float *out;
    const float *gamma, *beta;
    float *running_mean, *running_var;
    float *mean, *invstd;
    float *ws;
    size_t ws_floats;
    long long P;
    int C, z_cstride, out_cstride, out_coff;
    float eps, momentum, p_drop;
    int layer;
    unsigned long long key;
} cdnet_slice_bn_fwd_args;
typedef struct cdnet_slice_bn_bwd_args {
    const float *dy;
    const float *z;
    const float *mean, *invstd, *gamma;
    float *dgamma, *dbeta;
    float *g;
    float *ws;
    size_t ws_floats;
    long long P;
    int C, z_cstride, dy_cstride, dy_coff, g_cstride;
    float slope, p_drop;
    int layer;
    unsigned long long key;
} cdnet_slice_bn_bwd_args;
size_t cdnet_slice_bn_workspace_floats(long long P, int C);
int cdnet_slice_bn_train_forward(const cdnet_slice_bn_fwd_args *args, void *stream);
int cdnet_slice_bn_train_backward(const cdnet_slice_bn_bwd_args *args, void *stream);
int cdnet_dropout_mask(unsigned long long key, int layer, size_t count, float p_drop, uint8_t *mask, void *stream);


int cdnet_maxpool2_forward(const void *x, int x_cstride, void *y, int y_cstride, int y_coff, uint8_t *idx, int idx_cstride, int N, int H, int W,
                           int C, int f32, void *stream);
int cdnet_maxpool2_backward(const float *dy, int dy_cstride, int dy_coff, const uint8_t *idx, int idx_cstride, float *dx, int dx_cstride, int N,
                            int H, int W, int C, void *stream);
int cdnet_upsample4_bilinear_forward(const void *x, int x_cstride, void *y, int y_cstride, int y_coff, int N, int Hs, int Ws, int C, int f32,
                                     void *stream);
int cdnet_upsample4_bilinear_backward(const float *dy, int dy_cstride, int dy_coff, float *dx, int dx_cstride, int N, int Hs, int Ws, int C,
                                      void *stream);

int cdnet_input_pack(const float *x, int N, int C, int H, int W, void *out_bf16_nhwc16, void *stream);
int cdnet_input_pack_f32(const float *x, int N, int C, int H, int W, float *out_f32_nhwc16, void *stream);
int cdnet_bn_fold_eval(const float *gamma, const float *beta, const float *running_mean, const float *running_var,
                       const float *conv_bias, float eps, int C, float *scale, float *shift, void *stream);
int cdnet_bn_finalize_train(const float *stats, int T, int C, float count, const float *gamma, const float *beta,
                            const float *conv_bias, float eps, float momentum, float *running_mean,
                            float *running_var, float *scale, float *shift, float *save_mean, float *save_invstd,
                            void *stream);

typedef struct cdnet_head_feat {
    const uint16_t *raw;
    const uint16_t *res;
    const float *scale;
    const float *shift;
    int relu;
    int f16;
} cdnet_head_feat;

#define CDNET_HEAD_WEIGHT_FLOATS 855
int cdnet_dam_head_forward(const cdnet_head_feat *f1, const cdnet_head_feat *f2, const cdnet_head_feat *f3,
                           const float *head_weights, int N, int H, int W, float *mask, float *point,
                           float *direction, void *stream);
int cdnet_final_conv1x1(const cdnet_head_feat *f, const float *w, const float *b, int K, int N, int H, int W,
                        float *out, void *stream);
size_t cdnet_bias_grad_workspace_floats(int C);
int cdnet_bias_grad(const uint16_t *grad_out, size_t npix, int C, float *workspace, size_t workspace_floats, float *db, void *stream);
int cdnet_bias_grad_f32(const float *grad_out, size_t npix, int C, float *workspace, size_t workspace_floats, float *db, void *stream);
size_t cdnet_final_conv1x1_backward_workspace_floats(void);
int cdnet_final_conv1x1_backward(const cdnet_head_feat *f, const float *w, const float *dlogits, int K, int N, int H, int W,
                                 uint16_t *df, float *workspace, size_t workspace_floats, float *dw, float *db, void *stream);
int cdnet_final_conv1x1_c16(const cdnet_head_feat *f, const float *w, const float *b, int K, int N, int H, int W,
                            float *out, void *stream);
size_t cdnet_final_conv1x1_c16_backward_workspace_floats(void);
int cdnet_final_conv1x1_c16_backward(const cdnet_head_feat *f, const float *w, const float *dlogits, int K, int N, int H, int W,
                                     void *df, float *workspace, size_t workspace_floats, float *dw, float *db, void *stream);

int cdnet_conv_ws_eligible(const cdnet_conv_args *args);

int cdnet_src_materialize(const cdnet_conv_src *src, int N, int H, int W, uint16_t *out, void *stream);

size_t cdnet_conv_wgrad_slab_floats(int C_src, int Cout, int taps, int npar, int ci_tiles, int ksplit);
int cdnet_conv_backward_weight(const cdnet_conv_src *src, int src_coff, int Csrc_real, int Cin_real,
                               const uint16_t *grad_out, int Cout, int N, int H, int W, int taps, int npar,
                               int ostride, int ci_tiles, int ksplit, float *slab, float *dw, int mode, void *stream);

#define CDNET_WGRAD_FAMILY_GEN  1
#define CDNET_WGRAD_FAMILY_WS   2
#define CDNET_WGRAD_FAMILY_F32  3
#define CDNET_WGRAD_FAMILY_WS32 4
int cdnet_conv_backward_weight_last_form(void);

#define CDNET_WGRAD_DEFER_REDUCE 0x100
typedef struct cdnet_wgrad_reduce_desc {
    const float *slab;
    float *dw;
    int ksplit, npar, ci_blocks, co_blocks, taps, CI, CO, Csrc_real, Cin_real, src_coff, Cout, mode;
    int block0, blocks;
} cdnet_wgrad_reduce_desc;
int cdnet_wgrad_reduce_desc_fill(int C_src, int src_coff, int Csrc_real, int Cin_real, int Cout, int taps, int npar, int ci_tiles,
                                 int ksplit, const float *slab, float *dw, int mode, int block0, cdnet_wgrad_reduce_desc *out);
int cdnet_wgrad_reduce_batch(const cdnet_wgrad_reduce_desc *table_dev, int n, int total_blocks, void *stream);

typedef struct cdnet_grad_in {
    const uint16_t *g;
    int Hg, Wg;
    int oy, ox;
    int pooled;
    int coff, cstride;
    int pad_;
} cdnet_grad_in;

typedef struct cdnet_bn_bwd_args {
    const uint16_t *raw;
    const uint16_t *res;
    const float *scale, *shift;
    const float *mean, *invstd;
    cdnet_grad_in gin[3];
    int ngin;
    int f16, relu;
    int N, H, W, C;
} cdnet_bn_bwd_args;

size_t cdnet_bn_backward_workspace_floats(int C);
int cdnet_bn_backward_stats(const cdnet_bn_bwd_args *args, const float *gamma, float *dgamma, float *dbeta, float *workspace,
                            size_t workspace_floats, float *ktab, void *stream);
int cdnet_bn_backward_apply(const cdnet_bn_bwd_args *args, const float *ktab, uint16_t *draw, void *stream);
int cdnet_bn_backward_finalize(const cdnet_bn_bwd_args *args, const float *gamma, float *dgamma, float *dbeta, const float *partial,
                               int nb, float *ktab, void *stream);
int cdnet_bn_backward(const cdnet_bn_bwd_args *args, const float *gamma, float *dgamma, float *dbeta, float *workspace,
                      size_t workspace_floats, uint16_t *draw, uint16_t *dz_out, void *stream);

#define CDNET_BN_PATH_WINDOW  1
#define CDNET_BN_PATH_FLAT    2
#define CDNET_BN_PATH_GENERIC 3
int cdnet_bn_backward_last_plan(void);
int cdnet_bn_backward_last_sums_plan(void);

size_t cdnet_dam_head_backward_workspace_floats(int N, int H, int W);
int cdnet_dam_head_backward(const cdnet_head_feat *f1, const cdnet_head_feat *f2, const cdnet_head_feat *f3,
                            const float *head_weights, const float *dmask, const float *dpoint, const float *ddir,
                            int N, int H, int W, uint16_t *df1, uint16_t *df2, uint16_t *df3, float *workspace,
                            size_t workspace_floats, float *dhead_weights, void *stream);
int cdnet_dam_head_backward_fused_blocks(void);
int cdnet_dam_head_backward_fused_scratch_bytes(void);
size_t cdnet_dam_head_backward_fused_workspace_floats(void);
int cdnet_dam_head_backward_fused(const cdnet_head_feat *f1, const cdnet_head_feat *f2, const cdnet_head_feat *f3,
                                  const float *head_weights, const float *dmask, const float *dpoint, const float *ddir, int N, int H,
                                  int W, float *df1, float *df2, float *dz3, float *workspace, size_t workspace_floats,
                                  float *dhead_weights, void *stream);

size_t cdnet_dam_loss_workspace_floats(int B, int P);
int cdnet_dam_loss(const float *mask, const float *point, const float *direction, const uint8_t *label,
                   const uint8_t *dirlab, const uint16_t *point_target_f16, const uint8_t *weight_u8, int B, int H, int W,
                   int quirk_sample0, float *workspace, size_t workspace_floats, float *losses, float *dmask,
                   float *dpoint, float *ddir, void *stream);
size_t cdnet_dam_loss_classes_workspace_floats(int B, int P, int direction_classes);
int cdnet_dam_loss_classes(const float *mask, const float *point, const float *direction, const uint8_t *label,
                           const uint8_t *dirlab, const uint16_t *point_target_f16, const uint8_t *weight_u8, int B, int H, int W,
                           int direction_classes, int quirk_sample0, float *workspace, size_t workspace_floats, float *losses,
                           float *dmask, float *dpoint, float *ddir, void *stream);

#define CDNET_LOSS_WMAP 1u
#define CDNET_LOSS_CE   2u
#define CDNET_LOSS_DICE 4u

int cdnet_dam_loss_terms(const float *mask, const float *point, const float *direction, const uint8_t *label,
                         const uint8_t *dirlab, const uint16_t *point_target_f16, const uint8_t *weight_u8, int B, int H, int W,
                         int direction_classes, int quirk_sample0, float *workspace, size_t workspace_floats, float *losses,
                         float *dmask, float *dpoint, float *ddir, void *stream, unsigned terms);

size_t cdnet_mask_loss_workspace_floats(int B, int P);
int cdnet_mask_loss(const float *mask_logits, const uint8_t *label, const uint8_t *weight_u8, int B, int H, int W, unsigned terms,
                    float *workspace, size_t workspace_floats, float *losses, float *dmask, void *stream);

size_t cdnet_variance_loss_workspace_bytes(int B, int K, int H, int W);
int cdnet_variance_loss(const float *mask_logits, const uint8_t *label, int fg_value, int B, int K, int H, int W, float alpha,
                        void *workspace, size_t workspace_bytes, float *loss_var, float *total, float *dmask, int32_t *root_out,
                        int32_t *counts, void *stream);

size_t cdnet_boundary_loss_workspace_bytes(int kind, int B, int K, int H, int W);
int cdnet_boundary_loss(const float *mask_logits, const uint8_t *label, int kind, int B, int K, int H, int W, float beta,
                        void *workspace, size_t workspace_bytes, float *loss_out, float *total, float *dmask, void *stream);
int cdnet_boundary_loss_scratch_bytes(void);

#define CDNET_VAL_SUMS 42
size_t cdnet_dam_val_sums_workspace_floats(int B, int P);
int cdnet_dam_val_sums(const float *mask, const float *point, const float *dirn, const uint8_t *label, const uint8_t *dirlab,
                       const uint16_t *point_target_f16, const uint8_t *weight_u8, const int *dir_rank_host, int B, int H, int W,
                       float *workspace, size_t workspace_floats, float *sums, void *stream);
size_t cdnet_dam_val_sums_classes_workspace_floats(int B, int P, int direction_classes);
int cdnet_dam_val_sums_classes(const float *mask, const float *point, const float *dirn, const uint8_t *label, const uint8_t *dirlab,
                               const uint16_t *point_target_f16, const uint8_t *weight_u8, const int *dir_rank_host,
                               int direction_classes, int B, int H, int W, float *workspace, size_t workspace_floats, float *sums,
                               void *stream);

int cdnet_adam_step(float *param, const float *grad, float *exp_avg, float *exp_avg_sq, size_t n, float lr, float beta1,
                    float beta2, float eps, float weight_decay, int step, float grad_scale, void *stream);

int cdnet_moment_step(float *param, const float *grad, float *exp_avg, float *exp_avg_sq, float *slow, size_t n, double beta1,
                      double beta2, float grad_scale, int move, int rect, float decay, float step_size, float v_div, float eps,
                      int sync, float alpha, void *stream);
int cdnet_sgd_step(float *param, const float *grad, float *momentum_buffer, size_t n, float lr, float momentum, float weight_decay,
                   int step, float grad_scale, void *stream);

int cdnet_window_pack(const float *img, int C, int H, int W, int view_xform, int tile_h, int tile_w, int stride, int ny,
                      int nx, void *out_bf16_nhwc16, void *stream);
int cdnet_window_pack_f32(const float *img, int C, int H, int W, int view_xform, int tile_h, int tile_w, int stride, int ny,
                          int nx, float *out_f32_nhwc16, void *stream);
int cdnet_window_stitch(const float *tiles, int K, int tile_h, int tile_w, int stride, int overlap, int ny, int nx, int Hv,
                        int Wv, float *out, void *stream);

typedef struct cdnet_aug_sample {
    double minv[6];
    const uint8_t *img;
    const uint8_t *weight;
    const void *label;
    int32_t H, W, img_stride, weight_stride, label_stride, label_i32;
    float color[4];
    int32_t hflip, vflip, filter, y0, x0;
    float alpha, sigma;
    uint32_t seed;
} cdnet_aug_sample;
size_t cdnet_augment_workspace_bytes(int B, int size, int max_radius);
int cdnet_augment_batch(const cdnet_aug_sample *samples, const cdnet_aug_sample *samples_host, int B, int size, const float *norm_host,
                        void *workspace, size_t workspace_bytes, float *image, uint8_t *weight, void *label, int label_i32, int32_t *varied,
                        float *field, void *stream);

typedef struct cdnet_aug_geo {
    double paff[6];
    double rinv[6];
    int32_t Hr, Wr, fy0, fx0;
    uint32_t flags;
    int32_t reserved;
} cdnet_aug_geo;
size_t cdnet_augment_geo_workspace_bytes(int B, int size, int max_radius, int field_edge);
int cdnet_augment_batch_geo(const cdnet_aug_sample *samples, const cdnet_aug_sample *samples_host, const cdnet_aug_geo *geo,
                            const cdnet_aug_geo *geo_host, int field_edge, int B, int size, const float *norm_host, void *workspace,
                            size_t workspace_bytes, float *image, uint8_t *weight, void *label, int label_i32, int32_t *varied, float *field,
                            void *stream);

size_t cdnet_label_encoding_workspace_bytes(int N, int H, int W, int max_instances);
int cdnet_label_encoding(const uint8_t *label_ch0, int N, int H, int W, int max_instances, const double *rays_host,
                         const double *gauss_host, void *workspace, size_t workspace_bytes, uint8_t *label3,
                         uint16_t *point_f16, uint8_t *direction, int32_t *inst_out, int32_t *counts_out, void *stream);
size_t cdnet_label_encoding_instances_workspace_bytes(int N, int H, int W, int max_instances);
int cdnet_label_encoding_instances(const int32_t *label_inst, int N, int H, int W, int max_instances, const double *rays_host,
                                   const double *gauss_host, void *workspace, size_t workspace_bytes, uint8_t *label3,
                                   uint16_t *point_f16, uint8_t *direction, int32_t *inst, int32_t *counts, void *stream);

typedef struct cdnet_fuse_term {
    const uint16_t *x;
    int Hs, Ws;
    const float *scale;
    const float *shift;
    int f16, pad_;
} cdnet_fuse_term;
int cdnet_fuse_sum(const cdnet_fuse_term *terms, int nterm, int N, int H, int W, int C, int relu, uint16_t *out, int out_cstride,
                   int out_coff, void *stream);

int cdnet_upsample_bilinear_backward(const uint16_t *dout, int N, int H, int W, int C, int dout_cstride, int dout_coff, int Hs, int Ws,
                                     uint16_t *din, void *stream);
int cdnet_s2d_to_nhwc(const uint16_t *in, int N, int H2, int W2, int C, uint16_t *out, void *stream);
int cdnet_fuse_sum_f32(const cdnet_fuse_term *terms, int nterm, int N, int H, int W, int C, int relu, float *out, int out_cstride,
                       int out_coff, void *stream);
int cdnet_upsample_bilinear_backward_f32(const float *dout, int N, int H, int W, int C, int dout_cstride, int dout_coff, int Hs, int Ws,
                                         float *din, void *stream);
int cdnet_s2d_to_nhwc_f32(const float *in, int N, int H2, int W2, int C, float *out, void *stream);

typedef struct cdnet_grad_term {
    const uint16_t *g;
    int cstride, coff;
} cdnet_grad_term;
int cdnet_grad_sum(const cdnet_grad_term *terms, int nterm, const uint16_t *mask, long long npix, int C, uint16_t *out, void *stream);
int cdnet_grad_sum_f32(const cdnet_grad_term *terms, int nterm, const float *mask, long long npix, int C, float *out, void *stream);

int cdnet_label_pair_histogram(const int32_t *true_lab, const int32_t *pred_lab, int N, int plane, int cap, int hash_slots,
                               int32_t *area_true, int32_t *area_pred, uint32_t *hash_keys, int32_t *hash_counts, int32_t *err_flag,
                               void *stream);
int cdnet_remap_label(const int32_t *lab, int N, int plane, int cap, int32_t *scratch, int32_t *out, int32_t *err_flag, void *stream);
int cdnet_label_areas(const int32_t *lab, int N, int plane, int cap, int32_t *area, int32_t *err_flag, void *stream);
int cdnet_label_apply(const int32_t *lab, int N, int plane, int cap, const int32_t *lut, int32_t *out, void *stream);

size_t cdnet_label_csr_workspace_bytes(int cap);
int cdnet_label_csr(const int32_t *lab, int H, int W, int cap, void *workspace, size_t workspace_bytes, int32_t *tab, int32_t *pix,
                    int32_t *bpix, int32_t *err_flag, void *stream);
int cdnet_hausdorff_tile_pixels(void);
int cdnet_hausdorff_chunk_pixels(void);
int cdnet_hausdorff_pairs(const int32_t *true_lab, const int32_t *true_tab, const int32_t *true_pix, const int32_t *true_bpix,
                          const int32_t *pred_lab, const int32_t *pred_tab, const int32_t *pred_pix, const int32_t *pred_bpix, int H, int W,
                          int cap, const int32_t *pairs, int M, const int32_t *items, int n_items, int32_t *d2, int32_t *err_flag,
                          void *stream);

int cdnet_weight_map_radius(double w0, double sigma);
int cdnet_weight_map(const int32_t *instances, int H, int W, double w0, double sigma, uint8_t *weight, void *stream);

#ifdef __cplusplus
}
#endif
#endif
```

Baseline: 1093.

## Recompute head feature gradients from per-pixel coefficients inside BN backward sums pass

The fused head backward kernel can now write a compact 16-float per-pixel coefficient buffer instead of full 64-channel df1/df2 gradient tensors. The BN backward sums pass of the residual form then rebuilds those gradients on the fly as small dot products with head weights loaded into registers. This removes the writing and re-reading of two N×H×W×64 fp32 gradient tensors, at the cost of extra FMAs and register pressure in the BN kernel. It is limited to fp32, C=64, flat residual BN with dz reuse, and is guarded by tape checks.

Measured after the change: 1110, median of 6. 1.02x the previous value.

```diff
diff --git a/cdnet_amd/_lib.py b/cdnet_amd/_lib.py
--- a/cdnet_amd/_lib.py
+++ b/cdnet_amd/_lib.py
@@ -52,7 +52,9 @@
 class BnBwdArgs(C.Structure):
     _fields_ = [('raw', C.c_void_p), ('res', C.c_void_p), ('scale', C.c_void_p), ('shift', C.c_void_p),
                 ('mean', C.c_void_p), ('invstd', C.c_void_p), ('gin', GradIn * 3), ('ngin', C.c_int),
-                ('f16', C.c_int), ('relu', C.c_int), ('N', C.c_int), ('H', C.c_int), ('W', C.c_int), ('C', C.c_int)]
+                ('f16', C.c_int), ('relu', C.c_int), ('N', C.c_int), ('H', C.c_int), ('W', C.c_int), ('C', C.c_int),
+                ('hc_coef', C.c_void_p), ('hc_w', C.c_void_p), ('hc_slot', C.c_int), ('hc_k0', C.c_int), ('hc_nk', C.c_int),
+                ('hc_pad_', C.c_int)]
 
 
 class AugSample(C.Structure):
@@ -205,6 +207,8 @@
     'cdnet_dam_head_backward_fused_scratch_bytes': (_i, []),
     'cdnet_dam_head_backward_fused_workspace_floats': (_sz, []),
     'cdnet_dam_head_backward_fused': (_i, [_vp] * 7 + [_i, _i, _i, _vp, _vp, _vp, _vp, _sz, _vp, _vp]),
+    'cdnet_dam_head_backward_coef_scratch_bytes': (_i, []),
+    'cdnet_dam_head_backward_coef': (_i, [_vp] * 7 + [_i, _i, _i, _vp, _vp, _vp, _sz, _vp, _vp]),
     'cdnet_dam_loss_workspace_floats': (_sz, [_i, _i]),
     'cdnet_dam_loss': (_i, [_vp] * 7 + [_i, _i, _i, _i, _vp, _sz, _vp, _vp, _vp, _vp, _vp]),
     'cdnet_dam_loss_classes_workspace_floats': (_sz, [_i, _i, _i]),
diff --git a/cdnet_amd/csrc/bn_bwd.hip b/cdnet_amd/csrc/bn_bwd.hip
--- a/cdnet_amd/csrc/bn_bwd.hip
+++ b/cdnet_amd/csrc/bn_bwd.hip
@@ -28,6 +28,8 @@
     unsigned short *draw;
     unsigned short *dz_out;
     int rev;
+    const float *hc_coef, *hc_w;
+    int hc_slot, hc_nk;
 };
 
 
@@ -344,8 +346,34 @@
     if (!APPLY) bn_write_partial<8>(A.partial, A.C, VPP, s1, s2);
 }
 
-template <int NG, bool RES, bool APPLY>
+constexpr int HC_K0(int nk) { return nk == 3 ? 10 : 1; }
+template <int NK> struct HcRow;
+template <> struct HcRow<3> {
+    f32x2 a; float b;
+    __device__ __forceinline__ void load(const float *row) { a = *reinterpret_cast<const f32x2 *>(row + 10); b = row[12]; }
+    template <int K> __device__ __forceinline__ float at() const { if constexpr (K < 2) return a[K]; else return b; }
+};
+template <> struct HcRow<9> {
+    f32x4 a, b; f32x2 c;
+    __device__ __forceinline__ void load(const float *row) {
+        a = *reinterpret_cast<const f32x4 *>(row); b = *reinterpret_cast<const f32x4 *>(row + 4); c = *reinterpret_cast<const f32x2 *>(row + 8);
+    }
+    template <int K> __device__ __forceinline__ float at() const {
+        if constexpr (K < 3) return a[K + 1]; else if constexpr (K < 7) return b[K - 3]; else return c[K - 7];
+    }
+};
+template <> struct HcRow<0> {
+    __device__ __forceinline__ void load(const float *) {}
+};
+template <int NK, int K = 0>
+__device__ __forceinline__ float hc_value(const HcRow<NK> &row, const float (*w)[4], int j, float v = 0.f) {
+    if constexpr (K < NK) return hc_value<NK, K + 1>(row, w, j, fmaf(row.template at<K>(), w[K][j], v));
+    else return v;
+}
+
+template <int NG, bool RES, bool APPLY, int HS = -1, int NK = 0>
 __global__ __launch_bounds__(256) void bn_bwd_flat32_kernel(BnBwdArgs A) {
+    static_assert(HS < NG && (HS < 0) == (NK == 0) && (HS < 0 || (RES && !APPLY)), "head-coefficient source: sums pass of the residual form");
     const int VPP = A.C / 4;
     const int slot = (int)threadIdx.x % VPP, c0 = slot * 4;
     float sc[4], sh[4], mu[4], is[4], k1[4], k2[4], k3[4], s1[4], s2[4];
@@ -358,8 +386,14 @@
     const bool relu = A.relu != 0, outmask = A.relu == 2;
     const float *raw = reinterpret_cast<const float *>(A.raw), *resp = reinterpret_cast<const float *>(A.res);
     float *draw = reinterpret_cast<float *>(A.draw), *dzo = reinterpret_cast<float *>(A.dz_out);
+    float hw[NK > 0 ? NK : 1][4];
+#pragma unroll
+    for (int k = 0; k < NK; ++k)
+#pragma unroll
+        for (int j = 0; j < 4; ++j) hw[k][j] = A.hc_w[k * 64 + c0 + j];
     for (unsigned p0 = first_pixel(ppb, VPP); p0 < npix; p0 += step * BN_U) {
         f32x4 x[BN_U], r[BN_U], g[BN_U][NG];
+        HcRow<NK> hc[BN_U];
 #pragma unroll
         for (int u = 0; u < BN_U; ++u) {
             unsigned p = p0 + u * step;
@@ -369,7 +403,8 @@
             if (RES) r[u] = *reinterpret_cast<const f32x4 *>(resp + (size_t)p * A.C + c0);
 #pragma unroll
             for (int k = 0; k < NG; ++k)
-                g[u][k] = *reinterpret_cast<const f32x4 *>(reinterpret_cast<const float *>(A.gin[k].g) + (size_t)p * A.gin[k].cstride + A.gin[k].coff + c0);
+                if (k != HS) g[u][k] = *reinterpret_cast<const f32x4 *>(reinterpret_cast<const float *>(A.gin[k].g) + (size_t)p * A.gin[k].cstride + A.gin[k].coff + c0);
+            if (HS >= 0) hc[u].load(A.hc_coef + (size_t)p * 16);
         }
 #pragma unroll
         for (int u = 0; u < BN_U; ++u) {
@@ -380,9 +415,10 @@
             for (int j = 0; j < 4; ++j) {
                 float v = fmaf(x[u][j], sc[j], sh[j]);
                 if (RES) v = outmask ? r[u][j] : v + r[u][j];
-                float gs = g[u][0][j];
-#pragma unroll
-                for (int k = 1; k < NG; ++k) gs += g[u][k][j];
+                const float hv = hc_value<NK>(hc[u], hw, j);
+                float gs = HS == 0 ? hv : g[u][0][j];
+#pragma unroll
+                for (int k = 1; k < NG; ++k) gs += k == HS ? hv : g[u][k][j];
                 const float dz = (!valid || (relu && !(v > 0.f))) ? 0.f : gs;
                 const float xh = (x[u][j] - mu[j]) * is[j];
                 if (APPLY) { o[j] = k1[j] * (dz - k2[j] - xh * k3[j]); z[j] = dz; }
@@ -554,7 +590,7 @@
 
 }
 
-static int fill_bn_args(const cdnet_bn_bwd_args *a, BnBwdArgs &A, const char *who) {
+static int fill_bn_args(const cdnet_bn_bwd_args *a, BnBwdArgs &A, const char *who, bool hc_ok = false) {
     CDNET_REQUIRE(a && a->raw, "%s: null pointer", who);
     CDNET_REQUIRE(a->C % 8 == 0 && a->C >= 8 && a->C <= 2048 , "%s: C=%d unsupported", who, a->C);
     CDNET_REQUIRE(a->ngin >= 1 && a->ngin <= 3, "%s: ngin=%d", who, a->ngin);
@@ -564,11 +600,19 @@
         A.gin[k].g = a->gin[k].g; A.gin[k].Hg = a->gin[k].Hg; A.gin[k].Wg = a->gin[k].Wg;
         A.gin[k].oy = a->gin[k].oy; A.gin[k].ox = a->gin[k].ox; A.gin[k].pooled = a->gin[k].pooled;
         A.gin[k].coff = a->gin[k].coff; A.gin[k].cstride = a->gin[k].cstride ? a->gin[k].cstride : a->C;
-        if (k < a->ngin) CDNET_REQUIRE(a->gin[k].g, "%s: null gradient input %d", who, k);
+        if (k < a->ngin) CDNET_REQUIRE(a->gin[k].g || (a->hc_nk && k == a->hc_slot), "%s: null gradient input %d", who, k);
         if (k < a->ngin) CDNET_REQUIRE(a->gin[k].Hg >= 1 && a->gin[k].Wg >= 1, "%s: empty gradient input %d (%d x %d)", who, k, a->gin[k].Hg, a->gin[k].Wg);
     }
     A.ngin = a->ngin; A.N = a->N; A.H = a->H; A.W = a->W; A.C = a->C;
     A.partial = nullptr; A.k1 = A.k2 = A.k3 = nullptr; A.draw = nullptr; A.dz_out = nullptr;
+    A.hc_coef = a->hc_coef; A.hc_w = a->hc_w; A.hc_slot = a->hc_slot; A.hc_nk = a->hc_nk;
+    if (a->hc_nk) {
+        CDNET_REQUIRE(hc_ok, "%s: no head-coefficient source here (cdnet_bn_backward, flat fp32 residual form only)", who);
+        CDNET_REQUIRE((a->hc_nk == 3 || a->hc_nk == 9) && a->hc_k0 == HC_K0(a->hc_nk) && a->hc_coef && a->hc_w && a->C == 64 && a->hc_slot >= 0 &&
+                      a->hc_slot < a->ngin && !a->gin[a->hc_slot].g,
+                      "%s: head-coefficient source: hc_nk=%d hc_k0=%d hc_slot=%d C=%d (3 terms from column 10 or 9 from column 1, 64 channels, a slot "
+                      "below ngin whose g is NULL)", who, a->hc_nk, a->hc_k0, a->hc_slot, a->C);
+    }
     return CDNET_OK;
 }
 
@@ -632,6 +676,21 @@
     auto flat = [&](auto ng, auto res) {
         constexpr int NG = decltype(ng)::value;
         constexpr bool RES = decltype(res)::value;
+        if constexpr (RES && !APPLY) {
+            if (A.hc_nk) {
+                auto hc = [&](auto hs) {
+                    constexpr int HS = decltype(hs)::value;
+                    if constexpr (HS < NG) {
+                        if (A.hc_nk == 3) bn_bwd_flat32_kernel<NG, true, false, HS, 3><<<P.nb, 256, 0, st>>>(A);
+                        else bn_bwd_flat32_kernel<NG, true, false, HS, 9><<<P.nb, 256, 0, st>>>(A);
+                    }
+                };
+                if (A.hc_slot == 0) hc(std::integral_constant<int, 0>{});
+                else if (A.hc_slot == 1) hc(std::integral_constant<int, 1>{});
+                else hc(std::integral_constant<int, 2>{});
+                return;
+            }
+        }
         if (P.f32) bn_bwd_flat32_kernel<NG, RES, APPLY><<<P.nb, 256, 0, st>>>(A);
         else bn_bwd_flat_kernel<NG, RES, APPLY><<<P.nb, 256, 0, st>>>(A);
     };
@@ -680,7 +739,7 @@
 extern "C" int cdnet_bn_backward(const cdnet_bn_bwd_args *a, const float *gamma, float *dgamma, float *dbeta, float *workspace,
                                  size_t workspace_floats, uint16_t *draw, uint16_t *dz_out, void *stream) {
     BnBwdArgs A;
-    int rc = fill_bn_args(a, A, "cdnet_bn_backward");
+    int rc = fill_bn_args(a, A, "cdnet_bn_backward", true);
     if (rc) return rc;
     hipStream_t st = (hipStream_t)stream;
     const size_t npix = bn_npix(A);
@@ -689,6 +748,8 @@
     CDNET_REQUIRE(A.relu != 2 || (P.flat_sources && A.res), "cdnet_bn_backward: relu = 2 (mask from the stored output) needs same-size gradient sources and res");
     static const bool dz_reuse = !(getenv("CDNET_BN_DZ_REUSE") && atoi(getenv("CDNET_BN_DZ_REUSE")) == 0);
     const bool reuse = dz_reuse && P.path == BN_FLAT && A.mean && A.res && dz_out;
+    CDNET_REQUIRE(!A.hc_nk || (reuse && P.f32), "cdnet_bn_backward: a head-coefficient source needs fp32 tensors, same-size sources, BatchNorm, res and dz_out "
+                  "(the flat fp32 residual form, its second pass on the stored dz)");
     A.draw = draw;
     A.rev = 1;
     if (A.mean) {
diff --git a/cdnet_amd/csrc/head_bwd.hip b/cdnet_amd/csrc/head_bwd.hip
--- a/cdnet_amd/csrc/head_bwd.hip
+++ b/cdnet_amd/csrc/head_bwd.hip
@@ -332,11 +332,12 @@
     }
 }
 
+template <bool COEF>
 __global__ __launch_bounds__(512)
 void dam_head_bwd_fused_kernel(const float *__restrict__ f1, const float *__restrict__ f2, const float *__restrict__ f3,
                                const HeadW *__restrict__ hw, const float *__restrict__ dmask, const float *__restrict__ dpoint,
                                const float *__restrict__ ddir, int N, int plane, float *__restrict__ df1, float *__restrict__ df2,
-                               float *__restrict__ dz3, float *__restrict__ partial, float *__restrict__ sgbuf) {
+                               float *__restrict__ coef, float *__restrict__ dz3, float *__restrict__ partial, float *__restrict__ sgbuf) {
     __shared__ HeadW w;
     __shared__ __attribute__((aligned(16))) float s_cf[128 * 16];
     __shared__ __attribute__((aligned(16))) float s_f[3][128 * HF_ROW];
@@ -417,10 +418,12 @@
         }
         stage(F1, 2);
         __builtin_amdgcn_sched_barrier(0);
-        xf_axpy16(dm[0], w.wm[0] + q * 16, v, false);
-        xf_axpy16(dm[1], w.wm[1] + q * 16, v, true);
-        xf_axpy16(dm[2], w.wm[2] + q * 16, v, true);
-        if (ok) { stf8(df1, e, v); stf8(df1, e + 8, v + 8); }
+        if (!COEF) {
+            xf_axpy16(dm[0], w.wm[0] + q * 16, v, false);
+            xf_axpy16(dm[1], w.wm[1] + q * 16, v, true);
+            xf_axpy16(dm[2], w.wm[2] + q * 16, v, true);
+            if (ok) { stf8(df1, e, v); stf8(df1, e + 8, v + 8); }
+        }
         __builtin_amdgcn_sched_barrier(0);
         const float dq2 = dg2 * sg2 * (1.f - sg2);
         float du[9], dd[9], dg1 = 0.f;
@@ -430,9 +433,11 @@
             dg1 = fmaf(dd[k], u[k], dg1);
             du[k] = dd[k] * g1;
         }
-#pragma unroll
-        for (int k = 0; k < 9; ++k) xf_axpy16(du[k], w.wd[k] + q * 16, v, k != 0);
-        if (ok) { stf8(df2, e, v); stf8(df2, e + 8, v + 8); }
+        if (!COEF) {
+#pragma unroll
+            for (int k = 0; k < 9; ++k) xf_axpy16(du[k], w.wd[k] + q * 16, v, k != 0);
+            if (ok) { stf8(df2, e, v); stf8(df2, e + 8, v + 8); }
+        }
         __builtin_amdgcn_sched_barrier(0);
         const float dsg1 = dg1 * sg1 * (1.f - sg1);
         const float dpt = go_p + dsg1 * w.a1;
@@ -469,6 +474,7 @@
             else if (q == 2) cf = make_float4(du[7], du[8], dm[0], dm[1]);
             else cf = make_float4(dm[2], 0.f, 0.f, 0.f);
             *reinterpret_cast<float4 *>(s_cf + slot * 16 + q * 4) = cf;
+            if (COEF && ok) *reinterpret_cast<float4 *>(coef + ii * 16 + q * 4) = cf;
         }
         __syncthreads();
         if (sh < 2) {
@@ -683,12 +689,20 @@
 }
 
 extern "C" int cdnet_dam_head_backward_fused_blocks(void) { return HEAD_FUSED_BLOCKS; }
-extern "C" int cdnet_dam_head_backward_fused_scratch_bytes(void) {
+template <bool COEF>
+static int head_fused_scratch_bytes() {
     hipFuncAttributes at;
-    if (hipFuncGetAttributes(&at, reinterpret_cast<const void *>(dam_head_bwd_fused_kernel)) != hipSuccess) return -1;
+    if (hipFuncGetAttributes(&at, reinterpret_cast<const void *>(dam_head_bwd_fused_kernel<COEF>)) != hipSuccess) return -1;
     return (int)at.localSizeBytes;
 }
+extern "C" int cdnet_dam_head_backward_fused_scratch_bytes(void) { return head_fused_scratch_bytes<false>(); }
+extern "C" int cdnet_dam_head_backward_coef_scratch_bytes(void) { return head_fused_scratch_bytes<true>(); }
 extern "C" size_t cdnet_dam_head_backward_fused_workspace_floats(void) { return (size_t)HEAD_FUSED_BLOCKS * (HEADW_FLOATS + 64 * 24); }
+
+static int head_backward_fused(const char *who, const cdnet_head_feat *f1, const cdnet_head_feat *f2, const cdnet_head_feat *f3,
+                               const float *head_weights, const float *dmask, const float *dpoint, const float *ddir, int N, int H, int W,
+                               float *df1, float *df2, float *coef, float *dz3, float *workspace, size_t workspace_floats,
+                               float *dhead_weights, void *stream);
 
 extern "C" int cdnet_dam_head_backward_fused(const cdnet_head_feat *f1, const cdnet_head_feat *f2, const cdnet_head_feat *f3,
                                              const float *head_weights, const float *dmask, const float *dpoint, const float *ddir,
@@ -696,23 +710,42 @@
                                              size_t workspace_floats, float *dhead_weights, void *stream) {
     CDNET_REQUIRE(f1 && f2 && f3 && head_weights && dmask && dpoint && ddir && df1 && df2 && dz3 && workspace && dhead_weights,
                   "cdnet_dam_head_backward_fused: null pointer");
+    return head_backward_fused("cdnet_dam_head_backward_fused", f1, f2, f3, head_weights, dmask, dpoint, ddir, N, H, W, df1, df2, nullptr, dz3,
+                               workspace, workspace_floats, dhead_weights, stream);
+}
+
+extern "C" int cdnet_dam_head_backward_coef(const cdnet_head_feat *f1, const cdnet_head_feat *f2, const cdnet_head_feat *f3,
+                                            const float *head_weights, const float *dmask, const float *dpoint, const float *ddir,
+                                            int N, int H, int W, float *coef, float *dz3, float *workspace, size_t workspace_floats,
+                                            float *dhead_weights, void *stream) {
+    CDNET_REQUIRE(f1 && f2 && f3 && head_weights && dmask && dpoint && ddir && coef && dz3 && workspace && dhead_weights,
+                  "cdnet_dam_head_backward_coef: null pointer");
+    return head_backward_fused("cdnet_dam_head_backward_coef", f1, f2, f3, head_weights, dmask, dpoint, ddir, N, H, W, nullptr, nullptr, coef, dz3,
+                               workspace, workspace_floats, dhead_weights, stream);
+}
+
+static int head_backward_fused(const char *who, const cdnet_head_feat *f1, const cdnet_head_feat *f2, const cdnet_head_feat *f3,
+                               const float *head_weights, const float *dmask, const float *dpoint, const float *ddir, int N, int H, int W,
+                               float *df1, float *df2, float *coef, float *dz3, float *workspace, size_t workspace_floats,
+                               float *dhead_weights, void *stream) {
     auto plain32 = [](const cdnet_head_feat &f) { return f.raw && f.f16 == 2 && !f.scale && !f.shift && !f.relu && !f.res; };
     CDNET_REQUIRE(plain32(*f1) && plain32(*f2) && plain32(*f3),
-                  "cdnet_dam_head_backward_fused: plain stored fp32 features only (f16 = 2, no scale / shift / relu / res)");
-    CDNET_REQUIRE(N >= 1 && H >= 1 && W >= 1, "cdnet_dam_head_backward_fused: N=%d H=%d W=%d", N, H, W);
-    CDNET_REQUIRE((size_t)N * H * W * 64 < ((size_t)1 << 32), "cdnet_dam_head_backward_fused: tensor too large for 32-bit element indexing");
+                  "%s: plain stored fp32 features only (f16 = 2, no scale / shift / relu / res)", who);
+    CDNET_REQUIRE(N >= 1 && H >= 1 && W >= 1, "%s: N=%d H=%d W=%d", who, N, H, W);
+    CDNET_REQUIRE((size_t)N * H * W * 64 < ((size_t)1 << 32), "%s: tensor too large for 32-bit element indexing", who);
     static_assert(HEAD_FUSED_BLOCKS == 1024, "the chains of the two-kernel path: 1024 workgroups");
     const int nb = HEAD_FUSED_BLOCKS;
     const size_t need = (size_t)nb * (HEADW_FLOATS + 64 * 24);
-    if (workspace_floats < need) { set_error("cdnet_dam_head_backward_fused: workspace %zu < %zu floats", workspace_floats, need); return CDNET_E_WORKSPACE; }
+    if (workspace_floats < need) { set_error("%s: workspace %zu < %zu floats", who, workspace_floats, need); return CDNET_E_WORKSPACE; }
     hipStream_t st = (hipStream_t)stream;
     float *partial = workspace, *sgbuf = workspace + (size_t)nb * HEADW_FLOATS;
     auto fp = [](const cdnet_head_feat &f) { return reinterpret_cast<const float *>(f.raw); };
-    dam_head_bwd_fused_kernel<<<nb, 512, 0, st>>>(fp(*f1), fp(*f2), fp(*f3), reinterpret_cast<const HeadW *>(head_weights), dmask, dpoint, ddir,
-                                                  N, H * W, df1, df2, dz3, partial, sgbuf);
+    const HeadW *hw = reinterpret_cast<const HeadW *>(head_weights);
+    if (coef) dam_head_bwd_fused_kernel<true><<<nb, 512, 0, st>>>(fp(*f1), fp(*f2), fp(*f3), hw, dmask, dpoint, ddir, N, H * W, df1, df2, coef, dz3, partial, sgbuf);
+    else dam_head_bwd_fused_kernel<false><<<nb, 512, 0, st>>>(fp(*f1), fp(*f2), fp(*f3), hw, dmask, dpoint, ddir, N, H * W, df1, df2, coef, dz3, partial, sgbuf);
     head_scalar_reduce_kernel<<<nb, 64, 0, st>>>(sgbuf, partial);
     reduce_partials_kernel<<<cdiv(HEADW_FLOATS, 4), 256, 0, st>>>(workspace, nb, HEADW_FLOATS, dhead_weights);
-    return check_launch("cdnet_dam_head_backward_fused");
+    return check_launch(who);
 }
 
 extern "C" size_t cdnet_final_conv1x1_backward_workspace_floats(void) { return (size_t)1025 * (FC_KMOST * 64 + FC_KMOST); }
diff --git a/cdnet_amd/trainer.py b/cdnet_amd/trainer.py
--- a/cdnet_amd/trainer.py
+++ b/cdnet_amd/trainer.py
@@ -17,6 +17,7 @@
 _RU_1X1_SIDE = True
 WGRAD_STREAM = True
 HEAD_BWD_FUSE = True
+HEAD_COEF_SRC = os.environ.get('CDNET_HEAD_COEF_SRC', '1') != '0'
 _WGRAD_DEFER = 0x100
 _WGRAD_DEEP_HW = 16384
 
@@ -37,12 +38,13 @@
 
 
 class _G:
-    __slots__ = ('t', 'Hg', 'Wg', 'oy', 'ox', 'pooled', 'coff', 'cstride', 'event', 'masked')
+    __slots__ = ('t', 'Hg', 'Wg', 'oy', 'ox', 'pooled', 'coff', 'cstride', 'event', 'masked', 'hc')
 
     def __init__(self, t, Hg, Wg, oy=0, ox=0, pooled=0, coff=0, cstride=0):
         self.t, self.Hg, self.Wg, self.oy, self.ox, self.pooled, self.coff, self.cstride = t, Hg, Wg, oy, ox, pooled, coff, cstride
         self.event = None
         self.masked = False
+        self.hc = None
 
 
 def _choose_ci_tiles(C_src, Cout):
@@ -102,6 +104,7 @@
         self._packb_stream = True
         self._side_active = False
         self.head_fused = False
+        self.head_coef = False
         self._rd_mb = float(os.environ.get('CDNET_WGRAD_REDUCE_MB', '300'))
         self._rd_pending, self._rd_params, self._rd_bytes, self._rd_tables = [], [], 0, {}
         self._forwards, self._bn_base = 0, 0
@@ -254,11 +257,27 @@
         m = self.model
         f1, f2, f3 = m._last_feats
         N, H, W, _ = f1.x.shape
-        df = [self.buf('dF%d' % k, (N, H, W, 64), runtime.act_dtype()) for k in range(3)]
         hf = [runtime.head_feat(f) for f in (f1, f2, f3)]
         dhead = self.flat.G[:self.flat.n_head]
         owner = self._head_fusable(f1, f2, f3)
         self.head_fused = owner is not None
+        self.head_coef = owner is not None and HEAD_COEF_SRC and os.environ.get('CDNET_BN_DZ_REUSE', '1').strip() not in ('0', '') \
+            and self._head_coef_ok(f1) and self._head_coef_ok(f2)
+        if self.head_coef:
+            coef = self.buf('head_coef', (N, H, W, 16), torch.float32)
+            dz3 = self.buf('dF2', (N, H, W, 64), torch.float32)
+            hw = m.head_weight_block()
+            ws = self._ws('head', _lib.load().cdnet_dam_head_backward_fused_workspace_floats())
+            _lib.call('cdnet_dam_head_backward_coef', C.byref(hf[0]), C.byref(hf[1]), C.byref(hf[2]), _lib.ptr(hw), _lib.ptr(dmask),
+                      _lib.ptr(dpoint), _lib.ptr(ddir), N, H, W, _lib.ptr(coef), _lib.ptr(dz3), _lib.ptr(ws), ws.numel(), _lib.ptr(dhead),
+                      _lib.stream_ptr())
+            heads = [(f1.x, _G(None, H, W)), (f2.x, _G(None, H, W)), (f3.x, _G(dz3, H, W))]
+            heads[0][1].hc = (coef, hw, 640, 10, 3)
+            heads[1][1].hc = (coef, hw, 64, 1, 9)
+            heads[2][1].masked = True
+            self._run_tape(heads, None)
+            return
+        df = [self.buf('dF%d' % k, (N, H, W, 64), runtime.act_dtype()) for k in range(3)]
         if owner is not None:
             ws = self._ws('head', _lib.load().cdnet_dam_head_backward_fused_workspace_floats())
             _lib.call('cdnet_dam_head_backward_fused', C.byref(hf[0]), C.byref(hf[1]), C.byref(hf[2]), _lib.ptr(m.head_weight_block()),
@@ -273,6 +292,22 @@
                   _lib.ptr(dmask), _lib.ptr(dpoint), _lib.ptr(ddir), N, H, W, _lib.ptr(df[0]), _lib.ptr(df[1]),
                   _lib.ptr(df[2]), _lib.ptr(ws), ws.numel(), _lib.ptr(dhead), _lib.stream_ptr())
         self._run_tape([((f.grad_to or (f.x,))[0], _G(d, H, W)) for f, d in zip((f1, f2, f3), df)], None)
+
+    def _head_coef_ok(self, f):
+        readers = 0
+        for Rt in self.tape:
+            if isinstance(Rt, runtime.FuseRecord):
+                if any(t.x is f.x for t in Rt.terms):
+                    return False
+                continue
+            for sx in Rt.srcs:
+                if sx.res is f.x or (sx.x is f.x and (sx.pool or tuple(sx.off) != (0, 0))):
+                    return False
+                readers += sx.x is f.x
+        P = next((Rt for Rt in self.tape if not isinstance(Rt, runtime.FuseRecord) and Rt.out is f.x), None)
+        owner = None if P is None or P.layer.kind != 'conv1' else P.fused_res_of
+        return readers <= 2 and owner is not None and owner.layer.bn is not None and owner.relu == 2 and owner.res is f.x \
+            and owner.out.dtype == torch.float32 and tuple(owner.out.shape) == tuple(f.x.shape)
 
     def _head_fusable(self, f1, f2, f3):
         if not HEAD_BWD_FUSE or runtime.PRECISION != 'fp32' or getattr(self.model, 'VARIANT', None) != 'rev1':
@@ -549,7 +584,10 @@
         a.ngin = len(gl)
         assert 1 <= len(gl) <= 3, (L.name, len(gl))
         for k, g in enumerate(gl):
-            a.gin[k].g = g.t.data_ptr()
+            if g.hc is not None:
+                coef, hw, w0, k0, nk = g.hc
+                a.hc_coef, a.hc_w, a.hc_slot, a.hc_k0, a.hc_nk = coef.data_ptr(), hw.data_ptr() + 4 * w0, k, k0, nk
+            a.gin[k].g = None if g.t is None else g.t.data_ptr()
             a.gin[k].Hg, a.gin[k].Wg, a.gin[k].oy, a.gin[k].ox = g.Hg, g.Wg, g.oy, g.ox
             a.gin[k].pooled, a.gin[k].coff, a.gin[k].cstride = int(g.pooled), g.coff, g.cstride or out.shape[3]
         a.f16 = {torch.bfloat16: 0, torch.float16: 1, torch.float32: 2}[out.dtype]
diff --git a/include/cdnet_hip.h b/include/cdnet_hip.h
--- a/include/cdnet_hip.h
+++ b/include/cdnet_hip.h
@@ -312,6 +312,8 @@
     int ngin;
     int f16, relu;
     int N, H, W, C;
+    const float *hc_coef, *hc_w;
+    int hc_slot, hc_k0, hc_nk, hc_pad_;
 } cdnet_bn_bwd_args;
 
 size_t cdnet_bn_backward_workspace_floats(int C);
@@ -341,6 +343,11 @@
                                   const float *head_weights, const float *dmask, const float *dpoint, const float *ddir, int N, int H,
                                   int W, float *df1, float *df2, float *dz3, float *workspace, size_t workspace_floats,
                                   float *dhead_weights, void *stream);
+int cdnet_dam_head_backward_coef_scratch_bytes(void);
+int cdnet_dam_head_backward_coef(const cdnet_head_feat *f1, const cdnet_head_feat *f2, const cdnet_head_feat *f3,
+                                 const float *head_weights, const float *dmask, const float *dpoint, const float *ddir, int N, int H,
+                                 int W, float *coef, float *dz3, float *workspace, size_t workspace_floats, float *dhead_weights,
+                                 void *stream);
 
 size_t cdnet_dam_loss_workspace_floats(int B, int P);
 int cdnet_dam_loss(const float *mask, const float *point, const float *direction, const uint8_t *label,
```
